# Restream/reindexer

Hardware: NVIDIA H100
Metric: KNN QPS @ recall@10 (10Mx768, k=10) + HBM GB/s vs roofline (higher is better)
Workload: dtype f32

## Files before the change

### include/rxgpu.h

```cpp
#ifndef RXGPU_H
#define RXGPU_H

#include <stddef.h>
#include <stdint.h>

#ifdef __cplusplus
extern "C" {
#endif

#define RXGPU_ABI_VERSION 4

enum { RXGPU_OK = 0, RXGPU_ERR_PARAMS = 3, RXGPU_ERR_LOGIC = 4, RXGPU_ERR_NOT_FOUND = 13, RXGPU_ERR_SYSTEM = 37 };

typedef enum { RXGPU_L2 = 0, RXGPU_IP = 1, RXGPU_COS = 2 } rxgpu_metric;

enum {
	RXGPU_FLAG_HOST_MIRROR = 1u
};

typedef struct rxgpu_index rxgpu_index;

const char* rxgpu_last_error(void);
int rxgpu_abi_version(void);
int rxgpu_device_count(void);
// ... 145 lines not shown
int rxgpu_sq8_prepare_query(const rxgpu_index*, const float* query, float query_norm, uint8_t* codes, float* offset);
int rxgpu_sq8_search_knn(const rxgpu_index*, uint32_t nq, const float* queries , const float* query_norms,
						 uint32_t k, float* out_dist, uint64_t* out_label, uint32_t* out_count);
int rxgpu_hnsw_search_knn_sq8(const rxgpu_index*, uint32_t nq, const float* queries , const float* query_norms, uint32_t k, uint32_t ef,
							  float* out_dist, uint64_t* out_label, uint32_t* out_count, uint32_t* stats );

int rxgpu_ivf_import(rxgpu_index*, uint32_t nlist, const float* centroids , const uint64_t* list_sizes );
int rxgpu_ivf_search_knn(const rxgpu_index*, uint32_t nq, const float* queries , uint32_t k, uint32_t nprobe, float* out_dist,
						 uint64_t* out_label, uint32_t* out_count);
int rxgpu_ivf_search_knn_large_k(const rxgpu_index*, uint32_t nq, const float* queries , uint32_t k, uint32_t nprobe,
								 float* out_dist, uint64_t* out_label, uint32_t* out_count);
int rxgpu_ivf_search_range(const rxgpu_index*, const float* query , float radius, uint32_t nprobe, uint64_t max_out,
						   float* out_dist, uint64_t* out_label, uint64_t* out_n);
int rxgpu_ivf_search_range_batch(const rxgpu_index*, uint32_t nq, const float* queries ,
								 const float* radius , uint32_t nprobe, uint64_t max_out,
								 float* out_dist, uint64_t* out_label, uint64_t* out_n );

int rxgpu_ivf_create(rxgpu_index*, uint32_t nlist, const float* centroids );
int rxgpu_ivf_add(rxgpu_index*, uint64_t n, const uint32_t* list_nos, const uint64_t* labels, const float* vecs );
int rxgpu_ivf_remove(rxgpu_index*, uint64_t label);
uint64_t rxgpu_ivf_size(const rxgpu_index*);
int rxgpu_ivf_list_stats(const rxgpu_index*, uint64_t* slab_rows, uint64_t* dead_rows, uint64_t* relocations, uint64_t* compactions);

typedef struct {
	int32_t niter;
	int32_t seed;
	int32_t max_points_per_centroid;
} rxgpu_ivf_train_params;
typedef struct {
	double obj;
	int32_t nsplit;
	float assign_ms;
	float update_ms;
	float host_ms;
} rxgpu_ivf_train_stats;
int rxgpu_ivf_train(rxgpu_index*, uint32_t nlist, uint64_t n, const float* vecs ,
					const float* norm_coefs , const rxgpu_ivf_train_params* params, float* out_centroids,
					rxgpu_ivf_train_stats* stats);
int rxgpu_ivf_assign(const rxgpu_index*, uint64_t n, const float* vecs , const float* norm_coefs, uint32_t* out_list_nos,
					 float* out_dist);
int rxgpu_ivf_add_assign(rxgpu_index*, uint64_t n, const uint64_t* labels, const float* vecs , const float* norm_coefs,
						 uint32_t* out_list_nos);
int rxgpu_kmeans_plan(uint64_t n, uint32_t nlist, int32_t seed, int32_t max_points_per_centroid, int32_t* out_sample, int32_t* out_init);

typedef struct {
	uint32_t ndocs;
	const uint32_t* doc_ids;
	const uint32_t* pos_begin;
	const uint32_t* positions;
} rxgpu_ft_postings;
typedef struct {
	double bm25_boost, bm25_weight, term_len_boost, term_len_weight, position_boost, position_weight;
} rxgpu_ft_field_config;
typedef struct {
	uint32_t merge_limit;
	int32_t min_rank;
	double bm25_k1, bm25_b;
	int32_t bm25_type;
	double distance_boost, distance_weight, full_match_boost;
	uint32_t nfields;
	const rxgpu_ft_field_config* fields;
	double summation_ranks_by_fields_ratio;
} rxgpu_ft_config;
typedef struct {
	int32_t op;
	float boost;
	float term_len_boost;
	const float* field_boosts;
	uint32_t nsubterms;
	const uint32_t* postings;
	const float* procs;
	const uint8_t* need_sum_rank;
	const uint8_t* suppressed;
	uint32_t nsynonyms;
	const uint32_t* synonym_ids;
	int32_t phrase_num;
	int32_t distance;
} rxgpu_ft_term;
typedef struct {
	uint32_t nterms;
	const rxgpu_ft_term* terms;
} rxgpu_ft_synonym;
typedef struct {
	uint32_t nterms;
	const rxgpu_ft_term* terms;
	uint32_t nsynonyms;
	const rxgpu_ft_synonym* synonyms;
} rxgpu_ft_query;
typedef struct {
	int32_t id;
	float proc;
	uint8_t field;
	uint8_t normalized_proc;
} rxgpu_ft_merge_info;
typedef struct rxgpu_ft_index rxgpu_ft_index;

int rxgpu_ft_create(rxgpu_ft_index** out, uint32_t total_docs, uint32_t nfields, const uint32_t* words_in_field, const float* avg_words,
					const uint8_t* removed, int device);
void rxgpu_ft_destroy(rxgpu_ft_index*);
int rxgpu_ft_add_postings(rxgpu_ft_index*, const rxgpu_ft_postings* list, uint32_t* out_id);
int rxgpu_ft_add_postings_packed(rxgpu_ft_index*, const uint8_t* data, uint64_t len, uint32_t count, uint32_t* out_id);
int rxgpu_ft_add_postings_packed_batch(rxgpu_ft_index*, uint32_t nlists, const uint8_t* const* data, const uint64_t* lens,
									   const uint32_t* counts, uint32_t* out_ids);
int rxgpu_ft_decode_packed(const uint8_t* data, uint64_t len, uint32_t count, uint32_t* doc_ids, uint32_t* pos_begin,
						   uint32_t* positions, uint64_t max_positions, uint64_t* npos);
int rxgpu_ft_merge(rxgpu_ft_index*, const rxgpu_ft_config* cfg, uint32_t nterms, const rxgpu_ft_term* terms, const uint8_t* excluded,
				   int rank_sort_type, uint64_t max_out, rxgpu_ft_merge_info* out, uint64_t* out_n);
int rxgpu_ft_merge_query(rxgpu_ft_index*, const rxgpu_ft_config* cfg, const rxgpu_ft_query* query, const uint8_t* excluded, int rank_sort_type,
						 uint64_t max_out, rxgpu_ft_merge_info* out, uint64_t* out_n);
typedef struct {
	uint32_t start, end;
} rxgpu_ft_area;
int rxgpu_ft_merge_query_areas(rxgpu_ft_index*, const rxgpu_ft_config* cfg, const rxgpu_ft_query* query, const uint8_t* excluded,
							   int rank_sort_type, int32_t max_areas_in_doc, uint64_t max_out, rxgpu_ft_merge_info* out,
							   uint32_t* out_area_begin, rxgpu_ft_area* out_areas, uint32_t* out_raw_count, uint64_t* out_n);
int rxgpu_ft_set_rows(rxgpu_ft_index*, const uint32_t* row_begin, const int32_t* row_ids);
int rxgpu_ft_select(rxgpu_ft_index*, const rxgpu_ft_config* cfg, uint32_t nterms, const rxgpu_ft_term* terms, const uint8_t* excluded,
					const uint8_t* row_status , int rank_sort_type, uint64_t limit, int32_t* out_row_ids,
					float* out_ranks , uint64_t* out_n);
int rxgpu_ft_select_query(rxgpu_ft_index*, const rxgpu_ft_config* cfg, const rxgpu_ft_query* query, const uint8_t* excluded,
						  const uint8_t* row_status, int rank_sort_type, uint64_t limit, int32_t* out_row_ids, float* out_ranks, uint64_t* out_n);
int rxgpu_sharded_ft_select(rxgpu_comm*, rxgpu_ft_index* shard, uint32_t doc_base, const rxgpu_ft_config* cfg, uint32_t nterms,
							const rxgpu_ft_term* terms, const uint8_t* excluded, const uint8_t* row_status, int rank_sort_type, uint64_t limit,
							int32_t* out_row_ids, float* out_ranks, uint64_t* out_n);
typedef struct {
	uint32_t launches;
	uint32_t preselected;
	uint64_t postings_scanned;
	uint64_t algorithmic_bytes;
	float device_ms;
} rxgpu_ft_stats;
void rxgpu_ft_last_stats(rxgpu_ft_stats* out);

int rxgpu_index_append_synth(rxgpu_index*, uint64_t seed, uint64_t first_row, uint64_t n);
int rxgpu_synth_fill_device(float* d_out, uint64_t seed, uint64_t first_index, uint64_t count, int device, void* stream);
int rxgpu_set_query_tile(rxgpu_index*, uint32_t qt);
typedef struct {
	uint32_t launches;
	uint32_t passes;
	uint32_t query_tile;
	uint32_t tie_replays;
	uint32_t tie_from_lists;
	uint64_t algorithmic_bytes;
	uint32_t scan_launches;
	float scan_kernel_ms;
	uint32_t tc_used;
	uint32_t tc_fallbacks;
	uint64_t tc_candidates;
	uint32_t tc_cluster;
	uint32_t tc_kernel;
} rxgpu_search_stats;
void rxgpu_last_search_stats(rxgpu_search_stats* out);
int rxgpu_set_tensor_core_filter(rxgpu_index*, int mode);
int rxgpu_set_profile(int on);
int rxgpu_tc_diag(int mode, void* d_counters);
int rxgpu_tc_audit(const rxgpu_index*, uint32_t nq, const float* queries, const float* tau, uint32_t query_block, uint32_t* out_shape,
                   uint32_t* slot_row, float* rowc, float* blockc, signed char* row_codes, signed char* query_codes, float* qc, float* kab,
                   int32_t* block_thr, float* row_bound);

#ifdef __cplusplus
}
#endif
#endif
```

### reindexer_b200/binding.py

```python
from __future__ import annotations

import ctypes as C
import os

import numpy as np

_HERE = os.path.dirname(os.path.abspath(__file__))
LIB_PATH = os.path.join(_HERE, "librxgpu.so")

L2, IP, COS = 0, 1, 2
FLAG_HOST_MIRROR = 1

_f32p = C.POINTER(C.c_float)
_u64p = C.POINTER(C.c_uint64)
_u32p = C.POINTER(C.c_uint32)
_i32p = C.POINTER(C.c_int32)
_u8p = C.POINTER(C.c_uint8)


class RxGpuError(RuntimeError):
    def __init__(self, code, msg):
        super().__init__(f"[{code}] {msg}")
        self.code = code
        self.what = msg
# ... 36 lines not shown
                ("postings", _u32p), ("procs", _f32p), ("need_sum_rank", _u8p), ("suppressed", _u8p), ("nsynonyms", C.c_uint32),
                ("synonym_ids", _u32p), ("phrase_num", C.c_int32), ("distance", C.c_int32)]


class FtSynonym(C.Structure):
    _fields_ = [("nterms", C.c_uint32), ("terms", C.POINTER(FtTerm))]


class FtQuery(C.Structure):
    _fields_ = [("nterms", C.c_uint32), ("terms", C.POINTER(FtTerm)), ("nsynonyms", C.c_uint32), ("synonyms", C.POINTER(FtSynonym))]


class Sq8Params(C.Structure):
    _fields_ = [("min_q", C.c_float), ("max_q", C.c_float), ("alpha", C.c_float), ("alpha_2", C.c_float), ("delta", C.c_float)]


class FtStats(C.Structure):
    _fields_ = [("launches", C.c_uint32), ("preselected", C.c_uint32), ("postings_scanned", C.c_uint64), ("algorithmic_bytes", C.c_uint64),
                ("device_ms", C.c_float)]


FT_MERGE_INFO_DTYPE = np.dtype([("id", np.int32), ("proc", np.float32), ("field", np.uint8), ("normalized_proc", np.uint8)], align=True)


class IvfTrainParams(C.Structure):
    _fields_ = [("niter", C.c_int32), ("seed", C.c_int32), ("max_points_per_centroid", C.c_int32)]


class IvfTrainStats(C.Structure):
    _fields_ = [("obj", C.c_double), ("nsplit", C.c_int32), ("assign_ms", C.c_float), ("update_ms", C.c_float), ("host_ms", C.c_float)]


class HnswBuildStats(C.Structure):
    _fields_ = [("batches", C.c_uint64), ("rows", C.c_uint64), ("distances", C.c_uint64), ("reverse_links", C.c_uint64),
                ("lists_pruned", C.c_uint64), ("search_select_ms", C.c_float), ("sort_ms", C.c_float), ("link_ms", C.c_float)]


class SearchStats(C.Structure):
    _fields_ = [("launches", C.c_uint32), ("passes", C.c_uint32), ("query_tile", C.c_uint32), ("tie_replays", C.c_uint32), ("tie_from_lists", C.c_uint32),
                ("algorithmic_bytes", C.c_uint64), ("scan_launches", C.c_uint32), ("scan_kernel_ms", C.c_float),
                ("tc_used", C.c_uint32), ("tc_fallbacks", C.c_uint32), ("tc_candidates", C.c_uint64), ("tc_cluster", C.c_uint32), ("tc_kernel", C.c_uint32)]


_SIGNATURES = {
    "rxgpu_last_error": (C.c_char_p, []),
    "rxgpu_abi_version": (C.c_int, []),
    "rxgpu_device_count": (C.c_int, []),
    "rxgpu_index_create": (C.c_int, [C.POINTER(C.c_void_p), C.c_int, C.c_uint32, C.c_uint64, C.c_int, C.c_uint32]),
    "rxgpu_index_clone": (C.c_int, [C.POINTER(C.c_void_p), C.c_void_p, C.c_uint64]),
    "rxgpu_index_destroy": (None, [C.c_void_p]),
    "rxgpu_index_resize": (C.c_int, [C.c_void_p, C.c_uint64]),
    "rxgpu_index_upsert": (C.c_int, [C.c_void_p, C.c_uint64, _f32p]),
    "rxgpu_index_upsert_batch": (C.c_int, [C.c_void_p, C.c_uint64, _u64p, _f32p]),
    "rxgpu_index_remove": (C.c_int, [C.c_void_p, C.c_uint64]),
    "rxgpu_index_get": (C.c_int, [C.c_void_p, C.c_uint64, C.POINTER(_f32p)]),
    "rxgpu_index_size": (C.c_uint64, [C.c_void_p]),
    "rxgpu_index_capacity": (C.c_uint64, [C.c_void_p]),
    "rxgpu_index_element_size": (C.c_uint64, [C.c_void_p]),
    "rxgpu_index_device_bytes": (C.c_uint64, [C.c_void_p]),
    "rxgpu_index_dim": (C.c_uint32, [C.c_void_p]),
    "rxgpu_index_metric": (C.c_int, [C.c_void_p]),
    "rxgpu_index_device": (C.c_int, [C.c_void_p]),
    "rxgpu_search_knn": (C.c_int, [C.c_void_p, C.c_uint32, _f32p, C.c_uint32, _f32p, _u64p, _u32p]),
    "rxgpu_search_range": (C.c_int, [C.c_void_p, _f32p, C.c_float, C.c_uint64, _f32p, _u64p, _u64p]),
    "rxgpu_search_range_batch": (C.c_int, [C.c_void_p, C.c_uint32, _f32p, _f32p, C.c_uint64, _f32p, _u64p, _u64p]),
    "rxgpu_last_range_results": (C.c_int, [C.c_uint64, C.c_uint64, _f32p, _u64p]),
    "rxgpu_comm_unique_id": (C.c_int, [C.c_void_p]),
    "rxgpu_comm_create": (C.c_int, [C.POINTER(C.c_void_p), C.c_int, C.c_int, C.c_void_p, C.c_int]),
    "rxgpu_comm_destroy": (None, [C.c_void_p]),
    "rxgpu_comm_rank": (C.c_int, [C.c_void_p]),
    "rxgpu_comm_size": (C.c_int, [C.c_void_p]),
    "rxgpu_sharded_search_knn": (C.c_int, [C.c_void_p, C.c_void_p, C.c_uint32, C.c_void_p, C.c_int, C.c_uint32, _f32p, _u64p, _u32p]),
    "rxgpu_sharded_search_range_batch": (C.c_int, [C.c_void_p, C.c_void_p, C.c_uint32, C.c_void_p, C.c_int, _f32p, C.c_uint64, _f32p, _u64p,
                                                   _u64p]),
    "rxgpu_shard_payload_bytes": (C.c_uint64, [C.c_uint32, C.c_uint32]),
    "rxgpu_merge_shards_device": (C.c_int, [C.c_uint32, C.c_uint32, C.c_uint32, C.c_uint32, C.c_void_p, C.c_void_p, C.c_void_p, C.c_void_p,
                                            C.c_void_p, C.c_void_p, C.c_void_p]),
    "rxgpu_search_knn_device": (C.c_int, [C.c_void_p, C.c_uint32, C.c_void_p, C.c_uint32, C.c_void_p, C.c_void_p, C.c_void_p,
                                          C.c_void_p, C.c_void_p]),
    "rxgpu_search_tie_rows_device": (C.c_int, [C.c_void_p, C.c_void_p, C.c_float, C.c_uint32, C.c_void_p, C.c_void_p, C.c_void_p,
                                               C.c_void_p, C.c_void_p]),
    "rxgpu_merge_shards": (C.c_int, [C.c_uint32, C.c_uint32, C.c_uint32, C.c_uint32, _f32p, _u32p, _u64p, _u32p, _u64p, _f32p, _u64p,
                                     _u64p, _u32p, _u8p]),
    "rxgpu_tie_replay": (C.c_int, [C.c_uint32, C.c_float, C.c_uint32, _f32p, _u64p, _u64p, C.c_uint32, _f32p, _u64p, _u64p, _f32p,
                                   _u64p, _u32p]),
    "rxgpu_select_knn": (C.c_int, [C.c_void_p, _f32p, C.POINTER(SelectParams), C.c_uint64, _i32p, _f32p, _u64p]),
    "rxgpu_select_postprocess": (C.c_int, [C.c_int, C.POINTER(SelectParams), C.c_uint64, _f32p, _u64p, _i32p, _f32p, _u64p]),
    "rxgpu_hnsw_import": (C.c_int, [C.c_void_p, C.POINTER(HnswGraph)]),
    "rxgpu_hnsw_search_knn": (C.c_int, [C.c_void_p, C.c_uint32, _f32p, C.c_uint32, C.c_uint32, _f32p, _u64p, _u32p, _u32p]),
    "rxgpu_hnsw_mark_deleted": (C.c_int, [C.c_void_p, C.c_uint64]),
    "rxgpu_hnsw_deleted_count": (C.c_uint64, [C.c_void_p]),
    "rxgpu_gather_labels_device": (C.c_int, [C.c_void_p, C.c_uint64, C.c_void_p, C.c_void_p, C.c_void_p]),
    "rxgpu_hnsw_search_range": (C.c_int, [C.c_void_p, _f32p, C.c_float, C.c_uint32, C.c_uint64, _f32p, _u64p, C.POINTER(C.c_uint64)]),
    "rxgpu_hnsw_search_range_batch": (C.c_int, [C.c_void_p, C.c_uint32, _f32p, _f32p, C.c_uint32, C.c_uint64, _f32p, _u64p, _u64p]),
    "rxgpu_hnsw_build": (C.c_int, [C.c_void_p, C.c_uint32, C.c_uint32, C.c_uint64, _i32p, C.c_uint64, C.POINTER(HnswBuildStats)]),
    "rxgpu_hnsw_build_plan": (C.c_int, [C.c_uint32, C.c_uint64, C.c_uint64, C.c_int32, _i32p, C.c_uint64, _i32p, _u64p, C.POINTER(C.c_uint64)]),
    "rxgpu_hnsw_export": (C.c_int, [C.c_void_p, C.c_uint64, _u32p, _u32p, _i32p, C.POINTER(C.c_int64), _u32p, C.POINTER(HnswGraph)]),
    "rxgpu_hnsw_search_knn_device": (C.c_int, [C.c_void_p, C.c_uint32, C.c_void_p, C.c_uint32, C.c_uint32, C.c_void_p, C.c_void_p,
                                               C.c_void_p, C.c_void_p, C.c_void_p]),
    "rxgpu_ivf_create": (C.c_int, [C.c_void_p, C.c_uint32, _f32p]),
    "rxgpu_ivf_add": (C.c_int, [C.c_void_p, C.c_uint64, _u32p, _u64p, _f32p]),
    "rxgpu_ivf_remove": (C.c_int, [C.c_void_p, C.c_uint64]),
    "rxgpu_ivf_size": (C.c_uint64, [C.c_void_p]),
    "rxgpu_ivf_list_stats": (C.c_int, [C.c_void_p, C.POINTER(C.c_uint64), C.POINTER(C.c_uint64), C.POINTER(C.c_uint64), C.POINTER(C.c_uint64)]),
    "rxgpu_hnsw_load_index_cache": (C.c_int, [C.c_void_p, C.c_void_p, C.c_void_p]),
    "rxgpu_hnsw_update": (C.c_int, [C.c_void_p, C.c_int32, C.c_uint32, C.c_uint32, C.c_void_p]),
    "rxgpu_hnsw_update_count": (C.c_uint64, [C.c_void_p]),
    "rxgpu_hnsw_stream_begin": (C.c_int, [C.c_void_p, _f32p, C.c_uint32, C.POINTER(C.c_void_p)]),
    "rxgpu_hnsw_stream_next": (C.c_int, [C.c_void_p, C.c_uint32, _f32p, _u64p, _u32p, C.POINTER(C.c_int)]),
    "rxgpu_hnsw_stream_end": (None, [C.c_void_p]),
    "rxgpu_sq8_attach": (C.c_int, [C.c_void_p, C.POINTER(Sq8Params), _u8p, _f32p]),
    "rxgpu_sq8_export": (C.c_int, [C.c_void_p, _u8p, _f32p]),
    "rxgpu_sq8_prepare_query": (C.c_int, [C.c_void_p, _f32p, C.c_float, _u8p, _f32p]),
    "rxgpu_sq8_search_knn": (C.c_int, [C.c_void_p, C.c_uint32, _f32p, _f32p, C.c_uint32, _f32p, _u64p, _u32p]),
    "rxgpu_hnsw_search_knn_sq8": (C.c_int, [C.c_void_p, C.c_uint32, _f32p, _f32p, C.c_uint32, C.c_uint32, _f32p, _u64p, _u32p, _u32p]),
    "rxgpu_ivf_import": (C.c_int, [C.c_void_p, C.c_uint32, _f32p, _u64p]),
    "rxgpu_ivf_train": (C.c_int, [C.c_void_p, C.c_uint32, C.c_uint64, _f32p, _f32p, C.POINTER(IvfTrainParams), _f32p, C.POINTER(IvfTrainStats)]),
    "rxgpu_ivf_assign": (C.c_int, [C.c_void_p, C.c_uint64, _f32p, _f32p, _u32p, _f32p]),
    "rxgpu_ivf_add_assign": (C.c_int, [C.c_void_p, C.c_uint64, _u64p, _f32p, _f32p, _u32p]),
    "rxgpu_kmeans_plan": (C.c_int, [C.c_uint64, C.c_uint32, C.c_int32, C.c_int32, _i32p, _i32p]),
    "rxgpu_ivf_search_knn": (C.c_int, [C.c_void_p, C.c_uint32, _f32p, C.c_uint32, C.c_uint32, _f32p, _u64p, _u32p]),
    "rxgpu_ivf_search_knn_large_k": (C.c_int, [C.c_void_p, C.c_uint32, _f32p, C.c_uint32, C.c_uint32, _f32p, _u64p, _u32p]),
    "rxgpu_ivf_search_range": (C.c_int, [C.c_void_p, _f32p, C.c_float, C.c_uint32, C.c_uint64, _f32p, _u64p, C.POINTER(C.c_uint64)]),
    "rxgpu_ivf_search_range_batch": (C.c_int, [C.c_void_p, C.c_uint32, _f32p, _f32p, C.c_uint32, C.c_uint64, _f32p, _u64p, _u64p]),
    "rxgpu_ft_create": (C.c_int, [C.POINTER(C.c_void_p), C.c_uint32, C.c_uint32, _u32p, _f32p, _u8p, C.c_int]),
    "rxgpu_ft_destroy": (None, [C.c_void_p]),
    "rxgpu_ft_add_postings": (C.c_int, [C.c_void_p, C.POINTER(FtPostings), _u32p]),
    "rxgpu_ft_add_postings_packed": (C.c_int, [C.c_void_p, _u8p, C.c_uint64, C.c_uint32, _u32p]),
    "rxgpu_ft_decode_packed": (C.c_int, [_u8p, C.c_uint64, C.c_uint32, _u32p, _u32p, _u32p, C.c_uint64, C.POINTER(C.c_uint64)]),
    "rxgpu_ft_merge": (C.c_int, [C.c_void_p, C.POINTER(FtConfig), C.c_uint32, C.POINTER(FtTerm), _u8p, C.c_int, C.c_uint64, C.c_void_p,
                                 C.POINTER(C.c_uint64)]),
    "rxgpu_ft_add_postings_packed_batch": (C.c_int, [C.c_void_p, C.c_uint32, C.POINTER(C.c_void_p), C.POINTER(C.c_uint64), _u32p, _u32p]),
    "rxgpu_ft_merge_query": (C.c_int, [C.c_void_p, C.c_void_p, C.c_void_p, _u8p, C.c_int, C.c_uint64, C.c_void_p, C.POINTER(C.c_uint64)]),
    "rxgpu_ft_merge_query_areas": (C.c_int, [C.c_void_p, C.c_void_p, C.c_void_p, _u8p, C.c_int, C.c_int32, C.c_uint64, C.c_void_p, _u32p,
                                              C.c_void_p, _u32p, C.POINTER(C.c_uint64)]),
    "rxgpu_ft_select_query": (C.c_int, [C.c_void_p, C.c_void_p, C.c_void_p, _u8p, _u8p, C.c_int, C.c_uint64, _i32p, _f32p,
                                         C.POINTER(C.c_uint64)]),
    "rxgpu_ft_set_rows": (C.c_int, [C.c_void_p, _u32p, _i32p]),
    "rxgpu_sharded_ft_select": (C.c_int, [C.c_void_p, C.c_void_p, C.c_uint32, C.POINTER(FtConfig), C.c_uint32, C.POINTER(FtTerm), _u8p, _u8p,
                                           C.c_int, C.c_uint64, _i32p, _f32p, C.POINTER(C.c_uint64)]),
    "rxgpu_comm_create_local": (C.c_int, [C.POINTER(C.c_void_p), C.c_int, C.POINTER(C.c_int)]),
    "rxgpu_ft_select": (C.c_int, [C.c_void_p, C.POINTER(FtConfig), C.c_uint32, C.POINTER(FtTerm), _u8p, _u8p, C.c_int, C.c_uint64, _i32p, _f32p,
                                  C.POINTER(C.c_uint64)]),
    "rxgpu_ft_last_stats": (None, [C.POINTER(FtStats)]),
    "rxgpu_index_append_synth": (C.c_int, [C.c_void_p, C.c_uint64, C.c_uint64, C.c_uint64]),
    "rxgpu_synth_fill_device": (C.c_int, [C.c_void_p, C.c_uint64, C.c_uint64, C.c_uint64, C.c_int, C.c_void_p]),
    "rxgpu_set_query_tile": (C.c_int, [C.c_void_p, C.c_uint32]),
    "rxgpu_last_search_stats": (None, [C.POINTER(SearchStats)]),
    "rxgpu_set_profile": (C.c_int, [C.c_int]),
    "rxgpu_tc_diag": (C.c_int, [C.c_int, C.c_void_p]),
    "rxgpu_tc_audit": (C.c_int, [C.c_void_p, C.c_uint32, _f32p, _f32p, C.c_uint32, _u32p, _u32p, _f32p, _f32p, C.c_void_p, C.c_void_p, _f32p,
                                 _f32p, _i32p, _f32p]),
    "rxgpu_set_tensor_core_filter": (C.c_int, [C.c_void_p, C.c_int]),
}

_lib = None


def lib():
    global _lib
    if _lib is None:
        if not os.path.exists(LIB_PATH):
            raise RxGpuError(37, f"{LIB_PATH} is missing: build the CUDA extension first (no CPU fallback exists)")
        l = C.CDLL(LIB_PATH)
        for name, (res, args) in _SIGNATURES.items():
            fn = getattr(l, name)
            fn.restype = res
            fn.argtypes = args
        _lib = l
    return _lib


def _check(rc):
    if rc != 0:
        raise RxGpuError(rc, lib().rxgpu_last_error().decode(errors="replace"))


def _p(a, t):
    return a.ctypes.data_as(t)


def device_count() -> int:
    return lib().rxgpu_device_count()


def last_search_stats() -> dict:
    s = SearchStats()
    lib().rxgpu_last_search_stats(C.byref(s))
    return {f: getattr(s, f) for f, _ in SearchStats._fields_}


class GpuBruteforceSearch:

    def __init__(self, metric: int, dim: int, capacity: int, device: int = 0, host_mirror: bool = False, _handle=None):
        self._lib = lib()
        self.metric, self.dim = metric, dim
        if _handle is not None:
            self._h = _handle
            return
        h = C.c_void_p()
        _check(self._lib.rxgpu_index_create(C.byref(h), metric, dim, capacity, device, FLAG_HOST_MIRROR if host_mirror else 0))
        self._h = h

    def close(self):
        if getattr(self, "_h", None):
            self._lib.rxgpu_index_destroy(self._h)
            self._h = None

    __del__ = close

    def clone(self, new_capacity: int) -> "GpuBruteforceSearch":
        h = C.c_void_p()
        _check(self._lib.rxgpu_index_clone(C.byref(h), self._h, new_capacity))
        return GpuBruteforceSearch(self.metric, self.dim, new_capacity, _handle=h)

    def max_elements(self) -> int:
        return self._lib.rxgpu_index_capacity(self._h)

    def current_element_count(self) -> int:
        return self._lib.rxgpu_index_size(self._h)

    size = current_element_count

    def element_size(self) -> int:
        return self._lib.rxgpu_index_element_size(self._h)

    def device_bytes(self) -> int:
        return self._lib.rxgpu_index_device_bytes(self._h)

    def add_point(self, vec, label: int):
        vec = np.ascontiguousarray(vec, dtype=np.float32)
        assert vec.size == self.dim
        _check(self._lib.rxgpu_index_upsert(self._h, label, _p(vec, _f32p)))

    def add_points(self, labels, vecs):
        vecs = np.ascontiguousarray(vecs, dtype=np.float32)
        labels = np.ascontiguousarray(labels, dtype=np.uint64)
        assert vecs.shape == (len(labels), self.dim)
        _check(self._lib.rxgpu_index_upsert_batch(self._h, len(labels), _p(labels, _u64p), _p(vecs, _f32p)))

    def remove_point(self, label: int):
        _check(self._lib.rxgpu_index_remove(self._h, label))

    def resize_index(self, new_capacity: int):
        _check(self._lib.rxgpu_index_resize(self._h, new_capacity))

    def float_ptr_by_external_label(self, label: int) -> np.ndarray:
        p = _f32p()
        _check(self._lib.rxgpu_index_get(self._h, label, C.byref(p)))
        return np.ctypeslib.as_array(p, (self.dim,)).copy()

    def search_knn(self, queries, k: int):
        q = np.ascontiguousarray(queries, dtype=np.float32)
        single = q.ndim == 1
        q = q.reshape(-1, self.dim)
        nq = q.shape[0]
        d = np.zeros((nq, max(k, 1)), np.float32)
        l = np.zeros((nq, max(k, 1)), np.uint64)
        c = np.zeros(nq, np.uint32)
        _check(self._lib.rxgpu_search_knn(self._h, nq, _p(q, _f32p), k, _p(d, _f32p), _p(l, _u64p), _p(c, _u32p)))
        if single:
            return d[0, :c[0]], l[0, :c[0]]
        return d[:, :k], l[:, :k], c

    def search_range(self, query, radius: float, max_out: int | None = None):
        q = np.ascontiguousarray(query, dtype=np.float32)
        max_out = self.size() if max_out is None else max_out
        d = np.zeros(max(max_out, 1), np.float32)
        l = np.zeros(max(max_out, 1), np.uint64)
        n = C.c_uint64(0)
        _check(self._lib.rxgpu_search_range(self._h, _p(q, _f32p), radius, max_out, _p(d, _f32p), _p(l, _u64p), C.byref(n)))
        m = min(n.value, max_out)
        return d[:m], l[:m], n.value

    def search_range_batch(self, queries, radius, max_out: int | None = None):
        q = np.ascontiguousarray(queries, dtype=np.float32).reshape(-1, self.dim)
        nq = q.shape[0]
        r = np.ascontiguousarray(np.broadcast_to(np.asarray(radius, dtype=np.float32), (nq,)))
        max_out = min(self.size(), 1 << 17) if max_out is None else max_out
        d = np.zeros((nq, max(max_out, 1)), np.float32)
        l = np.zeros((nq, max(max_out, 1)), np.uint64)
        c = np.zeros(nq, np.uint64)
        _check(self._lib.rxgpu_search_range_batch(self._h, nq, _p(q, _f32p), _p(r, _f32p), max_out, _p(d, _f32p), _p(l, _u64p),
                                                  _p(c, _u64p)))
        return d[:, :max_out], l[:, :max_out], c

    def select(self, query, k: int | None = None, radius: float | None = None, need_sort=True, is_array=False, raw=False,
               max_out: int | None = None):
        q = np.ascontiguousarray(query, dtype=np.float32)
        prm = SelectParams(k or 0, int(radius is not None), float(radius or 0.0), int(need_sort), int(is_array), int(raw))
        max_out = max_out if max_out is not None else max(self.size(), 1)
        ids = np.zeros(max_out, np.int32)
        ranks = np.zeros(max_out, np.float32)
        n = C.c_uint64(0)
        _check(self._lib.rxgpu_select_knn(self._h, _p(q, _f32p), C.byref(prm), max_out, _p(ids, _i32p), _p(ranks, _f32p), C.byref(n)))
        m = min(n.value, max_out)
        return ids[:m], ranks[:m]

    def search_knn_device(self, nq, d_queries_ptr, k1, d_dist_ptr, d_idx_ptr, d_label_ptr, d_count_ptr, stream=0):
        _check(self._lib.rxgpu_search_knn_device(self._h, nq, d_queries_ptr, k1, d_dist_ptr, d_idx_ptr, d_label_ptr, d_count_ptr,
                                                 stream or None))

    def search_tie_rows_device(self, d_query_ptr, dstar, k, d_dist_ptr, d_idx_ptr, d_label_ptr, d_count_ptr, stream=0):
        _check(self._lib.rxgpu_search_tie_rows_device(self._h, d_query_ptr, dstar, k, d_dist_ptr, d_idx_ptr, d_label_ptr, d_count_ptr,
                                                      stream or None))

# ... 114 lines not shown
    def hnsw_update_count(self) -> int:
        return int(self._lib.rxgpu_hnsw_update_count(self._h))

    def hnsw_mark_deleted(self, label: int):
        _check(self._lib.rxgpu_hnsw_mark_deleted(self._h, int(label)))

    def hnsw_deleted_count(self) -> int:
        return int(self._lib.rxgpu_hnsw_deleted_count(self._h))

    def hnsw_search_knn_device(self, nq, d_queries_ptr, k, ef, d_dist_ptr, d_idx_ptr, d_count_ptr, d_stats_ptr=0, stream=0):
        _check(self._lib.rxgpu_hnsw_search_knn_device(self._h, nq, d_queries_ptr, k, ef, d_dist_ptr, d_idx_ptr, d_count_ptr,
                                                      d_stats_ptr or None, stream or None))

    def gather_labels_device(self, n, d_idx_ptr, d_label_ptr, stream=0):
        _check(self._lib.rxgpu_gather_labels_device(self._h, n, d_idx_ptr, d_label_ptr, stream or None))

    def hnsw_search_range(self, query, radius: float, ef: int, max_out: int | None = None):
        q = np.ascontiguousarray(query, dtype=np.float32)
        max_out = self.size() if max_out is None else max_out
        d = np.zeros(max(max_out, 1), np.float32)
        l = np.zeros(max(max_out, 1), np.uint64)
        n = C.c_uint64(0)
        _check(self._lib.rxgpu_hnsw_search_range(self._h, _p(q, _f32p), radius, ef, max_out, _p(d, _f32p), _p(l, _u64p), C.byref(n)))
        m = min(n.value, max_out)
        return d[:m], l[:m], n.value

    def hnsw_search_range_batch(self, queries, radii, ef: int, max_out: int):
        q = np.ascontiguousarray(queries, dtype=np.float32).reshape(-1, self.dim)
        nq = q.shape[0]
        r = np.ascontiguousarray(np.broadcast_to(np.asarray(radii, dtype=np.float32), (nq,)))
        d = np.zeros((nq, max(max_out, 1)), np.float32)
        l = np.zeros((nq, max(max_out, 1)), np.uint64)
        c = np.zeros(nq, np.uint64)
        _check(self._lib.rxgpu_hnsw_search_range_batch(self._h, nq, _p(q, _f32p), _p(r, _f32p), ef, max_out, _p(d, _f32p), _p(l, _u64p),
                                                       _p(c, _u64p)))
        return d[:, :max_out], l[:, :max_out], c

    def hnsw_stream(self, query, batch_size: int, ef: int = 0, max_batches: int = 10**9):
        q = np.ascontiguousarray(query, np.float32)
        s = C.c_void_p()
        _check(self._lib.rxgpu_hnsw_stream_begin(self._h, _p(q, _f32p), ef, C.byref(s)))
        try:
            for _ in range(max_batches):
                d = np.zeros(max(batch_size, 1), np.float32)
                l = np.zeros(max(batch_size, 1), np.uint64)
                n, ex = C.c_uint32(0), C.c_int(0)
                _check(self._lib.rxgpu_hnsw_stream_next(s, batch_size, _p(d, _f32p), _p(l, _u64p), C.byref(n), C.byref(ex)))
                yield d[:n.value].copy(), l[:n.value].copy()
                if ex.value:
                    break
        finally:
            self._lib.rxgpu_hnsw_stream_end(s)

    def sq8_attach(self, params: dict, codes=None, offsets=None):
        p = Sq8Params(params["min_q"], params["max_q"], params["alpha"], params["alpha_2"], params["delta"])
        if codes is None:
            _check(self._lib.rxgpu_sq8_attach(self._h, C.byref(p), None, None))
        else:
            c = np.ascontiguousarray(codes, np.uint8)
            o = np.ascontiguousarray(offsets, np.float32)
            assert c.shape == (self.size(), self.dim) and o.shape == (self.size(),)
            _check(self._lib.rxgpu_sq8_attach(self._h, C.byref(p), _p(c, _u8p), _p(o, _f32p)))

    def sq8_export(self):
        codes = np.zeros((self.size(), self.dim), np.uint8)
        offs = np.zeros(self.size(), np.float32)
        _check(self._lib.rxgpu_sq8_export(self._h, _p(codes, _u8p), _p(offs, _f32p)))
        return codes, offs

    def sq8_prepare_query(self, query, query_norm=1.0):
        q = np.ascontiguousarray(query, np.float32)
        codes = np.zeros(self.dim, np.uint8)
        off = C.c_float(0)
        _check(self._lib.rxgpu_sq8_prepare_query(self._h, _p(q, _f32p), query_norm, _p(codes, _u8p), C.byref(off)))
        return codes, off.value

    def _sq8_search(self, fn, queries, k, query_norms, extra):
        q = np.ascontiguousarray(queries, dtype=np.float32).reshape(-1, self.dim)
        nq = q.shape[0]
        qn = None if query_norms is None else np.ascontiguousarray(query_norms, np.float32)
        d = np.zeros((nq, max(k, 1)), np.float32)
        l = np.zeros((nq, max(k, 1)), np.uint64)
        c = np.zeros(nq, np.uint32)
        _check(fn(self._h, nq, _p(q, _f32p), None if qn is None else _p(qn, _f32p), k, *extra, _p(d, _f32p), _p(l, _u64p), _p(c, _u32p)))
        return d, l, c

    def sq8_search_knn(self, queries, k: int, query_norms=None):
        return self._sq8_search(self._lib.rxgpu_sq8_search_knn, queries, k, query_norms, ())

    def hnsw_search_knn_sq8(self, queries, k: int, ef: int = 0, query_norms=None, with_stats=False):
        q = np.ascontiguousarray(queries, dtype=np.float32).reshape(-1, self.dim)
        nq = q.shape[0]
        qn = None if query_norms is None else np.ascontiguousarray(query_norms, np.float32)
        d = np.zeros((nq, max(k, 1)), np.float32)
        l = np.zeros((nq, max(k, 1)), np.uint64)
        c = np.zeros(nq, np.uint32)
        st = np.zeros((nq, 2), np.uint32)
        _check(self._lib.rxgpu_hnsw_search_knn_sq8(self._h, nq, _p(q, _f32p), None if qn is None else _p(qn, _f32p), k, ef, _p(d, _f32p),
                                                   _p(l, _u64p), _p(c, _u32p), _p(st, _u32p)))
        return (d, l, c, st) if with_stats else (d, l, c)

    def ivf_import(self, centroids, list_sizes):
        c = np.ascontiguousarray(centroids, np.float32)
        ls = np.ascontiguousarray(list_sizes, np.uint64)
        _check(self._lib.rxgpu_ivf_import(self._h, len(ls), _p(c, _f32p), _p(ls, _u64p)))

    def ivf_search_knn(self, queries, k: int, nprobe: int):
        q = np.ascontiguousarray(queries, dtype=np.float32).reshape(-1, self.dim)
        nq = q.shape[0]
        d = np.zeros((nq, max(k, 1)), np.float32)
        l = np.zeros((nq, max(k, 1)), np.uint64)
        c = np.zeros(nq, np.uint32)
        _check(self._lib.rxgpu_ivf_search_knn(self._h, nq, _p(q, _f32p), k, nprobe, _p(d, _f32p), _p(l, _u64p), _p(c, _u32p)))
        return d, l, c

    def ivf_search_knn_large_k(self, queries, k: int, nprobe: int):
        q = np.ascontiguousarray(queries, dtype=np.float32).reshape(-1, self.dim)
        nq = q.shape[0]
        d = np.zeros((nq, max(k, 1)), np.float32)
        l = np.zeros((nq, max(k, 1)), np.uint64)
        c = np.zeros(nq, np.uint32)
        _check(self._lib.rxgpu_ivf_search_knn_large_k(self._h, nq, _p(q, _f32p), k, nprobe, _p(d, _f32p), _p(l, _u64p), _p(c, _u32p)))
        return d, l, c

    def ivf_search_range(self, query, radius: float, nprobe: int, max_out: int | None = None):
        q = np.ascontiguousarray(query, dtype=np.float32)
        max_out = max(self.size(), self.ivf_size()) if max_out is None else max_out
        d = np.zeros(max(max_out, 1), np.float32)
        l = np.zeros(max(max_out, 1), np.uint64)
        n = C.c_uint64(0)
        _check(self._lib.rxgpu_ivf_search_range(self._h, _p(q, _f32p), radius, nprobe, max_out, _p(d, _f32p), _p(l, _u64p), C.byref(n)))
        m = min(n.value, max_out)
        return d[:m], l[:m], n.value

    def ivf_search_range_batch(self, queries, radii, nprobe: int, max_out: int):
        q = np.ascontiguousarray(queries, dtype=np.float32).reshape(-1, self.dim)
        nq = q.shape[0]
        r = np.ascontiguousarray(np.broadcast_to(np.asarray(radii, dtype=np.float32), (nq,)))
        d = np.zeros((nq, max(max_out, 1)), np.float32)
        l = np.zeros((nq, max(max_out, 1)), np.uint64)
        c = np.zeros(nq, np.uint64)
        _check(self._lib.rxgpu_ivf_search_range_batch(self._h, nq, _p(q, _f32p), _p(r, _f32p), nprobe, max_out, _p(d, _f32p), _p(l, _u64p),
                                                      _p(c, _u64p)))
        return d[:, :max_out], l[:, :max_out], c

    def append_synth(self, seed: int, first_row: int, n: int):
        _check(self._lib.rxgpu_index_append_synth(self._h, seed, first_row, n))

    def set_query_tile(self, qt: int):
        _check(self._lib.rxgpu_set_query_tile(self._h, qt))

    def set_tensor_core_filter(self, mode: int):
        _check(self._lib.rxgpu_set_tensor_core_filter(self._h, mode))

    def tc_audit(self, queries, tau, query_block: int = 128, row_bound: bool = True) -> dict:
        q = np.ascontiguousarray(queries, dtype=np.float32).reshape(-1, self.dim)
        nq = q.shape[0]
        t = np.ascontiguousarray(np.broadcast_to(np.asarray(tau, dtype=np.float32), (nq,)))
        shape = np.zeros(2, np.uint32)
        _check(self._lib.rxgpu_tc_audit(self._h, 0, None, None, query_block, _p(shape, _u32p), *([None] * 9)))
        S, B = int(shape[0]), int(shape[1])
        o = {"slot_row": np.zeros(max(S, 1), np.uint32), "rowc": np.zeros((max(S, 1), 4), np.float32),
             "blockc": np.zeros((max(B, 1), 8), np.float32), "row_codes": np.zeros((max(S, 1), self.dim), np.int8),
             "query_codes": np.zeros((max(nq, 1), self.dim), np.int8), "qc": np.zeros((max(nq, 1), 4), np.float32),
             "kab": np.zeros((max((nq + query_block - 1) // query_block, 1), 2), np.float32),
             "block_thr": np.zeros((max(nq, 1), max(B, 1)), np.int32),
             "row_bound": np.zeros((max(nq, 1), max(S, 1), 2), np.float32) if row_bound and S else None}
        _check(self._lib.rxgpu_tc_audit(self._h, nq, _p(q, _f32p), _p(t, _f32p), query_block, _p(shape, _u32p), _p(o["slot_row"], _u32p),
                                        _p(o["rowc"], _f32p), _p(o["blockc"], _f32p), o["row_codes"].ctypes.data,
                                        o["query_codes"].ctypes.data, _p(o["qc"], _f32p), _p(o["kab"], _f32p), _p(o["block_thr"], _i32p),
                                        None if o["row_bound"] is None else _p(o["row_bound"], _f32p)))
        nqb = (nq + query_block - 1) // query_block
        out = {"slot_row": o["slot_row"][:S], "rowc": o["rowc"][:S], "blockc": o["blockc"][:B], "row_codes": o["row_codes"][:S],
               "query_codes": o["query_codes"][:nq], "qc": o["qc"][:nq], "kab": o["kab"][:nqb], "block_thr": o["block_thr"][:nq, :B],
               "row_bound": None if o["row_bound"] is None else o["row_bound"][:nq, :S]}
        return out


COMM_ID_BYTES = 128


def comm_unique_id() -> bytes:
    buf = C.create_string_buffer(COMM_ID_BYTES)
    _check(lib().rxgpu_comm_unique_id(buf))
    return buf.raw


class ShardComm:

    def __init__(self, nranks: int, rank: int, comm_id: bytes | None, device: int, _handle=None):
        self._lib = lib()
        if _handle is not None:
            self._h = _handle
            return
        self._h = C.c_void_p()
        idbuf = C.create_string_buffer(comm_id, COMM_ID_BYTES) if comm_id is not None else None
        _check(self._lib.rxgpu_comm_create(C.byref(self._h), nranks, rank, idbuf, device))

    @staticmethod
    def local_group(nranks: int, devices=None):
        hs = (C.c_void_p * nranks)()
        dv = None if devices is None else (C.c_int * nranks)(*devices)
        _check(lib().rxgpu_comm_create_local(hs, nranks, dv))
        return [ShardComm(nranks, r, None, 0, _handle=C.c_void_p(hs[r])) for r in range(nranks)]

    def close(self):
        if self._h:
            self._lib.rxgpu_comm_destroy(self._h)
            self._h = C.c_void_p()

    def __del__(self):
        try:
            self.close()
        except Exception:
            pass

    def search_knn(self, shard: "GpuBruteforceSearch", queries, k: int, nq: int | None = None):
        if isinstance(queries, np.ndarray):
            q = np.ascontiguousarray(queries, np.float32)
            nq, qp, on_dev = q.shape[0], q.ctypes.data_as(C.c_void_p), 0
        else:
            qp, on_dev = C.c_void_p(int(queries)), 1
        kk = max(k, 1)
        od = np.zeros((nq, kk), np.float32)
        ol = np.zeros((nq, kk), np.uint64)
        oc = np.zeros(nq, np.uint32)
        _check(self._lib.rxgpu_sharded_search_knn(self._h, shard._h, nq, qp, on_dev, k, _p(od, _f32p), _p(ol, _u64p), _p(oc, _u32p)))
        return od, ol, oc

    def search_range_batch(self, shard: "GpuBruteforceSearch", queries, radius, max_out: int, nq: int | None = None):
        if isinstance(queries, np.ndarray):
            q = np.ascontiguousarray(queries, np.float32)
            nq, qp, on_dev = q.shape[0], q.ctypes.data_as(C.c_void_p), 0
        else:
            qp, on_dev = C.c_void_p(int(queries)), 1
        r = np.ascontiguousarray(np.broadcast_to(np.asarray(radius, dtype=np.float32), (nq,)))
        od = np.zeros((nq, max(max_out, 1)), np.float32)
        ol = np.zeros((nq, max(max_out, 1)), np.uint64)
        oc = np.zeros(nq, np.uint64)
        _check(self._lib.rxgpu_sharded_search_range_batch(self._h, shard._h, nq, qp, on_dev, _p(r, _f32p), max_out, _p(od, _f32p),
                                                          _p(ol, _u64p), _p(oc, _u64p)))
        return od[:, :max_out], ol[:, :max_out], oc


def select_postprocess(metric, dist, label, k=None, has_radius=False, need_sort=True, is_array=False, raw=False):
    d = np.ascontiguousarray(dist, np.float32)
    l = np.ascontiguousarray(label, np.uint64)
    prm = SelectParams(k or 0, int(has_radius), 0.0, int(need_sort), int(is_array), int(raw))
    ids = np.zeros(max(len(d), 1), np.int32)
    ranks = np.zeros(max(len(d), 1), np.float32)
    n = C.c_uint64(0)
    _check(lib().rxgpu_select_postprocess(metric, C.byref(prm), len(d), _p(d, _f32p), _p(l, _u64p), _p(ids, _i32p), _p(ranks, _f32p), C.byref(n)))
    return ids[:n.value], ranks[:n.value]


def merge_shards(k, dist, idx, label, count, shard_base):
    dist = np.ascontiguousarray(dist, np.float32)
    idx = np.ascontiguousarray(idx, np.uint32)
    label = np.ascontiguousarray(label, np.uint64)
    count = np.ascontiguousarray(count, np.uint32)
    base = np.ascontiguousarray(shard_base, np.uint64)
    ns, nq, k1 = dist.shape
    od = np.zeros((nq, max(k, 1)), np.float32)
    og = np.zeros((nq, max(k, 1)), np.uint64)
    ol = np.zeros((nq, max(k, 1)), np.uint64)
    oc = np.zeros(nq, np.uint32)
    nt = np.zeros(nq, np.uint8)
    _check(lib().rxgpu_merge_shards(ns, nq, k, k1, _p(dist, _f32p), _p(idx, _u32p), _p(label, _u64p), _p(count, _u32p), _p(base, _u64p),
                                    _p(od, _f32p), _p(og, _u64p), _p(ol, _u64p), _p(oc, _u32p), _p(nt, _u8p)))
    return od, og, ol, oc, nt


def tie_replay(k, dstar, lower, first):
    ld, lg, ll = (np.ascontiguousarray(a, t) for a, t in zip(lower, (np.float32, np.uint64, np.uint64)))
    fd, fg, fl = (np.ascontiguousarray(a, t) for a, t in zip(first, (np.float32, np.uint64, np.uint64)))
    od = np.zeros(max(k, 1), np.float32)
    ol = np.zeros(max(k, 1), np.uint64)
    oc = C.c_uint32(0)
    _check(lib().rxgpu_tie_replay(k, dstar, len(ld), _p(ld, _f32p), _p(lg, _u64p), _p(ll, _u64p), len(fd), _p(fd, _f32p), _p(fg, _u64p),
                                  _p(fl, _u64p), _p(od, _f32p), _p(ol, _u64p), C.byref(oc)))
    return od[:oc.value], ol[:oc.value]


class GpuFtIndex:

    def __init__(self, total_docs, words_in_field, avg_words, removed=None, device=0):
        self._lib = lib()
        w = np.ascontiguousarray(words_in_field, np.uint32).reshape(total_docs, -1)
        self.total_docs, self.nfields = total_docs, w.shape[1]
        a = np.ascontiguousarray(avg_words, np.float32)
        r = None if removed is None else np.ascontiguousarray(removed, np.uint8)
        h = C.c_void_p()
        _check(self._lib.rxgpu_ft_create(C.byref(h), total_docs, self.nfields, _p(w, _u32p), _p(a, _f32p), None if r is None else _p(r, _u8p),
                                         device))
        self._h = h

    def close(self):
        if getattr(self, "_h", None):
            self._lib.rxgpu_ft_destroy(self._h)
            self._h = None

    __del__ = close

    def add_postings(self, doc_ids, pos_begin, positions) -> int:
        d = np.ascontiguousarray(doc_ids, np.uint32)
        b = np.ascontiguousarray(pos_begin, np.uint32)
# ... 161 lines not shown
```

### reindexer_b200/csrc/index.cu

```cuda
#include <cuda_runtime.h>

#include <cub/device/device_radix_sort.cuh>
#include <cub/device/device_scan.cuh>
#include <cub/device/device_segmented_radix_sort.cuh>
#include <cub/device/device_segmented_sort.cuh>

#include <algorithm>
#include <atomic>
#include <cstdio>
#include <cstdlib>
#include <cstring>
#include <limits>
#include <memory>
#include <mutex>
#include <new>
#include <string>
#include <unordered_map>
#include <unordered_set>
#include <vector>

#include "../../include/rxgpu.h"
#include "internal.h"
#include "../host/knn_select.h"
#include "knn_scan.cuh"
// ... 520 lines not shown
		auto convert = [&](uint32_t b, uint32_t e) {
			const unsigned blocks = unsigned((uint64_t(e - b) * 32 + 255) / 256);
			tc_convert_rows<<<blocks, 256, 0, st>>>(ix->d_rows, ix->pitch, ix->dim, b, e, ix->d_row_slot, static_cast<unsigned char*>(ix->d_shadow),
													pitchQ / kTcChunkK, ix->metric == RXGPU_COS ? ix->d_norms : nullptr, ix->d_rowc);
			g_stats.launches += 1;
		};
		bool full = ix->shadow_dirty_all;
		if (!full) {
			const uint32_t kept = std::min(old, size), added = size - kept, gone = old - kept;
			uint64_t rewritten = 0;
			for (const auto& r : ix->shadow_dirty) {
				rewritten += r.first < kept ? std::min(r.second, kept) - r.first : 0u;
			}
			const uint64_t slots = uint64_t(ix->shadow_slots) + added;
			full = slots > ix->shadow_slot_cap ||
				   (uint64_t(ix->shadow_dead) + gone + ix->shadow_unsorted + added + rewritten) * kShadowResortDiv > slots;
			if (!full) {
				if (gone) {
					tc_kill_rows<<<(gone + 255) / 256, 256, 0, st>>>(kept, old, ix->d_row_slot, ix->d_slot_row, ix->d_rowc);
					g_stats.launches += 1;
				}
				for (const auto& r : ix->shadow_dirty) {
					if (r.first < kept) {
						convert(r.first, std::min(r.second, kept));
					}
				}
				if (added) {
					tc_assign_slots<<<(added + 255) / 256, 256, 0, st>>>(kept, size, ix->shadow_slots, ix->d_slot_row, ix->d_row_slot);
					g_stats.launches += 1;
					convert(kept, size);
				}
				ix->shadow_slots = uint32_t(slots);
				ix->shadow_dead += gone;
				ix->shadow_unsorted += uint32_t(added + rewritten);
			}
		}
		if (full) {
			if (size) {
				if (int rc = sortShadowSlots(ix, st, size)) {
					return rc;
				}
				convert(0, size);
			}
			ix->shadow_slots = size;
			ix->shadow_dead = 0;
			ix->shadow_unsorted = 0;
		}
		ix->shadow_rows = size;
		ix->shadow_dirty_all = false;
		ix->shadow_dirty.clear();
		const uint32_t slots = ix->shadow_slots;
		const uint64_t padded = (uint64_t(slots) + kTcTileRows - 1) / kTcTileRows * kTcTileRows;
		RX_CUDA(cudaMemsetAsync(ix->d_rowc + slots, 0, size_t(padded - slots) * sizeof(float4), st));
		const uint32_t nblocks = uint32_t(padded / 64);
		if (nblocks) {
			tc_block_consts<<<(nblocks * 32 + 255) / 256, 256, 0, st>>>(ix->d_rowc, ix->d_slot_row, slots, nblocks,
																		   1.f - tc_l2eps(ix->dim), ix->metric, ix->d_blockc);
			g_stats.launches += 1;
		}
		RX_CUDA(cudaGetLastError());
		RX_CUDA(cudaStreamSynchronize(st));
		ix->shadow_version = ix->version;
	}
	return 0;
}

constexpr uint32_t kTcClusterDefault = 2;
constexpr uint64_t kTcClusterMinRows = 1u << 23;
uint32_t tcClusterSize(uint32_t nblocks, uint32_t ntiles, uint32_t cmax) {
	for (uint32_t c = cmax; c > 1; c /= 2) {
		const uint32_t pad = (c - nblocks % c) % c;
		if (ntiles >= 2 && pad <= 1 && pad < nblocks) {
			return c;
		}
	}
	return 1;
}

struct TcBatch {
	uint32_t nq, nqb, cluster, ngroups, nqPad, kchunks, stages, queueSlots;
	int diag;
	size_t smem;
	int resident;
	TcKernel kfn;
	CUtensorMap mapQ;
};

int tcPrepare(const rxgpu_index* ix, Workspace& ws, cudaStream_t st, const float* d_queries, uint32_t nq, uint32_t candCap, TcBatch& b) {
	if (int rc = ensureShadow(ix, st)) {
		return rc;
	}
	const uint32_t pitchQ = ix->pitch_q, kchunks = pitchQ / kTcChunkK;
	const uint32_t nqb = tcQueryBlock(nq, kchunks);
	const uint32_t ntiles = uint32_t((ix->size + kTcTileRows - 1) / kTcTileRows);
	const uint32_t nblocks = (nq + nqb - 1) / nqb;
	const uint32_t cmax = ix->tc_cluster_max ? ix->tc_cluster_max : ix->size >= kTcClusterMinRows ? kTcClusterDefault : 1u;
	const uint32_t cluster = tcClusterSize(nblocks, ntiles, cmax);
	const uint32_t ngroups = (nblocks + cluster - 1) / cluster;
	const uint32_t nqPad = ngroups * cluster * nqb;
	RX_CUDA(ws.d_qcodes.ensure(size_t(nqPad) * pitchQ));
	RX_CUDA(ws.d_qc.ensure(nqPad));
	RX_CUDA(ws.d_qf.ensure(size_t(nqPad) * pitchQ));
	RX_CUDA(ws.d_tau.ensure(nqPad));
	RX_CUDA(ws.d_cand_count.ensure(nqPad));
	RX_CUDA(ws.d_cand_rows.ensure(size_t(nqPad) * candCap));
	RX_CUDA(ws.h_cand_count.ensure(nqPad));
	tc_prepare_queries<<<(nqPad * 32 + 255) / 256, 256, 0, st>>>(d_queries, nq, nqPad, ix->dim, pitchQ, ws.d_qcodes.p, ws.d_qc.p,
																 ws.d_qf.p);
	g_stats.launches += 1;
	RX_CUDA(cudaGetLastError());
	if (int rc = makeCodeMap(&b.mapQ, ws.d_qcodes.p, pitchQ, nqPad, nqb)) {
		return rc;
	}
	b.kfn = tcKernel(nqb, cluster);
	b.stages = tc_ring_stages(nqb, kchunks, kTcSmemLimit);
	b.queueSlots = tc_queue_slots(nqb, kchunks, b.stages, kTcSmemLimit);
	b.smem = tc_smem_bytes(nqb, kchunks, b.stages) + tc_queue_bytes(b.queueSlots);
	if (b.stages == 0 || b.queueSlots == 0) {
		return fail(RXGPU_ERR_SYSTEM, "rxgpu: no room for the tensor-core filter's candidate queues");
	}
	b.diag = g_tc_diag.load();
	if (const int diag = b.diag) {
		if (nqb != 128) {
			return fail(RXGPU_ERR_PARAMS, "rxgpu: the diagnostic filter instantiations take query blocks of 128");
		}
		b.kfn = tcDiagKernel(diag, cluster);
	}
	RX_CUDA(raiseSmemCeilingOnce(b.kfn, ix->device, int(kTcSmemLimit)));
	cudaLaunchConfig_t cfg{};
	cfg.gridDim = dim3(unsigned(ix->sm_count) / cluster * cluster);
	cfg.blockDim = dim3(kTcThreads);
	cfg.dynamicSmemBytes = b.smem;
	cudaLaunchAttribute attr[1];
	attr[0].id = cudaLaunchAttributeClusterDimension;
	attr[0].val.clusterDim.x = cluster;
	attr[0].val.clusterDim.y = 1;
	attr[0].val.clusterDim.z = 1;
	cfg.attrs = attr;
	cfg.numAttrs = 1;
	b.resident = 0;
	RX_CUDA(cudaOccupancyMaxActiveClusters(&b.resident, b.kfn, &cfg));
	if (b.resident < 1) {
		return fail(RXGPU_ERR_SYSTEM, "rxgpu: tensor-core filter kernel cannot be made resident");
	}
	b.nq = nq;
	b.nqb = nqb;
	b.cluster = cluster;
	b.ngroups = ngroups;
	b.nqPad = nqPad;
	b.kchunks = kchunks;
	return 0;
}

int tcLaunch(const rxgpu_index* ix, Workspace& ws, cudaStream_t st, const TcBatch& b, uint32_t k1, uint32_t candCap, uint32_t nrows, bool fixedTau) {
	const uint32_t nq = b.nq, nqb = b.nqb, cluster = b.cluster, ngroups = b.ngroups, kchunks = b.kchunks, pitchQ = ix->pitch_q;
	const uint32_t ntiles = (nrows + kTcTileRows - 1) / kTcTileRows;
	const int resident = b.resident;
	const TcKernel kfn = b.kfn;
	const CUtensorMap mapQ = b.mapQ;
	RX_CUDA(cudaMemsetAsync(ws.d_cand_count.p, 0, size_t(b.nqPad) * 4, st));
	RX_CUDA(cudaGetLastError());
	cudaLaunchConfig_t cfg{};
	cfg.blockDim = dim3(kTcThreads);
	cfg.dynamicSmemBytes = b.smem;
	cfg.stream = st;
	cudaLaunchAttribute attr[1];
	attr[0].id = cudaLaunchAttributeClusterDimension;
	attr[0].val.clusterDim.x = cluster;
	attr[0].val.clusterDim.y = 1;
	attr[0].val.clusterDim.z = 1;
	cfg.attrs = attr;
	cfg.numAttrs = 1;
	TcArgs a{};
	a.shadow = static_cast<const unsigned char*>(ix->d_shadow);
	a.rowc = ix->d_rowc;
	a.slot_row = ix->d_slot_row;
	a.blockc = ix->d_blockc;
	a.qc = ws.d_qc.p;
	a.tau = ws.d_tau.p;
	a.ub_list = fixedTau ? nullptr : ws.d_ub_list.p;
	a.ub_lock = fixedTau ? nullptr : ws.d_ub_lock.p;
	a.init_rows = fixedTau ? UINT32_MAX : uint32_t(std::min<uint64_t>(ix->size, kTcInitRows));
	a.rows = ix->d_rows;
	a.norm_coefs = ix->metric == RXGPU_COS ? ix->d_norms : nullptr;
	a.qf = ws.d_qf.p;
	a.pitch = ix->pitch;
	a.cand_rows = ws.d_cand_rows.p;
	a.cand_count = ws.d_cand_count.p;
	a.cand_cap = candCap;
	a.n = nrows;
	a.dim = ix->dim;
	a.kchunks = kchunks;
	a.nq_total = nq;
	a.k1 = k1;
	a.metric = ix->metric;
	a.queue_slots = b.queueSlots;
	a.stages = b.stages;
	a.diag = g_tc_diag_buf;
	for (uint32_t g0 = 0; g0 < ngroups;) {
		const uint32_t groups = std::min<uint32_t>(ngroups - g0, uint32_t(resident));
		const uint32_t walkers = uint32_t(std::min<uint64_t>(uint32_t(resident) / groups, ntiles));
		cfg.gridDim = dim3(groups * walkers * cluster);
		a.q0 = g0 * cluster * nqb;
		a.groups = groups;
		cudaEvent_t e0 = nullptr, e1 = nullptr;
		if (g_profile.load(std::memory_order_relaxed)) {
			RX_CUDA(cudaEventCreate(&e0));
			RX_CUDA(cudaEventCreate(&e1));
			RX_CUDA(cudaEventRecord(e0, st));
		}
		RX_CUDA(cudaLaunchKernelEx(&cfg, kfn, mapQ, a));
		RX_CUDA(cudaGetLastError());
		if (e0) {
			RX_CUDA(cudaEventRecord(e1, st));
			g_prof_events.emplace_back(e0, e1);
		}
		g_stats.launches += 1;
		g_stats.passes += 1;
		const uint32_t served = std::min(groups * cluster * nqb, nq - a.q0);
		g_stats.algorithmic_bytes += uint64_t(nrows) * pitchQ + uint64_t(nrows) * sizeof(float4) + uint64_t(served) * pitchQ;
		g0 += groups;
	}
	g_stats.tc_cluster = cluster;
	g_stats.tc_kernel = 1 + uint32_t(b.diag);
	g_stats.query_tile = nqb * cluster;
	return 0;
}

int tcFilter(const rxgpu_index* ix, Workspace& ws, cudaStream_t st, const float* d_queries, uint32_t nq, uint32_t k1, uint32_t candCap,
			 const unsigned int* h_tau) {
	TcBatch b;
	if (int rc = tcPrepare(ix, ws, st, d_queries, nq, candCap, b)) {
		return rc;
	}
	if (h_tau) {
		RX_CUDA(cudaMemcpyAsync(ws.d_tau.p, h_tau, size_t(nq) * 4, cudaMemcpyHostToDevice, st));
	} else {
		RX_CUDA(ws.d_ub_list.ensure(size_t(b.nqPad) * kTcMaxK1));
		RX_CUDA(ws.d_ub_lock.ensure(b.nqPad));
		RX_CUDA(raiseSmemCeilingOnce(tc_init_tau, ix->device, int(tc_init_smem_bytes())));
		tc_init_tau<<<(nq + kTcInitQ - 1) / kTcInitQ, 256, tc_init_smem_bytes(), st>>>(
			ix->d_rows, ix->pitch, b.kchunks, ix->metric == RXGPU_COS ? ix->d_norms : nullptr, uint32_t(std::min<uint64_t>(ix->size, kTcInitRows)),
			ws.d_qf.p, nq, k1, ix->metric, ws.d_tau.p, ws.d_ub_list.p, ws.d_ub_lock.p);
		g_stats.launches += 1;
	}
	return tcLaunch(ix, ws, st, b, k1, candCap, ix->shadow_slots, h_tau != nullptr);
}

int rerankRange(const rxgpu_index* ix, Workspace& ws, cudaStream_t st, const float* d_queries, uint32_t nq, uint32_t nctas, const uint32_t* d_qsel,
				uint32_t cap, const float* d_radius, uint64_t* d_keys, unsigned int* d_nkeys) {
	RX_CUDA(cudaMemsetAsync(d_nkeys, 0, size_t(nq) * 4, st));
	const size_t rsmem = size_t((ix->dim + 127) / 128) * 512 + size_t(kScanWarps) * (1 + kCandBuf) * 8;
	const float* norms = ix->metric == RXGPU_COS ? ix->d_norms : nullptr;
	if (ix->metric == RXGPU_L2) {
		RX_CUDA(raiseSmemCeilingOnce(knn_rerank<true>, ix->device, kScanSmemBudget));
		knn_rerank<true><<<nctas, kScanThreads, rsmem, st>>>(ix->d_rows, ix->pitch, ix->dim, norms, d_queries, ws.d_cand_rows.p, ws.d_cand_count.p,
															  cap, 1, nullptr, d_qsel, nullptr, d_radius, d_keys, d_nkeys);
	} else {
		RX_CUDA(raiseSmemCeilingOnce(knn_rerank<false>, ix->device, kScanSmemBudget));
		knn_rerank<false><<<nctas, kScanThreads, rsmem, st>>>(ix->d_rows, ix->pitch, ix->dim, norms, d_queries, ws.d_cand_rows.p, ws.d_cand_count.p,
															   cap, 1, nullptr, d_qsel, nullptr, d_radius, d_keys, d_nkeys);
	}
	RX_CUDA(cudaGetLastError());
	g_stats.launches += 1;
	return 0;
}

int scanTopKStaged(const rxgpu_index* ix, Workspace& ws, cudaStream_t st, const float* d_queries, uint32_t nq, uint32_t k1,
				   float* d_out_dist, uint32_t* d_out_idx, uint64_t* d_out_label, uint32_t* d_out_count) {
	const uint32_t cap = stageCandCap(k1);
	const uint32_t size = uint32_t(ix->size);
	TcBatch b;
	if (int rc = tcPrepare(ix, ws, st, d_queries, nq, cap, b)) {
		return rc;
	}
	RX_CUDA(ws.d_radius.ensure(nq));
	RX_CUDA(ws.d_range_n.ensure(nq));
	RX_CUDA(ws.d_range.ensure(size_t(nq) * cap));
	RX_CUDA(ws.d_stage_status.ensure(nq));
	RX_CUDA(ws.h_stage_status.ensure(nq));
	RX_CUDA(ws.d_reranked.ensure(1));
	RX_CUDA(ws.h_reranked.ensure(1));
	RX_CUDA(cudaMemsetAsync(ws.d_reranked.p, 0, sizeof(unsigned long long), st));
	uint32_t rows = std::min(size, stageSeedRows(k1));
	if (int rc = scanTopKExact(ix, ws, st, d_queries, nq, k1, kModeTopK, 0.f, d_out_dist, d_out_idx, d_out_label, d_out_count, rows)) {
		return rc;
	}
	knn_seed_tau<<<(nq + 255) / 256, 256, 0, st>>>(d_out_dist, d_out_count, k1, nq, ws.d_tau.p, ws.d_radius.p, ws.d_stage_status.p);
	RX_CUDA(cudaGetLastError());
	g_stats.launches += 1;
	SelectArgs s{};
	s.keys = ws.d_range.p;
	s.nkeys = ws.d_range_n.p;
	s.cand_count = ws.d_cand_count.p;
	s.labels = ix->d_labels;
	s.cap = cap;
	s.k1 = k1;
	s.mode = kModeTopK;
	s.tau = ws.d_tau.p;
	s.radius = ws.d_radius.p;
	s.status = ws.d_stage_status.p;
	s.reranked = ws.d_reranked.p;
	s.out_dist = d_out_dist;
	s.out_idx = d_out_idx;
	s.out_label = d_out_label;
	s.out_count = d_out_count;
	s.neg_zero = ix->metric != RXGPU_L2;
	const uint32_t slots = ix->shadow_slots;
	uint32_t prefix = rows;
	do {
		prefix = uint32_t(std::min<uint64_t>(slots, uint64_t(prefix) * kStageRatio));
		if (int rc = tcLaunch(ix, ws, st, b, k1, cap, prefix, true)) {
			return rc;
		}
		if (int rc = rerankRange(ix, ws, st, d_queries, nq, nq, nullptr, cap, ws.d_radius.p, ws.d_range.p, ws.d_range_n.p)) {
			return rc;
		}
		s.last = prefix == slots;
		knn_select_topk<<<nq, kSelThreads, 0, st>>>(s);
		RX_CUDA(cudaGetLastError());
		g_stats.launches += 1;
	} while (prefix < slots);
	RX_CUDA(cudaMemcpyAsync(ws.h_cand_count.p, ws.d_cand_count.p, size_t(nq) * 4, cudaMemcpyDeviceToHost, st));
	RX_CUDA(cudaMemcpyAsync(ws.h_stage_status.p, ws.d_stage_status.p, size_t(nq) * 4, cudaMemcpyDeviceToHost, st));
	RX_CUDA(cudaMemcpyAsync(ws.h_reranked.p, ws.d_reranked.p, sizeof(unsigned long long), cudaMemcpyDeviceToHost, st));
	RX_CUDA(cudaStreamSynchronize(st));
	for (uint32_t q = 0; q < nq; ++q) {
		if (ws.h_stage_status.p[q]) {
			g_stats.tc_fallbacks += 1;
			ws.h_cand_count.p[q] = UINT32_MAX;
			if (int rc = scanTopKExact(ix, ws, st, d_queries + size_t(q) * ix->dim, 1, k1, kModeTopK, 0.f, d_out_dist + size_t(q) * k1,
									   d_out_idx + size_t(q) * k1, d_out_label ? d_out_label + size_t(q) * k1 : nullptr, d_out_count + q)) {
				return rc;
			}
		}
	}
	ws.tc_lists_valid = true;
	ws.tc_lists_nq = nq;
	ws.tc_lists_cap = cap;
	ws.tc_lists_version = ix->version;
	g_stats.tc_used = 1;
	g_stats.tc_candidates = *ws.h_reranked.p;
	g_stats.algorithmic_bytes += *ws.h_reranked.p * (uint64_t(ix->dim) * 4 + 4);
	return 0;
}

int scanTopKTensorCore(const rxgpu_index* ix, Workspace& ws, cudaStream_t st, const float* d_queries, uint32_t nq, uint32_t k1,
					   float* d_out_dist, uint32_t* d_out_idx, uint64_t* d_out_label, uint32_t* d_out_count) {
	const uint32_t candCap = tcCandCap(k1);
	if (int rc = tcFilter(ix, ws, st, d_queries, nq, k1, candCap, nullptr)) {
		return rc;
	}
	RX_CUDA(ws.d_lists.ensure(size_t(nq) * k1));
	const size_t rsmem = size_t((ix->dim + 127) / 128) * 512 + size_t(kScanWarps) * (k1 + kCandBuf) * 8;
	const float* norms = ix->metric == RXGPU_COS ? ix->d_norms : nullptr;
	if (ix->metric == RXGPU_L2) {
		RX_CUDA(raiseSmemCeilingOnce(knn_rerank<true>, ix->device, kScanSmemBudget));
		knn_rerank<true><<<nq, kScanThreads, rsmem, st>>>(ix->d_rows, ix->pitch, ix->dim, norms, d_queries, ws.d_cand_rows.p,
														   ws.d_cand_count.p, candCap, k1, ws.d_lists.p);
	} else {
		RX_CUDA(raiseSmemCeilingOnce(knn_rerank<false>, ix->device, kScanSmemBudget));
		knn_rerank<false><<<nq, kScanThreads, rsmem, st>>>(ix->d_rows, ix->pitch, ix->dim, norms, d_queries, ws.d_cand_rows.p,
															ws.d_cand_count.p, candCap, k1, ws.d_lists.p);
	}
	MergeArgs m{};
	m.lists = ws.d_lists.p;
	m.labels = ix->d_labels;
	m.out_dist = d_out_dist;
	m.out_idx = d_out_idx;
	m.out_label = d_out_label;
	m.out_count = d_out_count;
	m.nlists = 1;
	m.qt = nq;
	m.k1 = k1;
	m.q_offset = 0;
	m.out_stride = k1;
	m.out_offset = 0;
	m.mode = kModeTopK;
	m.neg_zero = ix->metric != RXGPU_L2;
	knn_merge_lists<<<nq, 256, 0, st>>>(m);
	RX_CUDA(cudaGetLastError());
	g_stats.launches += 2;
	RX_CUDA(cudaMemcpyAsync(ws.h_cand_count.p, ws.d_cand_count.p, size_t(nq) * 4, cudaMemcpyDeviceToHost, st));
	RX_CUDA(cudaStreamSynchronize(st));
	uint64_t cands = 0;
	for (uint32_t q = 0; q < nq; ++q) {
		cands += std::min<unsigned>(ws.h_cand_count.p[q], candCap);
		if (ws.h_cand_count.p[q] > candCap) {
			g_stats.tc_fallbacks += 1;
			if (int rc = scanTopKExact(ix, ws, st, d_queries + size_t(q) * ix->dim, 1, k1, kModeTopK, 0.f, d_out_dist + size_t(q) * k1,
									   d_out_idx + size_t(q) * k1, d_out_label ? d_out_label + size_t(q) * k1 : nullptr, d_out_count + q)) {
				return rc;
			}
		}
	}
	ws.tc_lists_valid = true;
	ws.tc_lists_nq = nq;
	ws.tc_lists_cap = candCap;
	ws.tc_lists_version = ix->version;
	g_stats.tc_used = 1;
	g_stats.tc_candidates = cands;
	g_stats.algorithmic_bytes += cands * (uint64_t(ix->dim) * 4 + 4);
	return 0;
}

}

namespace rxgpu {
int scanTopK(const rxgpu_index* ix, Workspace& ws, cudaStream_t st, const float* d_queries, uint32_t nq, uint32_t k1, int mode, float bound,
			 float* d_out_dist, uint32_t* d_out_idx, uint64_t* d_out_label, uint32_t* d_out_count) {
	if (tcEligible(ix, nq, k1, mode) && k1 > kTcMaxK1) {
		return scanTopKStaged(ix, ws, st, d_queries, nq, k1, d_out_dist, d_out_idx, d_out_label, d_out_count);
	}
	if (tcEligible(ix, nq, k1, mode)) {
		return scanTopKTensorCore(ix, ws, st, d_queries, nq, k1, d_out_dist, d_out_idx, d_out_label, d_out_count);
	}
	if (mode == kModeTopK) {
		ws.tc_lists_valid = false;
	}
	return scanTopKExact(ix, ws, st, d_queries, nq, k1, mode, bound, d_out_dist, d_out_idx, d_out_label, d_out_count);
}

int setRowAt(rxgpu_index* ix, uint32_t idx, uint64_t label, const float* vec) {
	if (idx > ix->size || (idx == ix->size && ix->size >= ix->capacity)) {
		return fail(RXGPU_ERR_LOGIC, "The number of elements exceeds the specified limit\n");
	}
	const uint32_t other = ix->dict.find(label);
	if (other != LabelMap::kNotFound && other != idx) {
		return fail(RXGPU_ERR_LOGIC, "rxgpu: label already belongs to another row");
	}
	RX_CUDA(ix->st_rows.ensure(ix->pitch));
	RX_CUDA(cudaMemsetAsync(ix->st_rows.p, 0, size_t(ix->pitch) * 4, ix->stream));
	RX_CUDA(cudaMemcpyAsync(ix->st_rows.p, vec, size_t(ix->dim) * 4, cudaMemcpyHostToDevice, ix->stream));
	RX_CUDA(cudaMemcpyAsync(ix->d_rows + size_t(idx) * ix->pitch, ix->st_rows.p, size_t(ix->pitch) * 4, cudaMemcpyDeviceToDevice, ix->stream));
	RX_CUDA(cudaMemcpyAsync(ix->d_labels + idx, &label, 8, cudaMemcpyHostToDevice, ix->stream));
	if (ix->metric == RXGPU_COS) {
		norm_coef_kernel<<<1, 32, 0, ix->stream>>>(ix->d_rows, ix->pitch, ix->dim, idx, idx + 1, ix->d_norms);
		RX_CUDA(cudaGetLastError());
	}
	RX_CUDA(cudaStreamSynchronize(ix->stream));
	if (idx < ix->size) {
		if (ix->h_labels[idx] != label) {
			ix->dict.erase(ix->h_labels[idx]);
		}
		ix->h_labels[idx] = label;
	} else {
		ix->h_labels.push_back(label);
		ix->size += 1;
	}
	ix->dict.put(label, idx);
	if (ix->flags & RXGPU_FLAG_HOST_MIRROR) {
		std::memcpy(ix->h_rows.data() + size_t(idx) * ix->dim, vec, ix->dim * sizeof(float));
	}
	ix->touchRows(idx, uint64_t(idx) + 1);
	ix->version++;
	return 0;
}

int tieRowsAfterScan(const rxgpu_index* ix, Workspace& ws, cudaStream_t st, const float* d_queries, uint32_t nsel, const uint32_t* sel,
					 const float* dstar, uint32_t k, float* d_out_dist, uint32_t* d_out_idx, uint64_t* d_out_label, uint32_t* d_out_count) {
	if (nsel == 0) {
		return 0;
	}
	bool fromLists = ws.tc_lists_valid && ws.tc_lists_version == ix->version && k < kTcStagedMaxK1;
	for (uint32_t i = 0; fromLists && i < nsel; ++i) {
		fromLists = sel[i] < ws.tc_lists_nq && ws.h_cand_count.p[sel[i]] <= ws.tc_lists_cap;
	}
	if (!fromLists) {
		for (uint32_t i = 0; i < nsel; ++i) {
			if (int rc = scanTopKExact(ix, ws, st, d_queries + size_t(sel[i]) * ix->dim, 1, k, kModeTieRows, dstar[i], d_out_dist + size_t(i) * k,
									   d_out_idx + size_t(i) * k, d_out_label ? d_out_label + size_t(i) * k : nullptr, d_out_count + i)) {
				return rc;
			}
		}
		g_stats.tie_replays += nsel;
		return 0;
	}
	RX_CUDA(ws.d_sel.ensure(nsel));
	RX_CUDA(cudaMemcpyAsync(ws.d_sel.p, sel, size_t(nsel) * 4, cudaMemcpyHostToDevice, st));
	if (k > kTcMaxK1) {
		const uint32_t nq = ws.tc_lists_nq, cap = ws.tc_lists_cap;
		std::vector<float> rad(nq, -INFINITY);
		for (uint32_t i = 0; i < nsel; ++i) {
			rad[sel[i]] = nextafterf(dstar[i], INFINITY);
		}
		RX_CUDA(ws.d_radius.ensure(nq));
		RX_CUDA(ws.d_range_n.ensure(nq));
		RX_CUDA(ws.d_range.ensure(size_t(nq) * cap));
		RX_CUDA(cudaMemcpyAsync(ws.d_radius.p, rad.data(), size_t(nq) * 4, cudaMemcpyHostToDevice, st));
		if (int rc = rerankRange(ix, ws, st, d_queries, nq, nsel, ws.d_sel.p, cap, ws.d_radius.p, ws.d_range.p, ws.d_range_n.p)) {
			return rc;
		}
		SelectArgs s{};
		s.keys = ws.d_range.p;
		s.nkeys = ws.d_range_n.p;
		s.cand_count = ws.d_cand_count.p;
		s.qsel = ws.d_sel.p;
		s.labels = ix->d_labels;
		s.cap = cap;
		s.k1 = k;
		s.mode = kModeTieRows;
		s.out_dist = d_out_dist;
		s.out_idx = d_out_idx;
		s.out_label = d_out_label;
		s.out_count = d_out_count;
		s.neg_zero = ix->metric != RXGPU_L2;
		knn_select_topk<<<nsel, kSelThreads, 0, st>>>(s);
		RX_CUDA(cudaGetLastError());
		g_stats.launches += 1;
		g_stats.tie_replays += nsel;
		g_stats.tie_from_lists += nsel;
		return 0;
	}
	RX_CUDA(ws.d_selbound.ensure(nsel));
	RX_CUDA(ws.d_lists.ensure(size_t(nsel) * k));
	RX_CUDA(cudaMemcpyAsync(ws.d_selbound.p, dstar, size_t(nsel) * 4, cudaMemcpyHostToDevice, st));
	const size_t rsmem = size_t((ix->dim + 127) / 128) * 512 + size_t(kScanWarps) * (k + kCandBuf) * 8;
	const float* norms = ix->metric == RXGPU_COS ? ix->d_norms : nullptr;
	if (ix->metric == RXGPU_L2) {
		RX_CUDA(raiseSmemCeilingOnce(knn_rerank<true>, ix->device, kScanSmemBudget));
		knn_rerank<true><<<nsel, kScanThreads, rsmem, st>>>(ix->d_rows, ix->pitch, ix->dim, norms, d_queries, ws.d_cand_rows.p, ws.d_cand_count.p,
															 ws.tc_lists_cap, k, ws.d_lists.p, ws.d_sel.p, ws.d_selbound.p);
	} else {
		RX_CUDA(raiseSmemCeilingOnce(knn_rerank<false>, ix->device, kScanSmemBudget));
		knn_rerank<false><<<nsel, kScanThreads, rsmem, st>>>(ix->d_rows, ix->pitch, ix->dim, norms, d_queries, ws.d_cand_rows.p, ws.d_cand_count.p,
															  ws.tc_lists_cap, k, ws.d_lists.p, ws.d_sel.p, ws.d_selbound.p);
	}
	MergeArgs m{};
	m.lists = ws.d_lists.p;
	m.labels = ix->d_labels;
	m.out_dist = d_out_dist;
	m.out_idx = d_out_idx;
	m.out_label = d_out_label;
	m.out_count = d_out_count;
	m.nlists = 1;
	m.qt = nsel;
	m.k1 = k;
	m.q_offset = 0;
	m.out_stride = k;
	m.out_offset = 0;
	m.mode = kModeTieRows;
	m.neg_zero = ix->metric != RXGPU_L2;
	knn_merge_lists<<<nsel, 256, 0, st>>>(m);
	RX_CUDA(cudaGetLastError());
	g_stats.launches += 2;
	g_stats.tie_replays += nsel;
// ... 211 lines not shown
				RX_CUDA(ix->st_labels.ensure(size_t(std::min(slice, m))));
				for (uint64_t off = 0; off < m; off += slice) {
					const uint64_t cnt = std::min(slice, m - off);
					RX_CUDA(cudaMemcpyAsync(ix->st_rows.p, vecs + off * ix->dim, size_t(cnt) * ix->dim * sizeof(float), cudaMemcpyHostToDevice,
											ix->stream));
					RX_CUDA(cudaMemcpyAsync(ix->st_dst.p, dst.data() + off, size_t(cnt) * sizeof(uint32_t), cudaMemcpyHostToDevice, ix->stream));
					RX_CUDA(cudaMemcpyAsync(ix->st_labels.p, labels + off, size_t(cnt) * sizeof(uint64_t), cudaMemcpyHostToDevice, ix->stream));
					bool dup = false;
					if (cnt > 1) {
						std::vector<uint32_t> sorted(dst.begin() + off, dst.begin() + off + cnt);
						std::sort(sorted.begin(), sorted.end());
						dup = std::adjacent_find(sorted.begin(), sorted.end()) != sorted.end();
					}
					if (!dup) {
						scatter_rows_kernel<<<unsigned(cnt), 128, 0, ix->stream>>>(ix->st_rows.p, ix->st_dst.p, ix->st_labels.p, uint32_t(cnt), ix->dim,
																				   ix->pitch, ix->d_rows, ix->d_labels);
						RX_CUDA(cudaGetLastError());
					} else {
						for (uint64_t i = 0; i < cnt; ++i) {
							scatter_rows_kernel<<<1, 128, 0, ix->stream>>>(ix->st_rows.p + i * ix->dim, ix->st_dst.p + i, ix->st_labels.p + i, 1, ix->dim,
																		   ix->pitch, ix->d_rows, ix->d_labels);
						}
						RX_CUDA(cudaGetLastError());
					}
					if (ix->metric == RXGPU_COS) {
						for (uint64_t i = 0; i < cnt;) {
							uint64_t j = i + 1;
							while (j < cnt && dst[off + j] == dst[off + j - 1] + 1) {
								++j;
							}
							if (int rc = normsForRange(ix, dst[off + i], uint64_t(dst[off + j - 1]) + 1)) {
								return rc;
							}
							i = j;
						}
					}
					if (off + slice < m) {
						RX_CUDA(cudaStreamSynchronize(ix->stream));
					}
				}
			}
			RX_CUDA(cudaStreamSynchronize(ix->stream));
			for (size_t i = 0; i < fresh.size(); ++i) {
				ix->dict.put(fresh[i], uint32_t(ix->size + i));
				ix->h_labels.push_back(fresh[i]);
			}
			if (ix->flags & RXGPU_FLAG_HOST_MIRROR) {
				for (uint64_t i = 0; i < m; ++i) {
					std::memcpy(ix->h_rows.data() + size_t(dst[i]) * ix->dim, vecs + i * ix->dim, ix->dim * sizeof(float));
				}
			}
			for (uint64_t i = 0; i < m;) {
				uint64_t j = i + 1;
				while (j < m && dst[j] == dst[j - 1] + 1) {
					++j;
				}
				ix->touchRows(dst[i], uint64_t(dst[j - 1]) + 1);
				i = j;
			}
			ix->size = newSize;
			ix->version++;
		}
		if (accepted < n) {
			return fail(RXGPU_ERR_LOGIC, "The number of elements exceeds the specified limit\n");
		}
	} catch (const std::bad_alloc&) {
		return fail(RXGPU_ERR_SYSTEM, "rxgpu: out of host memory");
	}
	return 0;
}

int rxgpu_index_upsert(rxgpu_index* ix, uint64_t label, const float* vec) { return rxgpu_index_upsert_batch(ix, 1, &label, vec); }

int rxgpu_index_remove(rxgpu_index* ix, uint64_t label) {
	if (int rc = checkIndex(ix)) {
		return rc;
	}
	const uint32_t cur = ix->dict.find(label);
	if (cur == LabelMap::kNotFound) {
		return 0;
	}
	ix->dict.erase(label);
	ix->version++;
	const uint64_t last = ix->size - 1;
	if (cur != last) {
		ix->touchRows(cur, uint64_t(cur) + 1);
		const uint64_t lastLabel = ix->h_labels[last];
		ix->dict.put(lastLabel, cur);
		ix->h_labels[cur] = lastLabel;
		RX_CUDA(cudaMemcpyAsync(ix->d_rows + size_t(cur) * ix->pitch, ix->d_rows + size_t(last) * ix->pitch, ix->pitch * sizeof(float),
								cudaMemcpyDeviceToDevice, ix->stream));
		RX_CUDA(cudaMemcpyAsync(ix->d_labels + cur, ix->d_labels + last, sizeof(uint64_t), cudaMemcpyDeviceToDevice, ix->stream));
		if (ix->d_norms) {
			RX_CUDA(cudaMemcpyAsync(ix->d_norms + cur, ix->d_norms + last, sizeof(float), cudaMemcpyDeviceToDevice, ix->stream));
		}
		if (ix->flags & RXGPU_FLAG_HOST_MIRROR) {
			std::memcpy(ix->h_rows.data() + size_t(cur) * ix->dim, ix->h_rows.data() + size_t(last) * ix->dim, ix->dim * sizeof(float));
		}
		RX_CUDA(cudaStreamSynchronize(ix->stream));
	}
	ix->h_labels.pop_back();
	ix->size--;
	return 0;
}

int rxgpu_index_get(const rxgpu_index* ix, uint64_t label, const float** host_row) {
	if (!ix || !host_row) {
		return fail(RXGPU_ERR_PARAMS, "rxgpu: null handle");
	}
	const uint32_t idx = ix->dict.find(label);
	if (idx == LabelMap::kNotFound) {
		return fail(RXGPU_ERR_NOT_FOUND, "Label not found");
	}
	if (ix->flags & RXGPU_FLAG_HOST_MIRROR) {
		*host_row = ix->h_rows.data() + size_t(idx) * ix->dim;
		return 0;
	}
	RX_CUDA(cudaSetDevice(ix->device));
	g_row_scratch.resize(ix->dim);
	RX_CUDA(cudaMemcpy(g_row_scratch.data(), ix->d_rows + size_t(idx) * ix->pitch, ix->dim * sizeof(float), cudaMemcpyDeviceToHost));
	*host_row = g_row_scratch.data();
	return 0;
}

uint64_t rxgpu_index_size(const rxgpu_index* ix) { return ix ? ix->size : 0; }
uint64_t rxgpu_index_capacity(const rxgpu_index* ix) { return ix ? ix->capacity : 0; }
uint64_t rxgpu_index_element_size(const rxgpu_index* ix) { return ix ? uint64_t(ix->dim) * 4 + 8 : 0; }
uint64_t rxgpu_index_device_bytes(const rxgpu_index* ix) {
	if (!ix) {
		return 0;
	}
	const uint64_t cap = ix->capacity ? ix->capacity : 1;
	return cap * ix->pitch * 4 + cap * 8 + (ix->d_norms ? cap * 4 : 0);
}
uint32_t rxgpu_index_dim(const rxgpu_index* ix) { return ix ? ix->dim : 0; }
int rxgpu_index_metric(const rxgpu_index* ix) { return ix ? ix->metric : -1; }
int rxgpu_index_device(const rxgpu_index* ix) { return ix ? ix->device : -1; }

int rxgpu_set_query_tile(rxgpu_index* ix, uint32_t qt) {
	if (!ix) {
		return fail(RXGPU_ERR_PARAMS, "rxgpu: null handle");
	}
	ix->qt_override = qt;
	return 0;
}
int rxgpu_set_tensor_core_filter(rxgpu_index* ix, int mode) {
	if (!ix || mode < 0 || mode > 5) {
		return fail(RXGPU_ERR_PARAMS, "rxgpu: tensor-core filter mode must be 0..5");
	}
	ix->tc_mode = uint32_t(mode >= 3 ? 1 : mode);
	ix->tc_cluster_max = mode == 3 ? 1u : mode == 4 ? 2u : mode == 5 ? 4u : 0u;
	return 0;
}
int rxgpu_tc_diag(int mode, void* d_counters) {
	if (mode < 0 || mode > kTcDiagNoTest || (mode && !d_counters)) {
		return fail(RXGPU_ERR_PARAMS, "rxgpu: diagnostic filter mode must be 0..4, with a counter buffer");
	}
	const char* env = std::getenv("RXGPU_TC_DIAG");
	if (mode && !(env && std::strcmp(env, "1") == 0)) {
		return fail(RXGPU_ERR_LOGIC, "rxgpu: diagnostic filter instantiations are enabled only with RXGPU_TC_DIAG=1 in the environment");
	}
	g_tc_diag_buf = static_cast<unsigned long long*>(d_counters);
	g_tc_diag.store(mode);
	return 0;
}
int rxgpu_tc_audit(const rxgpu_index* ix, uint32_t nq, const float* queries, const float* tau, uint32_t query_block, uint32_t* out_shape,
				   uint32_t* slot_row, float* rowc, float* blockc, signed char* row_codes, signed char* query_codes, float* qc, float* kab,
				   int32_t* block_thr, float* row_bound) {
	if (int rc = checkIndex(ix)) {
		return rc;
	}
	if (!out_shape || (nq && (!queries || !tau)) || query_block == 0 || query_block > kTcMaxNq || query_block % 32) {
		return fail(RXGPU_ERR_PARAMS, "rxgpu: audit needs the shape output, queries with their thresholds and a query block of 32..128");
	}
	RX_CUDA(cudaSetDevice(ix->device));
	cudaStream_t st = ix->stream;
	if (int rc = ensureShadow(ix, st)) {
		return rc;
	}
	const uint32_t pitch = ix->pitch_q, kchunks = pitch / kTcChunkK, dim = ix->dim, slots = ix->shadow_slots;
	const uint32_t nblocks = uint32_t((uint64_t(slots) + kTcTileRows - 1) / kTcTileRows * kTcTileRows / 64);
	const uint32_t nqblocks = (nq + query_block - 1) / query_block;
	out_shape[0] = slots;
	out_shape[1] = nblocks;
	auto fetch = [&](void* dst, const void* src, size_t bytes) -> cudaError_t {
		return dst && bytes ? cudaMemcpy(dst, src, bytes, cudaMemcpyDeviceToHost) : cudaSuccess;
	};
	RX_CUDA(fetch(slot_row, ix->d_slot_row, size_t(slots) * 4));
	RX_CUDA(fetch(rowc, ix->d_rowc, size_t(slots) * sizeof(float4)));
	RX_CUDA(fetch(blockc, ix->d_blockc, size_t(nblocks) * 2 * sizeof(float4)));
	std::vector<signed char> sh(size_t(nblocks) * 64 * pitch), codes(size_t(nblocks) * 64 * pitch);
	RX_CUDA(fetch(sh.data(), ix->d_shadow, sh.size()));
	for (uint32_t s = 0; s < nblocks * 64; ++s) {
		const uint32_t blk = s / 64, r = s % 64;
		for (uint32_t c = 0; c < pitch; c += 16) {
			const uint32_t kc = c / kTcChunkK, unit = ((c % kTcChunkK) >> 4) ^ (r & 7u);
			std::memcpy(&codes[size_t(s) * pitch + c], &sh[(size_t(blk) * kchunks + kc) * kTcBlockBytes + r * 128u + unit * 16u], 16);
		}
	}
	if (row_codes) {
		for (uint32_t s = 0; s < slots; ++s) {
			std::memcpy(row_codes + size_t(s) * dim, &codes[size_t(s) * pitch], dim);
		}
	}
	if (nq == 0) {
		return 0;
	}
	DevBuf<float> d_q, d_qf, d_tau;
	DevBuf<unsigned char> d_qcodes;
	DevBuf<signed char> d_rcodes;
	DevBuf<float4> d_qc;
	DevBuf<float2> d_kab, d_bound;
	DevBuf<int> d_thr;
	RX_CUDA(d_q.ensure(size_t(nq) * dim));
	RX_CUDA(d_qf.ensure(size_t(nq) * pitch));
	RX_CUDA(d_tau.ensure(nq));
	RX_CUDA(d_qcodes.ensure(size_t(nq) * pitch));
	RX_CUDA(d_qc.ensure(nq));
	RX_CUDA(d_kab.ensure(nqblocks));
	RX_CUDA(d_thr.ensure(std::max<size_t>(size_t(nq) * nblocks, 1)));
	RX_CUDA(cudaMemcpyAsync(d_q.p, queries, size_t(nq) * dim * 4, cudaMemcpyHostToDevice, st));
	RX_CUDA(cudaMemcpyAsync(d_tau.p, tau, size_t(nq) * 4, cudaMemcpyHostToDevice, st));
	tc_prepare_queries<<<(nq * 32 + 255) / 256, 256, 0, st>>>(d_q.p, nq, nq, dim, pitch, d_qcodes.p, d_qc.p, d_qf.p);
	tc_audit_thresholds<<<nqblocks, 256, 0, st>>>(d_qc.p, d_tau.p, nq, query_block, dim, ix->metric, ix->d_blockc, nblocks, d_kab.p, d_thr.p);
	if (row_bound && slots) {
		RX_CUDA(d_rcodes.ensure(size_t(slots) * pitch));
		RX_CUDA(d_bound.ensure(size_t(nq) * slots));
		RX_CUDA(cudaMemcpyAsync(d_rcodes.p, codes.data(), size_t(slots) * pitch, cudaMemcpyHostToDevice, st));
		tc_audit_bounds<<<dim3((slots + 255) / 256, nq), 256, 0, st>>>(reinterpret_cast<const signed char*>(d_qcodes.p), d_qc.p, d_rcodes.p,
																		ix->d_rowc, pitch, slots, dim, ix->metric, d_bound.p);
	}
	RX_CUDA(cudaGetLastError());
	RX_CUDA(cudaStreamSynchronize(st));
	if (query_codes) {
		std::vector<signed char> qcodes(size_t(nq) * pitch);
		RX_CUDA(fetch(qcodes.data(), d_qcodes.p, qcodes.size()));
		for (uint32_t q = 0; q < nq; ++q) {
			std::memcpy(query_codes + size_t(q) * dim, &qcodes[size_t(q) * pitch], dim);
		}
	}
	RX_CUDA(fetch(qc, d_qc.p, size_t(nq) * sizeof(float4)));
	RX_CUDA(fetch(kab, d_kab.p, size_t(nqblocks) * sizeof(float2)));
	RX_CUDA(fetch(block_thr, d_thr.p, size_t(nq) * nblocks * 4));
	if (row_bound && slots) {
		RX_CUDA(fetch(row_bound, d_bound.p, size_t(nq) * slots * sizeof(float2)));
	}
	return 0;
}
int rxgpu_set_profile(int on) {
	g_profile.store(on ? 1 : 0);
	return 0;
}
void rxgpu_last_search_stats(rxgpu_search_stats* out) {
	if (out) {
		*out = g_stats;
	}
}

int rxgpu_search_knn_device(const rxgpu_index* ix, uint32_t nq, const float* d_queries, uint32_t k1, float* d_out_dist,
							uint32_t* d_out_idx, uint64_t* d_out_label, uint32_t* d_out_count, void* stream) {
	if (int rc = checkIndex(ix)) {
		return rc;
	}
	g_stats = rxgpu_search_stats{};
	if (nq == 0) {
		return 0;
	}
	if (k1 == 0 || k1 > kMaxSearchK1) {
		return fail(RXGPU_ERR_PARAMS, "rxgpu: k must be in [1, 65535]");
	}
	WsLease lease(ix);
	Workspace& ws = *lease.ws;
	cudaStream_t st = stream ? static_cast<cudaStream_t>(stream) : ix->stream;
	lease.st = st;
	if (ix->size == 0) {
		RX_CUDA(cudaMemsetAsync(d_out_count, 0, nq * sizeof(uint32_t), st));
		RX_CUDA(cudaStreamSynchronize(st));
		return 0;
	}
	if (int rc = scanTopK(ix, ws, st, d_queries, nq, k1, kModeTopK, 0.f, d_out_dist, d_out_idx, d_out_label, d_out_count)) {
		return rc;
	}
	RX_CUDA(cudaStreamSynchronize(st));
	collectProfile();
	return 0;
}

int rxgpu_search_tie_rows_device(const rxgpu_index* ix, const float* d_query, float dstar, uint32_t k, float* d_out_dist,
								 uint32_t* d_out_idx, uint64_t* d_out_label, uint32_t* d_out_count, void* stream) {
	if (int rc = checkIndex(ix)) {
		return rc;
	}
	if (k == 0 || k > kMaxSearchK1) {
		return fail(RXGPU_ERR_PARAMS, "rxgpu: k must be in [1, 65535]");
	}
	WsLease lease(ix);
	cudaStream_t st = stream ? static_cast<cudaStream_t>(stream) : ix->stream;
	lease.st = st;
	if (ix->size == 0) {
		RX_CUDA(cudaMemsetAsync(d_out_count, 0, sizeof(uint32_t), st));
		RX_CUDA(cudaStreamSynchronize(st));
		return 0;
	}
	if (int rc = scanTopK(ix, *lease.ws, st, d_query, 1, k, kModeTieRows, dstar, d_out_dist, d_out_idx, d_out_label, d_out_count)) {
		return rc;
	}
// ... 583 lines not shown
```

### reindexer_b200/csrc/internal.h

```cpp
#pragma once
#include <cuda_runtime.h>

#include <algorithm>
#include <atomic>
#include <functional>
#include <memory>
#include <mutex>
#include <string>
#include <utility>
#include <vector>

#include "../../include/rxgpu.h"
#include "../host/flat_map.h"

namespace rxgpu {

extern thread_local std::string g_err;
extern thread_local rxgpu_search_stats g_stats;
extern thread_local std::vector<std::pair<cudaEvent_t, cudaEvent_t>> g_prof_events;
extern std::atomic<int> g_profile;

inline void collectProfile() {
	for (auto& ev : g_prof_events) {
		float ms = 0.f;
		if (cudaEventElapsedTime(&ms, ev.first, ev.second) == cudaSuccess) {
			g_stats.scan_kernel_ms += ms;
			g_stats.scan_launches += 1;
		}
		cudaEventDestroy(ev.first);
		cudaEventDestroy(ev.second);
	}
	g_prof_events.clear();
}

inline int fail(int code, std::string msg) {
	g_err = std::move(msg);
	return code;
}

#define RX_CUDA(expr)                                                                                        \
	do {                                                                                                     \
		cudaError_t e_ = (expr);                                                                             \
		if (e_ != cudaSuccess) {                                                                             \
			return fail(RXGPU_ERR_SYSTEM, std::string("CUDA error: ") + cudaGetErrorString(e_) + " at " #expr); \
		}                                                                                                    \
	} while (0)

template <typename T>
struct DevBuf {
	T* p = nullptr;
	size_t n = 0;
	~DevBuf() { release(); }
	void release() {
		if (p) {
			cudaFree(p);
			p = nullptr;
			n = 0;
		}
	}
	cudaError_t ensure(size_t want) {
		if (want <= n) {
			return cudaSuccess;
		}
		release();
		cudaError_t e = cudaMalloc(reinterpret_cast<void**>(&p), want * sizeof(T));
		if (e == cudaSuccess) {
			n = want;
		}
		return e;
	}
};
template <typename T>
struct PinBuf {
	T* p = nullptr;
	size_t n = 0;
	~PinBuf() {
		if (p) {
			cudaFreeHost(p);
		}
	}
	cudaError_t ensure(size_t want) {
		if (want <= n) {
			return cudaSuccess;
		}
		if (p) {
			cudaFreeHost(p);
			p = nullptr;
			n = 0;
		}
		cudaError_t e = cudaMallocHost(reinterpret_cast<void**>(&p), want * sizeof(T));
		if (e == cudaSuccess) {
			n = want;
		}
		return e;
	}
};

constexpr int kScanSmemBudget = 100 * 1024;
inline cudaError_t raiseSmemCeilingOnceImpl(const void* fn, int device, int bytes) {
	static std::mutex mtx;
	static std::vector<std::pair<const void*, int>> done;
	std::lock_guard<std::mutex> lck(mtx);
	for (const auto& d : done) {
		if (d.first == fn && d.second == device) {
			return cudaSuccess;
		}
	}
	const cudaError_t e = cudaFuncSetAttribute(fn, cudaFuncAttributeMaxDynamicSharedMemorySize, bytes);
	if (e == cudaSuccess) {
		done.emplace_back(fn, device);
	}
	return e;
}
template <typename Kernel>
inline cudaError_t raiseSmemCeilingOnce(Kernel kfn, int device, int bytes) {
	return raiseSmemCeilingOnceImpl(reinterpret_cast<const void*>(kfn), device, bytes);
}

struct Workspace {
	cudaStream_t stream = nullptr;
	DevBuf<float> d_queries;
	DevBuf<uint64_t> d_lists;
	DevBuf<uint64_t> d_floor;
	DevBuf<float> d_out_dist;
	DevBuf<uint32_t> d_out_idx;
	DevBuf<uint64_t> d_out_label;
	DevBuf<uint32_t> d_out_count;
	DevBuf<uint64_t> d_range;
	DevBuf<unsigned long long> d_range_count;
	DevBuf<float> d_radius;
	DevBuf<unsigned int> d_range_n;
	PinBuf<unsigned int> h_range_n;
	DevBuf<unsigned char> d_qcodes;
	DevBuf<float4> d_qc;
	DevBuf<float> d_qf;
	DevBuf<unsigned int> d_tau, d_cand_count, d_ub_lock;
	DevBuf<float> d_ub_list;
	DevBuf<uint32_t> d_cand_rows;
	PinBuf<unsigned int> h_cand_count;
	DevBuf<unsigned int> d_stage_status;
	PinBuf<unsigned int> h_stage_status;
	DevBuf<unsigned long long> d_reranked;
	PinBuf<unsigned long long> h_reranked;
	PinBuf<float> h_queries;
	PinBuf<float> h_out_dist;
	PinBuf<uint32_t> h_out_idx;
	PinBuf<uint64_t> h_out_label;
	PinBuf<uint32_t> h_out_count;
	PinBuf<uint64_t> h_range;
	bool tc_lists_valid = false;
	uint32_t tc_lists_nq = 0;
	uint32_t tc_lists_cap = 0;
	uint64_t tc_lists_version = 0;
	DevBuf<uint32_t> d_sel;
	DevBuf<float> d_selbound;
	DevBuf<float> d_tie_dist;
	DevBuf<uint32_t> d_tie_idx, d_tie_count;
	DevBuf<uint64_t> d_tie_label;
	~Workspace() {
		if (stream) {
			cudaStreamDestroy(stream);
		}
	}
};

}

struct rxgpu_hnsw_device;
struct rxgpu_ivf_device;
struct rxgpu_sq8_device;
namespace rxgpu {
void hnswRelease(rxgpu_hnsw_device*);
void ivfRelease(rxgpu_ivf_device*);
void sq8Release(rxgpu_sq8_device*);
}

struct rxgpu_index {
	int metric = 0;
	uint32_t dim = 0;
	uint32_t pitch = 0;
	uint64_t capacity = 0;
	uint64_t size = 0;
	int device = 0;
	uint32_t flags = 0;
	int sm_count = 132;
	uint32_t qt_override = 0;
	uint64_t version = 0;

	float* d_rows = nullptr;
	uint64_t* d_labels = nullptr;
	float* d_norms = nullptr;

	std::vector<uint64_t> h_labels;
	rxgpu::LabelMap dict;
	std::vector<float> h_rows;

	cudaStream_t stream = nullptr;
	rxgpu::DevBuf<float> st_rows;
	rxgpu::DevBuf<uint32_t> st_dst;
	rxgpu::DevBuf<uint64_t> st_labels;
	mutable std::mutex ws_mtx;
	mutable std::vector<std::unique_ptr<rxgpu::Workspace>> ws_free;
	rxgpu_hnsw_device* hnsw = nullptr;
	rxgpu_ivf_device* ivf = nullptr;
	rxgpu_sq8_device* sq8 = nullptr;

	mutable std::mutex tc_mtx;
	mutable void* d_shadow = nullptr;
	mutable float4* d_rowc = nullptr;
	mutable uint32_t* d_slot_row = nullptr;
	mutable uint32_t* d_row_slot = nullptr;
	mutable float4* d_blockc = nullptr;
	mutable uint32_t pitch_q = 0;
	mutable uint64_t shadow_slot_cap = 0;
	mutable uint32_t shadow_slots = 0;
	mutable uint32_t shadow_rows = 0;
	mutable uint32_t shadow_unsorted = 0;
	mutable uint32_t shadow_dead = 0;
	mutable uint64_t shadow_version = ~0ull;
	static constexpr size_t kShadowLogMax = 4096;
	mutable std::vector<std::pair<uint32_t, uint32_t>> shadow_dirty;
	mutable bool shadow_dirty_all = true;
	uint64_t rows_touched_from = ~0ull;
	void touchRows(uint64_t begin, uint64_t end) {
		std::lock_guard<std::mutex> lck(tc_mtx);
		if (begin < end) {
			rows_touched_from = std::min(rows_touched_from, begin);
		}
		if (!d_shadow || shadow_dirty_all || begin >= end) {
			return;
		}
		if (!shadow_dirty.empty() && shadow_dirty.back().second == begin) {
			shadow_dirty.back().second = uint32_t(end);
		} else if (shadow_dirty.size() < kShadowLogMax) {
			shadow_dirty.emplace_back(uint32_t(begin), uint32_t(end));
		} else {
			shadow_dirty_all = true;
			shadow_dirty.clear();
		}
	}
	uint32_t tc_mode = 0;
	uint32_t tc_cluster_max = 0;

	~rxgpu_index() {
		cudaSetDevice(device);
		ws_free.clear();
		if (hnsw) {
			rxgpu::hnswRelease(hnsw);
		}
		if (ivf) {
			rxgpu::ivfRelease(ivf);
		}
		if (sq8) {
			rxgpu::sq8Release(sq8);
		}
		if (d_rows) {
			cudaFree(d_rows);
		}
		if (d_labels) {
			cudaFree(d_labels);
		}
		if (d_norms) {
			cudaFree(d_norms);
		}
		if (d_shadow) {
			cudaFree(d_shadow);
		}
		cudaFree(d_rowc);
		cudaFree(d_slot_row);
		cudaFree(d_row_slot);
		cudaFree(d_blockc);
		if (stream) {
			cudaStreamDestroy(stream);
		}
	}
};

namespace rxgpu {

struct WsLease {
	const rxgpu_index* idx;
	std::unique_ptr<Workspace> ws;
	cudaStream_t st = nullptr;
	explicit WsLease(const rxgpu_index* i) : idx(i) {
		{
			std::lock_guard<std::mutex> lck(idx->ws_mtx);
			if (!idx->ws_free.empty()) {
				ws = std::move(idx->ws_free.back());
				idx->ws_free.pop_back();
			}
		}
		if (!ws) {
			ws = std::make_unique<Workspace>();
		}
	}
	~WsLease() {
		if (st) {
			cudaStreamSynchronize(st);
		}
		std::lock_guard<std::mutex> lck(idx->ws_mtx);
		idx->ws_free.emplace_back(std::move(ws));
	}
};

int scanTopK(const rxgpu_index* ix, Workspace& ws, cudaStream_t st, const float* d_queries, uint32_t nq, uint32_t k1, int mode, float bound,
			 float* d_out_dist, uint32_t* d_out_idx, uint64_t* d_out_label, uint32_t* d_out_count);
int tieRowsAfterScan(const rxgpu_index* ix, Workspace& ws, cudaStream_t st, const float* d_queries, uint32_t nsel, const uint32_t* sel,
					 const float* dstar, uint32_t k, float* d_out_dist, uint32_t* d_out_idx, uint64_t* d_out_label, uint32_t* d_out_count);

struct Hit;
using RangeEmit = std::function<void(uint32_t q, const std::vector<Hit>& hits)>;
int rangeBatch(const rxgpu_index* ix, Workspace& ws, cudaStream_t st, const float* d_queries, uint32_t nq, const float* radius,
			   uint64_t max_out, const RangeEmit& emit);

struct ScanArgs;
struct MergeArgs;
cudaError_t launchScan(const rxgpu_index* ix, int qt, const ScanArgs& a, unsigned* gridOut, cudaStream_t st, bool dryRun = false,
					   bool keysOut = false);
cudaError_t launchMergeLists(const MergeArgs& m, uint32_t nq, cudaStream_t st);
cudaError_t launchNormCoefs(const float* rows, uint32_t pitch, uint32_t dim, uint32_t row_begin, uint32_t row_end, float* coefs, cudaStream_t st);
cudaError_t scatterRows(const float* staged, const uint32_t* dst, const uint64_t* staged_labels, uint32_t n, uint32_t dim, uint32_t pitch,
						float* rows, uint64_t* labels, float* norms, cudaStream_t st);
int scanRangeHits(const rxgpu_index* ix, cudaStream_t st, ScanArgs a, DevBuf<uint64_t>& d_keys, DevBuf<unsigned long long>& d_count,
				  PinBuf<uint64_t>& h_keys, const uint64_t* h_labels, std::vector<Hit>& res, uint32_t& scans);

struct IvfCentroids {
	const float* centroids;
	const float* cnorm;
	uint32_t nlist;
	bool own;
};
int ivfCentroids(const rxgpu_index* ix, IvfCentroids& out);
int ivfCheckCoarseDim(uint32_t dim);
cudaError_t ivfAssignRows(const rxgpu_index* ix, const float* centroids, const float* cnorm, uint32_t nlist, const float* x, uint32_t n,
						  uint64_t* keys, cudaStream_t st);
constexpr uint32_t kIvfMaxCentroids = 1u << 17;

int setRowAt(rxgpu_index* ix, uint32_t idx, uint64_t label, const float* vec);

inline int checkIndex(const rxgpu_index* ix) {
	if (!ix) {
		return fail(RXGPU_ERR_PARAMS, "rxgpu: null index handle");
	}
	RX_CUDA(cudaSetDevice(ix->device));
	return 0;
}

enum class CommOp { SumU64, SumU32, MaxU32 };
int commRank(const rxgpu_comm*);
int commSize(const rxgpu_comm*);
int commDevice(const rxgpu_comm*);
std::mutex& commMutex(rxgpu_comm*);
int commAllReduce(rxgpu_comm*, void* d_buf, size_t count, CommOp op, cudaStream_t st);
int commAllGather(rxgpu_comm*, const void* d_send, void* d_recv, size_t bytes, cudaStream_t st);

}
```

### reindexer_b200/csrc/knn_tc.cuh

```cuda
#pragma once
#include <cuda.h>

#include <type_traits>

#include "common.cuh"
#include "knn_scan.cuh"

namespace rxgpu {

constexpr int kTcThreads = 512;
constexpr int kTcConsumers = 3;
constexpr int kTcTileRows = 128;
constexpr int kTcChunkK = 128;
constexpr int kTcStages = 12;
constexpr int kTcStagesMin = 8;
constexpr int kTcBlockBytes = 64 * kTcChunkK;
constexpr uint32_t kTcMaxNq = 128;
constexpr uint32_t kTcMaxK1 = 128;
constexpr float kTcL2Eps = 1e-5f;

struct TcArgs {
	const unsigned char* shadow;
	const float4* rowc;
	const uint32_t* slot_row;
	const float4* blockc;
	const float4* qc;
	unsigned int* tau;
	float* ub_list;
	unsigned int* ub_lock;
	uint32_t init_rows;
	const float* rows;
	const float* norm_coefs;
	const float* qf;
	uint32_t pitch;
	uint32_t* cand_rows;
	unsigned int* cand_count;
	uint32_t cand_cap;
	uint32_t n;
	uint32_t dim;
	uint32_t kchunks;
	uint32_t nq_total;
	uint32_t q0;
	uint32_t groups;
	uint32_t k1;
	int metric;
	uint32_t queue_slots;
	uint32_t stages;
	unsigned long long* diag;
};

constexpr int kTcDiagStamps = 1;
constexpr int kTcDiagNoRare = 2;
constexpr int kTcDiagNoFetch = 3;
constexpr int kTcDiagNoTest = 4;
constexpr uint32_t kTcDiagSlots = 64;
constexpr uint32_t kTcDiagWalk = 8192;
constexpr uint32_t kTcDiagMarkEvery = 64;
enum : uint32_t {
	kTcDgFull,
	kTcDgMma,
	kTcDgDrain,
	kTcDgBar1,
	kTcDgTest,
	kTcDgAppend,
	kTcDgTurn,
	kTcDgBar2,
	kTcDgTile,
	kTcDgBlocks,
	kTcDgHits,
	kTcDgQueueWait,
	kTcDgPerWg,
	kTcDgEmpty = kTcConsumers * kTcDgPerWg,
	kTcDgProd = kTcDgEmpty + 1,
	kTcDgRescored = kTcDgProd + 1,
	kTcDgInserts,
	kTcDgRescoreCycles,
};
static_assert(kTcDgRescoreCycles < kTcDiagSlots, "diagnostic counters fit their slots");

__host__ __device__ inline size_t tc_smem_bytes(uint32_t nq_block, uint32_t kchunks, uint32_t stages = kTcStages) {
	return 1024  + size_t(nq_block) * kchunks * 128 + size_t(stages) * kTcBlockBytes + 256  +
		   size_t(nq_block) * (16  + kTcConsumers * (4 + 4) ) + 64;
}

__device__ __forceinline__ uint32_t smem_u32(const void* p) { return uint32_t(__cvta_generic_to_shared(p)); }
__device__ __forceinline__ void mbar_init(uint64_t* bar, uint32_t count) {
	asm volatile("mbarrier.init.shared::cta.b64 [%0], %1;" ::"r"(smem_u32(bar)), "r"(count));
}
__device__ __forceinline__ void mbar_expect_tx(uint64_t* bar, uint32_t bytes) {
	asm volatile("mbarrier.arrive.expect_tx.shared::cta.b64 _, [%0], %1;" ::"r"(smem_u32(bar)), "r"(bytes) : "memory");
}
__device__ __forceinline__ void mbar_arrive(uint64_t* bar) {
	asm volatile("mbarrier.arrive.shared::cta.b64 _, [%0];" ::"r"(smem_u32(bar)) : "memory");
}
__device__ __forceinline__ void mbar_wait(uint64_t* bar, uint32_t parity) {
	asm volatile(
		"{\n"
		".reg .pred p;\n"
		"WAIT_%=:\n"
		"mbarrier.try_wait.parity.shared::cta.b64 p, [%0], %1;\n"
		"@p bra DONE_%=;\n"
		"bra WAIT_%=;\n"
		"DONE_%=:\n"
		"}\n" ::"r"(smem_u32(bar)),
		"r"(parity)
		: "memory");
}
__device__ __forceinline__ void mbar_arrive_cluster(uint64_t* bar, uint32_t cta) {
	uint32_t remote;
	asm volatile("mapa.shared::cluster.u32 %0, %1, %2;" : "=r"(remote) : "r"(smem_u32(bar)), "r"(cta));
	asm volatile("mbarrier.arrive.shared::cluster.b64 _, [%0];" ::"r"(remote) : "memory");
}
__device__ __forceinline__ void tma_load_2d(void* dst, const CUtensorMap* map, uint64_t* bar, int32_t x, int32_t y) {
	asm volatile("cp.async.bulk.tensor.2d.shared::cluster.global.tile.mbarrier::complete_tx::bytes [%0], [%1, {%3, %4}], [%2];" ::"r"(
					 smem_u32(dst)),
				 "l"(map), "r"(smem_u32(bar)), "r"(x), "r"(y)
				 : "memory");
}
__device__ __forceinline__ void bulk_load(void* dst, const void* src, uint32_t bytes, uint64_t* bar) {
	asm volatile("cp.async.bulk.shared::cluster.global.mbarrier::complete_tx::bytes [%0], [%1], %2, [%3];" ::"r"(smem_u32(dst)), "l"(src),
				 "r"(bytes), "r"(smem_u32(bar))
				 : "memory");
}
__device__ __forceinline__ void bulk_load_mc(void* dst, const void* src, uint32_t bytes, uint64_t* bar, uint16_t mask) {
	asm volatile("cp.async.bulk.shared::cluster.global.mbarrier::complete_tx::bytes.multicast::cluster [%0], [%1], %2, [%3], %4;" ::"r"(
					 smem_u32(dst)),
				 "l"(src), "r"(bytes), "r"(smem_u32(bar)), "h"(mask)
				 : "memory");
}
__device__ __forceinline__ bool elect_one_sync() {
	uint32_t p;
	asm volatile(
		"{\n"
		".reg .pred P;\n"
		"elect.sync _|P, 0xffffffff;\n"
		"selp.u32 %0, 1, 0, P;\n"
		"}\n"
		: "=r"(p));
	return p != 0;
}
__device__ __forceinline__ uint32_t cluster_ctarank() {
	uint32_t r;
	asm volatile("mov.u32 %0, %%cluster_ctarank;" : "=r"(r));
	return r;
}
__device__ __forceinline__ void cluster_sync_all() {
	asm volatile("barrier.cluster.arrive.release.aligned;" ::: "memory");
	asm volatile("barrier.cluster.wait.acquire.aligned;" ::: "memory");
}
__device__ __forceinline__ uint64_t wgmma_desc_sw128(uint32_t smem_addr) {
	uint64_t d = 0;
	d |= uint64_t((smem_addr & 0x3FFFFu) >> 4);
	d |= uint64_t(1) << 16;
	d |= uint64_t(1024 >> 4) << 32;
	d |= uint64_t(1) << 62;
	return d;
}
__device__ __forceinline__ void wgmma_fence() { asm volatile("wgmma.fence.sync.aligned;" ::: "memory"); }
__device__ __forceinline__ void wgmma_commit() { asm volatile("wgmma.commit_group.sync.aligned;" ::: "memory"); }
template <int N>
__device__ __forceinline__ void wgmma_wait() {
	asm volatile("wgmma.wait_group.sync.aligned %0;" ::"n"(N) : "memory");
}
__device__ __forceinline__ void wgmma_m64n32k32(int (&d)[16], uint64_t adesc, uint64_t bdesc, uint32_t accumulate) {
	asm volatile(
		"{\n"
		".reg .pred p;\n"
		"setp.ne.b32 p, %18, 0;\n"
		"wgmma.mma_async.sync.aligned.m64n32k32.s32.s8.s8 "
		"{%0,%1,%2,%3,%4,%5,%6,%7,%8,%9,%10,%11,%12,%13,%14,%15}, "
		"%16, %17, p;\n"
		"}\n"
		: "+r"(d[0]), "+r"(d[1]), "+r"(d[2]), "+r"(d[3]), "+r"(d[4]), "+r"(d[5]), "+r"(d[6]), "+r"(d[7]), "+r"(d[8]), "+r"(d[9]), "+r"(d[10]), "+r"(d[11]),
		  "+r"(d[12]), "+r"(d[13]), "+r"(d[14]), "+r"(d[15])
		: "l"(adesc), "l"(bdesc), "r"(accumulate));
}
__device__ __forceinline__ void wgmma_m64n64k32(int (&d)[32], uint64_t adesc, uint64_t bdesc, uint32_t accumulate) {
	asm volatile(
		"{\n"
		".reg .pred p;\n"
		"setp.ne.b32 p, %34, 0;\n"
		"wgmma.mma_async.sync.aligned.m64n64k32.s32.s8.s8 "
		"{%0,%1,%2,%3,%4,%5,%6,%7,%8,%9,%10,%11,%12,%13,%14,%15,"
		"%16,%17,%18,%19,%20,%21,%22,%23,%24,%25,%26,%27,%28,%29,%30,%31}, "
		"%32, %33, p;\n"
		"}\n"
		: "+r"(d[0]), "+r"(d[1]), "+r"(d[2]), "+r"(d[3]), "+r"(d[4]), "+r"(d[5]), "+r"(d[6]), "+r"(d[7]), "+r"(d[8]), "+r"(d[9]), "+r"(d[10]), "+r"(d[11]),
		  "+r"(d[12]), "+r"(d[13]), "+r"(d[14]), "+r"(d[15]), "+r"(d[16]), "+r"(d[17]), "+r"(d[18]), "+r"(d[19]), "+r"(d[20]), "+r"(d[21]), "+r"(d[22]), "+r"(d[23]),
		  "+r"(d[24]), "+r"(d[25]), "+r"(d[26]), "+r"(d[27]), "+r"(d[28]), "+r"(d[29]), "+r"(d[30]), "+r"(d[31])
		: "l"(adesc), "l"(bdesc), "r"(accumulate));
}
__device__ __forceinline__ void wgmma_m64n96k32(int (&d)[48], uint64_t adesc, uint64_t bdesc, uint32_t accumulate) {
	asm volatile(
		"{\n"
		".reg .pred p;\n"
		"setp.ne.b32 p, %50, 0;\n"
		"wgmma.mma_async.sync.aligned.m64n96k32.s32.s8.s8 "
		"{%0,%1,%2,%3,%4,%5,%6,%7,%8,%9,%10,%11,%12,%13,%14,%15,"
		"%16,%17,%18,%19,%20,%21,%22,%23,%24,%25,%26,%27,%28,%29,%30,%31,"
		"%32,%33,%34,%35,%36,%37,%38,%39,%40,%41,%42,%43,%44,%45,%46,%47}, "
		"%48, %49, p;\n"
		"}\n"
		: "+r"(d[0]), "+r"(d[1]), "+r"(d[2]), "+r"(d[3]), "+r"(d[4]), "+r"(d[5]), "+r"(d[6]), "+r"(d[7]), "+r"(d[8]), "+r"(d[9]), "+r"(d[10]), "+r"(d[11]),
		  "+r"(d[12]), "+r"(d[13]), "+r"(d[14]), "+r"(d[15]), "+r"(d[16]), "+r"(d[17]), "+r"(d[18]), "+r"(d[19]), "+r"(d[20]), "+r"(d[21]), "+r"(d[22]), "+r"(d[23]),
		  "+r"(d[24]), "+r"(d[25]), "+r"(d[26]), "+r"(d[27]), "+r"(d[28]), "+r"(d[29]), "+r"(d[30]), "+r"(d[31]), "+r"(d[32]), "+r"(d[33]), "+r"(d[34]), "+r"(d[35]),
		  "+r"(d[36]), "+r"(d[37]), "+r"(d[38]), "+r"(d[39]), "+r"(d[40]), "+r"(d[41]), "+r"(d[42]), "+r"(d[43]), "+r"(d[44]), "+r"(d[45]), "+r"(d[46]), "+r"(d[47])
		: "l"(adesc), "l"(bdesc), "r"(accumulate));
}
__device__ __forceinline__ void wgmma_m64n128k32(int (&d)[64], uint64_t adesc, uint64_t bdesc, uint32_t accumulate) {
	asm volatile(
		"{\n"
		".reg .pred p;\n"
		"setp.ne.b32 p, %66, 0;\n"
		"wgmma.mma_async.sync.aligned.m64n128k32.s32.s8.s8 "
		"{%0,%1,%2,%3,%4,%5,%6,%7,%8,%9,%10,%11,%12,%13,%14,%15,"
		"%16,%17,%18,%19,%20,%21,%22,%23,%24,%25,%26,%27,%28,%29,%30,%31,"
		"%32,%33,%34,%35,%36,%37,%38,%39,%40,%41,%42,%43,%44,%45,%46,%47,"
		"%48,%49,%50,%51,%52,%53,%54,%55,%56,%57,%58,%59,%60,%61,%62,%63}, "
		"%64, %65, p;\n"
		"}\n"
		: "+r"(d[0]), "+r"(d[1]), "+r"(d[2]), "+r"(d[3]), "+r"(d[4]), "+r"(d[5]), "+r"(d[6]), "+r"(d[7]), "+r"(d[8]), "+r"(d[9]), "+r"(d[10]), "+r"(d[11]),
		  "+r"(d[12]), "+r"(d[13]), "+r"(d[14]), "+r"(d[15]), "+r"(d[16]), "+r"(d[17]), "+r"(d[18]), "+r"(d[19]), "+r"(d[20]), "+r"(d[21]), "+r"(d[22]), "+r"(d[23]),
		  "+r"(d[24]), "+r"(d[25]), "+r"(d[26]), "+r"(d[27]), "+r"(d[28]), "+r"(d[29]), "+r"(d[30]), "+r"(d[31]), "+r"(d[32]), "+r"(d[33]), "+r"(d[34]), "+r"(d[35]),
		  "+r"(d[36]), "+r"(d[37]), "+r"(d[38]), "+r"(d[39]), "+r"(d[40]), "+r"(d[41]), "+r"(d[42]), "+r"(d[43]), "+r"(d[44]), "+r"(d[45]), "+r"(d[46]), "+r"(d[47]),
		  "+r"(d[48]), "+r"(d[49]), "+r"(d[50]), "+r"(d[51]), "+r"(d[52]), "+r"(d[53]), "+r"(d[54]), "+r"(d[55]), "+r"(d[56]), "+r"(d[57]), "+r"(d[58]), "+r"(d[59]),
		  "+r"(d[60]), "+r"(d[61]), "+r"(d[62]), "+r"(d[63])
		: "l"(adesc), "l"(bdesc), "r"(accumulate));
}
template <int N>
__device__ __forceinline__ void wgmma_s8(int (&d)[N / 2], uint64_t adesc, uint64_t bdesc, uint32_t accumulate) {
	if constexpr (N == 32) {
		wgmma_m64n32k32(d, adesc, bdesc, accumulate);
	} else if constexpr (N == 64) {
		wgmma_m64n64k32(d, adesc, bdesc, accumulate);
	} else if constexpr (N == 96) {
		wgmma_m64n96k32(d, adesc, bdesc, accumulate);
	} else {
		static_assert(N == 128, "query block of 32, 64, 96 or 128");
		wgmma_m64n128k32(d, adesc, bdesc, accumulate);
	}
}

__host__ __device__ __forceinline__ float tc_l2eps(uint32_t dim) { return kTcL2Eps + float(dim + 1) * 0x1p-23f; }
constexpr uint32_t kTcDeadSlot = 0xFFFFFFFFu;
constexpr int kTcPassAll = -(1 << 30), kTcPassNone = 1 << 30;
__device__ __forceinline__ int tc_block_threshold(float R, float P, float Z, float ka, float kb, float4 b0, float4 b1) {
	if (b1.z != 0.f) {
		return b1.z > 0.f ? kTcPassAll : kTcPassNone;
	}
	const float m = P * fmaf(ka, b0.z, kb * b0.w);
	const float t = fminf(-R * b0.x, -R * b0.y) - m + Z * b1.x;
	if (t == INFINITY) {
		return kTcPassNone;
	}
	const float mag = fmaf(fabsf(R), b0.y, fmaf(Z, b1.y, m));
	const float f = t - fmaf(mag, 0x1p-18f, 1.f);
	if (!(f >= -0x1p30f)) {
		return kTcPassAll;
	}
	return f > 0x1p30f ? kTcPassNone : int(floorf(f));
}
__device__ __forceinline__ void tc_block_ab_add(float* s_ab, float4 qc, float delta) {
	if (qc.z > 0.f) {
		atomicMax(reinterpret_cast<unsigned int*>(&s_ab[0]), __float_as_uint((qc.z + qc.y) / qc.z));
		atomicMax(reinterpret_cast<unsigned int*>(&s_ab[1]), __float_as_uint(qc.y / qc.z + delta));
	}
}
__device__ __forceinline__ float2 tc_block_ab_k(const float* s_ab) {
	return make_float2((1.f + 0x1p-7f) * s_ab[0], (1.f + 0x1p-7f) * s_ab[1]);
}
__device__ __forceinline__ float2 tc_make_pr(int metric, float tau, float4 qc, float l2eps) {
	const float p = qc.z * qc.w;
	if (metric != kL2) {
		return make_float2(p, tau * qc.w);
	}
	return make_float2(p, 0.5f * (tau - (1.f - l2eps) * qc.z * qc.z) * qc.w);
}

struct TcQueue {
	uint32_t tail;
	uint32_t head;
	uint32_t done;
	uint32_t full_waits;
};
constexpr uint32_t kTcQueueMax = 512;
constexpr uint32_t kTcQueueMin = 128;
__host__ __device__ inline size_t tc_queue_bytes(uint32_t slots) {
	return kTcConsumers * sizeof(TcQueue) + size_t(kTcConsumers) * slots * 16;
}
inline uint32_t tc_ring_stages(uint32_t nq_block, uint32_t kchunks, size_t limit) {
	for (uint32_t s = kTcStages; s >= uint32_t(kTcStagesMin); --s) {
		if (tc_smem_bytes(nq_block, kchunks, s) + tc_queue_bytes(kTcQueueMin) <= limit) {
			return s;
		}
	}
	return 0;
}
inline uint32_t tc_queue_slots(uint32_t nq_block, uint32_t kchunks, uint32_t stages, size_t limit) {
	for (uint32_t s = kTcQueueMax; s >= kTcQueueMin; s /= 2) {
		if (tc_smem_bytes(nq_block, kchunks, stages) + tc_queue_bytes(s) <= limit) {
			return s;
		}
	}
	return 0;
}

__device__ __forceinline__ uint32_t ld_acquire_shared(const uint32_t* p) {
	uint32_t v;
	asm volatile("ld.acquire.cta.shared::cta.u32 %0, [%1];" : "=r"(v) : "r"(smem_u32(p)) : "memory");
	return v;
}
__device__ __forceinline__ void st_release_shared(uint32_t* p, uint32_t v) {
	asm volatile("st.release.cta.shared::cta.u32 [%0], %1;" ::"r"(smem_u32(p)), "r"(v) : "memory");
}

__device__ __forceinline__ bool tc_enqueue(TcQueue* qu, uint4* rec, uint32_t slots, uint32_t q, uint32_t slot, float x) {
	const uint32_t t = atomicAdd(&qu->tail, 1u);
	bool waited = false;
	while (t - ld_acquire_shared(&qu->head) >= slots) {
		waited = true;
		__nanosleep(64);
	}
	uint4* r = rec + (t & (slots - 1));
	r->x = q;
	r->y = slot;
	r->z = __float_as_uint(x);
	st_release_shared(&r->w, t + 1);
	return waited;
}

__device__ __noinline__ bool tc_enqueue_quad(TcQueue* qu, uint4* rec, uint32_t slots, uint32_t h, uint32_t q, uint32_t slot0, uint32_t slot1,
											 float x0, float x1, float x2, float x3) {
	bool waited = false;
	if (h & 1u) waited |= tc_enqueue(qu, rec, slots, q, slot0, x0);
	if (h & 2u) waited |= tc_enqueue(qu, rec, slots, q + 1, slot0, x1);
	if (h & 4u) waited |= tc_enqueue(qu, rec, slots, q, slot1, x2);
	if (h & 8u) waited |= tc_enqueue(qu, rec, slots, q + 1, slot1, x3);
	return waited;
}

constexpr float kTcTinyNorm = 0x1p-48f, kTcTinyNorm2 = 0x1p-96f;
__device__ __forceinline__ float2 tc_row_bound(const TcArgs& a, float x, float4 qc, float4 rc) {
	const float p = qc.x * rc.x * x;
	const float e = (1.f + 0x1p-8f) * fmaf(qc.z + qc.y, rc.y, (qc.y + float(a.dim + 16) * 0x1p-23f * qc.z) * rc.z);
	if (a.metric == kL2) {
		const float nn = qc.z * qc.z + rc.z * rc.z;
		return make_float2(fmaf(-2.f, p, fmaf(qc.z, qc.z, rc.z * rc.z)), nn < kTcTinyNorm2 ? INFINITY : 2.f * e + tc_l2eps(a.dim) * nn);
	}
	const float err = qc.z * rc.z < kTcTinyNorm2 ? INFINITY : e;
	if (a.metric == kCos) {
		return make_float2(-p * rc.w, err * rc.w);
	}
	return make_float2(-p, err);
}

__device__ __noinline__ float tc_bound_insert(const TcArgs& a, uint32_t q, float ub) {
	while (atomicCAS(&a.ub_lock[q], 0u, 1u) != 0u) {
	}
	__threadfence();
	volatile float* list = a.ub_list + size_t(q) * kTcMaxK1;
	uint32_t mi = 0;
	float mx = list[0];
	for (uint32_t x = 1; x < a.k1; ++x) {
		const float y = list[x];
		if (y > mx) {
			mx = y;
			mi = x;
		}
	}
	float tightened = mx;
	if (ub < mx) {
		list[mi] = ub;
		float nmx = list[0];
		for (uint32_t x = 1; x < a.k1; ++x) {
			nmx = fmaxf(nmx, list[x]);
		}
		atomicMin(&a.tau[q], float_ord(nmx));
		tightened = nmx;
	}
	__threadfence();
	atomicExch(&a.ub_lock[q], 0u);
	return tightened;
}

constexpr int kTcRescoreRows = 4;
template <bool kIsL2>
__device__ __noinline__ float tc_rescore(const TcArgs& a, unsigned todo, uint32_t row, uint32_t ql, uint32_t q0, int lane) {
	const uint32_t nch = a.kchunks, pitch4 = a.pitch >> 2;
	const float4* rows4 = reinterpret_cast<const float4*>(a.rows);
	float mine = 0.f;
	while (todo) {
		uint32_t rr[kTcRescoreRows];
		const float4* qp[kTcRescoreRows][1];
		int who[kTcRescoreRows];
#pragma unroll
		for (int i = 0; i < kTcRescoreRows; ++i) {
			who[i] = todo ? __ffs(todo) - 1 : who[0];
			todo &= todo - 1u;
			rr[i] = __shfl_sync(0xffffffffu, row, who[i]);
			qp[i][0] = reinterpret_cast<const float4*>(a.qf) + size_t(q0 + __shfl_sync(0xffffffffu, ql, who[i])) * nch * 32u;
		}
		float d[kTcRescoreRows][1];
		row_dists_warp<kIsL2, kTcRescoreRows, 1>(rows4, pitch4, nch, rr, qp, a.norm_coefs, lane, d);
#pragma unroll
		for (int i = 0; i < kTcRescoreRows; ++i) {
			mine = lane == who[i] ? d[i][0] : mine;
		}
	}
	return mine;
}

template <int kNq>
__device__ __forceinline__ float tc_min_thr(const float* s_thr, uint32_t ql) {
	float t = s_thr[ql];
#pragma unroll
	for (int w = 1; w < kTcConsumers; ++w) {
		t = fminf(t, s_thr[w * kNq + ql]);
	}
	return t;
}
template <int kNq, int kDiag>
__device__ __forceinline__ void tc_bookkeeper(const TcArgs& a, TcQueue* qu, const uint4* rec, uint32_t slots, uint32_t q0, const float4* s_qc,
											  float* s_thr, int lane, unsigned long long* dg) {
	[[maybe_unused]] unsigned long long n_rescored = 0, n_inserts = 0;
	[[maybe_unused]] long long rescore_cycles = 0;
	uint32_t head = 0;
	for (;;) {
		const bool fin = ld_acquire_shared(&qu->done) == 4;
		const uint32_t n = __shfl_sync(0xffffffffu, min(ld_acquire_shared(&qu->tail) - head, 32u), 0);
		if (n == 0) {
			if (__shfl_sync(0xffffffffu, fin, 0)) {
				break;
			}
			__nanosleep(256);
			continue;
		}
		bool active = uint32_t(lane) < n;
		uint32_t ql = 0, slot = 0;
		float x = 0.f;
		if (active) {
			const uint32_t t = head + lane;
			const uint4* r = rec + (t & (slots - 1));
			while (ld_acquire_shared(&r->w) != t + 1) {
			}
			ql = r->x;
			slot = r->y;
			x = __uint_as_float(r->z);
		}
		__syncwarp();
		head += n;
		if (lane == 0) {
			st_release_shared(&qu->head, head);
		}
		const uint32_t row = active ? a.slot_row[slot] : kTcDeadSlot;
		active = active && row != kTcDeadSlot;
		float d = 0.f, err = 0.f, tau = 0.f;
		if (active) {
			const float4 qc = s_qc[ql], rc = a.rowc[slot];
			const float2 de = tc_row_bound(a, x, qc, rc);
			d = de.x;
			err = de.y;
			tau = tc_min_thr<kNq>(s_thr, ql);
		}
		const bool append = active && !(d - err > tau);
		const unsigned peers = __match_any_sync(0xffffffffu, append ? ql : ~0u);
		const int leader = __ffs(peers) - 1;
		unsigned base = 0;
		if (append && lane == leader) {
			base = atomicAdd(&a.cand_count[q0 + ql], unsigned(__popc(peers)));
		}
		base = __shfl_sync(0xffffffffu, base, leader);
		if (append) {
			const unsigned pos = base + __popc(peers & ((1u << lane) - 1u));
			if (pos < a.cand_cap) {
				a.cand_rows[size_t(q0 + ql) * a.cand_cap + pos] = row;
			}
		}
		const bool rescore = append && row >= a.init_rows && d < tau;
		const unsigned todo = __ballot_sync(0xffffffffu, rescore);
		if (todo) {
			[[maybe_unused]] const long long c0 = kDiag == kTcDiagStamps ? clock64() : 0ll;
			const float dx = a.metric == kL2 ? tc_rescore<true>(a, todo, row, ql, q0, lane) : tc_rescore<false>(a, todo, row, ql, q0, lane);
			if constexpr (kDiag != 0) {
				n_rescored += __popc(todo);
				if constexpr (kDiag == kTcDiagStamps) {
					rescore_cycles += clock64() - c0;
				}
			}
			if (rescore && dx < tc_min_thr<kNq>(s_thr, ql)) {
				if constexpr (kDiag != 0) {
					++n_inserts;
				}
				const float nt = tc_bound_insert(a, q0 + ql, dx);
				for (uint32_t w = 0; w < kTcConsumers; ++w) {
					if (nt < s_thr[w * kNq + ql]) {
						s_thr[w * kNq + ql] = nt;
					}
				}
			}
		}
		__syncwarp();
	}
	if constexpr (kDiag != 0) {
		const unsigned long long ins = __reduce_add_sync(0xffffffffu, uint32_t(n_inserts));
		if (lane == 0) {
			atomicAdd(&dg[kTcDgRescored], n_rescored);
			atomicAdd(&dg[kTcDgInserts], ins);
			atomicAdd(&dg[kTcDgRescoreCycles], (unsigned long long)rescore_cycles);
		}
	}
}

template <int kNq, int kCluster, int kDiag = 0>
__global__ void __launch_bounds__(kTcThreads, 1)
	knn_tc_filter(const __grid_constant__ CUtensorMap map_queries, const __grid_constant__ TcArgs a) {
	static_assert(kNq % 32 == 0 && kNq <= int(kTcMaxNq), "query block");
	static_assert(kCluster == 1 || kCluster == 2 || kCluster == 4, "a stage is split in 1, 2 or 4 equal copies");
	constexpr bool kStamp = kDiag == kTcDiagStamps;
	auto clk = [] {
		if constexpr (kStamp) {
			return clock64();
		} else {
			return 0ll;
		}
	};
	unsigned long long* dg = kDiag ? a.diag + size_t(blockIdx.x) * kTcDiagSlots : nullptr;
	extern __shared__ unsigned char smem_raw[];
	unsigned char* base = smem_raw + ((1024u - (smem_u32(smem_raw) & 1023u)) & 1023u);
	constexpr uint32_t kQchunkBytes = kNq * 128;
	unsigned char* s_q = base;
	unsigned char* s_rows = s_q + size_t(a.kchunks) * kQchunkBytes;
	const uint32_t nstages = a.stages;
	uint64_t* bars = reinterpret_cast<uint64_t*>(s_rows + size_t(nstages) * kTcBlockBytes);
	uint64_t* full_bar = bars;
	uint64_t* empty_bar = bars + kTcStages;
	uint64_t* q_bar = bars + 2 * kTcStages;
	float* s_ab = reinterpret_cast<float*>(q_bar + 1);
	float4* s_qc = reinterpret_cast<float4*>(bars + 32);
	float* s_thr = reinterpret_cast<float*>(s_qc + kNq);
	int* s_tb = reinterpret_cast<int*>(s_thr + kTcConsumers * kNq);
	TcQueue* s_queue = reinterpret_cast<TcQueue*>(s_tb + kTcConsumers * kNq);
	uint4* s_rec = reinterpret_cast<uint4*>(s_queue + kTcConsumers);
	static_assert(2 * kTcStages + 2 <= 32, "barriers and (a*, b*) fit in front of the per-query constants");

	const int warp = __shfl_sync(0xffffffffu, int(threadIdx.x >> 5), 0), lane = threadIdx.x & 31;
	const uint32_t ntiles = (a.n + kTcTileRows - 1) / kTcTileRows;
	const uint32_t crank = kCluster > 1 ? cluster_ctarank() : 0u;
	const uint32_t cid = blockIdx.x / kCluster, ncl = gridDim.x / kCluster;
	const uint32_t walker = cid / a.groups, walkers = ncl / a.groups;
	const uint32_t q0 = a.q0 + ((cid % a.groups) * kCluster + crank) * kNq;
	const uint32_t nq_valid = q0 < a.nq_total ? min(uint32_t(kNq), a.nq_total - q0) : 0u;
	const float l2eps = tc_l2eps(a.dim);

	if (threadIdx.x == 0) {
		for (uint32_t s = 0; s < nstages; ++s) {
			mbar_init(&full_bar[s], 1);
			mbar_init(&empty_bar[s], 4 * kCluster);
		}
		mbar_init(q_bar, 1);
		asm volatile("fence.mbarrier_init.release.cluster;" ::: "memory");
		s_ab[0] = s_ab[1] = 0.f;
		for (int w = 0; w < kTcConsumers; ++w) {
			s_queue[w] = TcQueue{0u, 0u, 0u, 0u};
		}
	}
	for (uint32_t i = threadIdx.x; i < kTcConsumers * a.queue_slots; i += blockDim.x) {
		s_rec[i].w = 0u;
	}
	if constexpr (kDiag == kTcDiagNoFetch) {
		for (uint32_t i = threadIdx.x; i < nstages * kTcBlockBytes / 16; i += blockDim.x) {
			reinterpret_cast<uint4*>(s_rows)[i] = make_uint4(0u, 0u, 0u, 0u);
		}
		asm volatile("fence.proxy.async.shared::cta;" ::: "memory");
	}
	__syncthreads();
	const float delta = float(a.dim + 16) * 0x1p-23f;
	for (uint32_t i = threadIdx.x; i < kNq; i += blockDim.x) {
		const bool valid = i < nq_valid;
		const float thr = valid ? ord_float(a.tau[q0 + i]) : -INFINITY;
		const float4 qc = valid ? a.qc[q0 + i] : make_float4(0.f, 0.f, 0.f, 0.f);
		tc_block_ab_add(s_ab, qc, delta);
		s_qc[i] = qc;
		for (int w = 0; w < kTcConsumers; ++w) {
			s_thr[w * kNq + i] = thr;
			s_tb[w * kNq + i] = kTcPassNone;
		}
	}
	__syncthreads();
	if constexpr (kCluster > 1) {
		cluster_sync_all();
	}
	const uint32_t nblocks = walker < ntiles ? 2 * ((ntiles - walker + walkers - 1) / walkers) : 0u;

	if (warp == 0) {
		if (elect_one_sync()) {
			mbar_expect_tx(q_bar, a.kchunks * kQchunkBytes);
			for (uint32_t kc = 0; kc < a.kchunks; ++kc) {
				tma_load_2d(s_q + size_t(kc) * kQchunkBytes, &map_queries, q_bar, int32_t(kc * kTcChunkK), int32_t(q0));
			}
		}
		__syncwarp();
		uint64_t* full = full_bar;
		uint64_t* empty = empty_bar;
		unsigned char* ring_smem = s_rows;
		uint32_t stage = 0, phase = 0;
		[[maybe_unused]] long long t_empty = 0;
		[[maybe_unused]] const long long t_start = clk();
		for (uint32_t i = 0; i < nblocks; ++i) {
			const unsigned char* src = a.shadow + size_t(2 * (walker + (i >> 1) * walkers) + (i & 1u)) * a.kchunks * kTcBlockBytes;
			for (uint32_t kc = 0; kc < a.kchunks; ++kc) {
				[[maybe_unused]] const long long c0 = clk();
				mbar_wait(&empty[stage], phase ^ 1);
				if constexpr (kStamp) {
					t_empty += clk() - c0;
				}
				unsigned char* dst = ring_smem + size_t(stage) * kTcBlockBytes;
				if constexpr (kDiag == kTcDiagNoFetch) {
					if (elect_one_sync()) {
						mbar_arrive(&full[stage]);
					}
				} else if (elect_one_sync()) {
					mbar_expect_tx(&full[stage], kTcBlockBytes);
					if constexpr (kCluster == 1) {
						bulk_load(dst, src + size_t(kc) * kTcBlockBytes, kTcBlockBytes, &full[stage]);
					} else {
						constexpr uint32_t kPart = kTcBlockBytes / kCluster;
						bulk_load_mc(dst + crank * kPart, src + size_t(kc) * kTcBlockBytes + crank * kPart, kPart, &full[stage],
									 uint16_t((1u << kCluster) - 1u));
					}
				}
				__syncwarp();
				if (++stage == nstages) {
					stage = 0;
					phase ^= 1;
				}
			}
		}
		if constexpr (kStamp) {
			if (lane == 0) {
				atomicAdd(&dg[kTcDgEmpty], (unsigned long long)t_empty);
				atomicAdd(&dg[kTcDgProd], (unsigned long long)(clk() - t_start));
			}
		}
	} else if (warp < 4) {
		const uint32_t wg = uint32_t(warp) - 1;
		tc_bookkeeper<kNq, kDiag>(a, s_queue + wg, s_rec + wg * a.queue_slots, a.queue_slots, q0, s_qc, s_thr, lane, dg);
	} else {
		const uint32_t wg = uint32_t(warp) / 4 - 1, wtid = threadIdx.x - 128 * (wg + 1);
		float* thr = s_thr + wg * kNq;
		int* tb = s_tb + wg * kNq;
		TcQueue* qu = s_queue + wg;
		uint4* rec = s_rec + wg * a.queue_slots;
		const uint32_t slots = a.queue_slots;
		uint64_t* full = full_bar;
		uint64_t* empty = empty_bar;
		const unsigned char* ring_smem = s_rows;
		const uint32_t r0 = (wtid >> 5) * 16 + (lane >> 2), c2 = 2 * (lane & 3);
		const uint32_t my_q = wtid;
		unsigned int tau_ahead = my_q < nq_valid ? a.tau[q0 + my_q] : 0u;
		const bool l2 = a.metric == kL2;
		const float2 kab = tc_block_ab_k(s_ab);
		const float ka = kab.x, kb = kab.y;
		auto release = [&](uint32_t st) {
			if constexpr (kCluster == 1) {
				if (lane == 0) {
					mbar_arrive(&empty[st]);
				}
			} else if (lane < kCluster) {
				mbar_arrive_cluster(&empty[st], uint32_t(lane));
			}
		};
		mbar_wait(q_bar, 0);
		[[maybe_unused]] long long dt[kTcDgPerWg] = {};
		[[maybe_unused]] unsigned long long nhits = 0;
		[[maybe_unused]] uint32_t sink = 0;
		for (uint32_t blk = wg; blk < nblocks; blk += kTcConsumers) {
			const uint32_t t = walker + (blk >> 1) * walkers, half = blk & 1u;
			[[maybe_unused]] const uint32_t walk = blk >> 1;
			[[maybe_unused]] long long s0 = clk(), s1, s2, s3, s4, s5;
			if constexpr (kStamp) {
				if (half == 0 && wtid == 0 && walk % kTcDiagMarkEvery == 0 && walk < kTcDiagWalk) {
					unsigned long long now;
					asm volatile("mov.u64 %0, %%globaltimer;" : "=l"(now));
					a.diag[size_t(gridDim.x) * kTcDiagSlots + kTcDiagWalk + size_t(blockIdx.x) * (kTcDiagWalk / kTcDiagMarkEvery) +
						   walk / kTcDiagMarkEvery] = now;
				}
			}
			if (my_q < nq_valid) {
				const float tn = ord_float(tau_ahead);
				if (tn < thr[my_q]) {
					thr[my_q] = tn;
				}
				tau_ahead = a.tau[q0 + my_q];
			}
			const uint32_t sb = 2 * t + half, slot0 = sb * 64 + r0, slot1 = slot0 + 8;
			float4 bc0 = {}, bc1 = {};
			if (my_q < nq_valid) {
				bc0 = a.blockc[2 * sb];
				bc1 = a.blockc[2 * sb + 1];
			}
			int acc[kNq / 2];
#pragma unroll
			for (int i = 0; i < kNq / 2; ++i) {
				acc[i] = 0;
			}
			const uint32_t g0 = blk * a.kchunks;
			uint32_t stage = g0 % nstages, phase = (g0 / nstages) & 1u;
			[[maybe_unused]] const long long c_turn = clk();
			if (blk != 0) {
				asm volatile("bar.sync %0, 256;" ::"r"(4 + wg) : "memory");
			}
			if constexpr (kStamp) {
				dt[kTcDgTurn] += clk() - c_turn;
			}
			uint32_t prev = 0;
			for (uint32_t kc = 0; kc < a.kchunks; ++kc) {
				[[maybe_unused]] const long long c0 = clk();
				mbar_wait(&full[stage], phase);
				if constexpr (kStamp) {
					dt[kTcDgFull] += clk() - c0;
				}
				const uint32_t a_addr = smem_u32(ring_smem + size_t(stage) * kTcBlockBytes);
				const uint32_t b_addr = smem_u32(s_q + size_t(kc) * kQchunkBytes);
				wgmma_fence();
#pragma unroll
				for (uint32_t k = 0; k < kTcChunkK / 32; ++k) {
					wgmma_s8<kNq>(acc, wgmma_desc_sw128(a_addr + k * 32), wgmma_desc_sw128(b_addr + k * 32), (kc | k) != 0);
				}
				wgmma_commit();
				if (kc > 0) {
					wgmma_wait<1>();
					release(prev);
				}
				prev = stage;
				if (++stage == nstages) {
					stage = 0;
					phase ^= 1;
				}
			}
			if (blk + 1 < nblocks) {
				asm volatile("bar.arrive %0, 256;" ::"r"(4 + (wg + 1) % kTcConsumers) : "memory");
			}
			s1 = clk();
			wgmma_wait<0>();
			release(prev);
			if (my_q < nq_valid) {
				const float4 qc = s_qc[my_q];
				const float2 pr = tc_make_pr(a.metric, thr[my_q], qc, l2eps);
				tb[my_q] = tc_block_threshold(pr.y, pr.x, l2 ? qc.w : 0.f, ka, kb, bc0, bc1);
			}
			s2 = clk();
			asm volatile("bar.sync %0, 128;" ::"r"(1 + wg) : "memory");
			s3 = clk();
			const uint32_t ok = (slot0 < a.n ? 0x33333333u : 0u) | (slot1 < a.n ? 0xCCCCCCCCu : 0u);
			constexpr int kMaskWords = (kNq / 2 + 31) / 32;
			uint32_t hm[kMaskWords] = {};
			if constexpr (kDiag == kTcDiagNoTest) {
#pragma unroll
				for (int i = 0; i < kNq / 2; ++i) {
					sink ^= uint32_t(acc[i]);
				}
			} else {
#pragma unroll
				for (int j = 0; j < kNq / 8; ++j) {
					const int2 t2 = *reinterpret_cast<const int2*>(&tb[8 * j + c2]);
					const bool h0 = acc[4 * j] >= t2.x, h1 = acc[4 * j + 1] >= t2.y;
					const bool h2 = acc[4 * j + 2] >= t2.x, h3 = acc[4 * j + 3] >= t2.y;
					hm[4 * j / 32] |= (uint32_t(h0) | uint32_t(h1) << 1 | uint32_t(h2) << 2 | uint32_t(h3) << 3) << (4 * j % 32);
				}
			}
#pragma unroll
			for (int w = 0; w < kMaskWords; ++w) {
				hm[w] &= ok;
			}
			s4 = clk();
			[[maybe_unused]] uint32_t nh = 0;
#pragma unroll
			for (int w = 0; w < kMaskWords; ++w) {
				nh += __popc(hm[w]);
			}
			if constexpr (kDiag != 0) {
				nhits += nh;
			}
			if constexpr (kDiag != kTcDiagNoRare && kDiag != kTcDiagNoTest) {
				if (__any_sync(0xffffffffu, nh != 0)) {
#pragma unroll
					for (int j = 0; j < kNq / 8; ++j) {
						const uint32_t h = hm[4 * j / 32] >> (4 * j % 32) & 15u;
						if (h) {
							const bool waited = tc_enqueue_quad(qu, rec, slots, h, 8 * j + c2, slot0, slot1, float(acc[4 * j]), float(acc[4 * j + 1]),
																float(acc[4 * j + 2]), float(acc[4 * j + 3]));
							if constexpr (kStamp) {
								if (waited) {
									atomicAdd(&qu->full_waits, 1u);
								}
							}
						}
					}
				}
			}
			__syncwarp();
			s5 = clk();
			asm volatile("bar.sync %0, 128;" ::"r"(1 + wg) : "memory");
			if constexpr (kStamp) {
				const long long s6 = clk();
				dt[kTcDgMma] += s1 - s0;
				dt[kTcDgDrain] += s2 - s1;
				dt[kTcDgBar1] += s3 - s2;
				dt[kTcDgTest] += s4 - s3;
				dt[kTcDgAppend] += s5 - s4;
				dt[kTcDgBar2] += s6 - s5;
				dt[kTcDgTile] += s6 - s0;
				dt[kTcDgBlocks] += 1;
				const uint32_t h = __reduce_add_sync(0xffffffffu, nh);
				if (lane == 0 && h && walk < kTcDiagWalk) {
					atomicAdd(&a.diag[size_t(gridDim.x) * kTcDiagSlots + walk], (unsigned long long)h);
				}
			}
		}
		__syncwarp();
		if (lane == 0) {
			__threadfence_block();
			atomicAdd(&qu->done, 1u);
		}
		if constexpr (kDiag != 0) {
			const uint32_t h = __reduce_add_sync(0xffffffffu, uint32_t(nhits));
			const uint32_t x = __reduce_xor_sync(0xffffffffu, sink);
			if (lane == 0) {
				atomicAdd(&dg[wg * kTcDgPerWg + kTcDgHits], (unsigned long long)h);
				if constexpr (kDiag == kTcDiagNoTest) {
					atomicXor(&dg[wg * kTcDgPerWg + kTcDgTurn], (unsigned long long)x);
				}
				if constexpr (kStamp) {
					dt[kTcDgMma] -= dt[kTcDgFull] + dt[kTcDgTurn];
					for (uint32_t i = 0; i < kTcDgPerWg; ++i) {
						if (i != kTcDgHits) {
							atomicAdd(&dg[wg * kTcDgPerWg + i], (unsigned long long)dt[i]);
						}
					}
				}
			}
		}
	}
	__syncthreads();
	if constexpr (kStamp) {
		if (threadIdx.x < kTcConsumers) {
			dg[threadIdx.x * kTcDgPerWg + kTcDgQueueWait] = s_queue[threadIdx.x].full_waits;
		}
	}
	if constexpr (kCluster > 1) {
		cluster_sync_all();
	}
}

template <bool kIsL2>
__global__ void __launch_bounds__(kScanThreads) knn_rerank(const float* rows, uint32_t pitch, uint32_t dim, const float* norm_coefs,
															const float* queries, const uint32_t* cand_rows, const unsigned int* cand_count,
															uint32_t cand_cap, uint32_t k1, uint64_t* lists ,
															const uint32_t* qsel = nullptr, const float* tie_bound = nullptr,
															const float* radius = nullptr, uint64_t* range_keys = nullptr,
															unsigned int* range_count = nullptr) {
	extern __shared__ __align__(16) unsigned char smem_raw[];
	const int lane = threadIdx.x & 31, warp = threadIdx.x >> 5;
	const uint32_t q = qsel ? qsel[blockIdx.x] : blockIdx.x;
	const bool tie = tie_bound != nullptr;
	const bool range = radius != nullptr;
	const float rad = range ? radius[q] : 0.f;
	const float bound = tie ? tie_bound[blockIdx.x] : 0.f;
	const uint32_t nch = (dim + 127u) / 128u, dp4 = nch * 32u, pitch4 = pitch >> 2;
	const uint32_t m = k1 + kCandBuf;
	float4* sq4 = reinterpret_cast<float4*>(smem_raw);
	uint64_t* skeys = reinterpret_cast<uint64_t*>(smem_raw + size_t(dp4) * 16);
	{
		float* sq = reinterpret_cast<float*>(sq4);
		for (uint32_t i = threadIdx.x; i < dp4 * 4; i += blockDim.x) {
			sq[i] = i < dim ? queries[size_t(q) * dim + i] : 0.f;
		}
		for (uint32_t i = threadIdx.x; i < kScanWarps * m; i += blockDim.x) {
			skeys[i] = kKeyNone;
		}
	}
	__syncthreads();
	uint64_t* wkeys = skeys + size_t(warp) * m;
	uint64_t thr = kKeyNone;
	uint32_t cnt = 0;
	const uint32_t ncand = min(cand_count[q], cand_cap);
	const float4* rows4 = reinterpret_cast<const float4*>(rows);
	const uint32_t* my = cand_rows + size_t(q) * cand_cap;
	for (uint32_t i = warp; i < ncand; i += kScanWarps) {
		const uint32_t row = my[i];
		const float dist = row_dist_warp<kIsL2>(rows4, pitch4, nch, row, sq4, norm_coefs, lane);
		if (range) {
			if (lane == 0 && dist < rad) {
				range_keys[size_t(q) * cand_cap + atomicAdd(&range_count[q], 1u)] = make_key(dist, row);
			}
			continue;
		}
		const uint64_t key = !tie ? make_key(dist, row) : (dist <= bound ? ((uint64_t(row) << 32) | float_ord(dist)) : kKeyNone);
		if (key < thr) {
			if (lane == 0) {
				wkeys[k1 + cnt] = key;
			}
			++cnt;
			__syncwarp();
			if (cnt == kCandBuf) {
				warp_select(wkeys, k1 + cnt, k1, lane);
				thr = wkeys[k1 - 1];
				cnt = 0;
			}
		}
	}
	if (range) {
		return;
	}
	if (cnt) {
		warp_select(wkeys, k1 + cnt, k1, lane);
	}
	__syncthreads();
	if (warp == 0) {
		uint64_t last = 0;
		bool first = true;
		for (uint32_t r = 0; r < k1; ++r) {
			uint64_t best = kKeyNone;
			for (uint32_t i = lane; i < kScanWarps * k1; i += 32) {
				const uint32_t w = i / k1, j = i - w * k1;
				const uint64_t kx = skeys[size_t(w) * m + j];
				if ((first || kx > last) && kx < best) {
					best = kx;
				}
			}
#pragma unroll
			for (int off = 16; off > 0; off >>= 1) {
				const uint64_t ok = __shfl_xor_sync(0xffffffffu, best, off);
				best = ok < best ? ok : best;
			}
			if (lane == 0) {
				lists[size_t(blockIdx.x) * k1 + r] = best;
			}
			last = best;
			first = false;
		}
	}
}

constexpr uint32_t kTcStagedMaxK1 = 1024;
constexpr int kSelThreads = 512;
constexpr uint32_t kSelSort = 4096;

__global__ void knn_seed_tau(const float* seed_dist, const uint32_t* seed_count, uint32_t k1, uint32_t nq, unsigned int* tau, float* radius,
							 unsigned int* status) {
	const uint32_t q = blockIdx.x * blockDim.x + threadIdx.x;
	if (q >= nq) {
		return;
	}
	const float t = seed_count[q] >= k1 ? seed_dist[size_t(q) * k1 + k1 - 1] : NAN;
	const bool ok = isfinite(t);
	tau[q] = float_ord(ok ? t : -INFINITY);
	radius[q] = ok ? nextafterf(t, INFINITY) : -INFINITY;
	status[q] = ok ? 0u : 1u;
}

struct SelectArgs {
	const uint64_t* keys;
	const unsigned int* nkeys;
	const unsigned int* cand_count;
	const uint32_t* qsel;
	const uint64_t* labels;
	uint32_t cap;
	uint32_t k1;
	int mode;
	int last;
	unsigned int* tau;
	float* radius;
	unsigned int* status;
	unsigned long long* reranked;
	float* out_dist;
	uint32_t* out_idx;
	uint64_t* out_label;
	uint32_t* out_count;
	bool neg_zero;
};

__global__ void __launch_bounds__(kSelThreads) knn_select_topk(const SelectArgs a) {
	__shared__ uint64_t s_keys[kSelSort];
	__shared__ uint32_t s_hist[256];
	__shared__ uint64_t s_prefix, s_bound;
	__shared__ uint32_t s_below, s_n;
	const uint32_t b = blockIdx.x, q = a.qsel ? a.qsel[b] : b;
	const bool tie = a.mode == kModeTieRows;
	const int lane = threadIdx.x & 31;
	if (!tie) {
		if (threadIdx.x == 0) {
			atomicAdd(a.reranked, (unsigned long long)min(a.cand_count[q], a.cap));
		}
		if (a.status[q]) {
			if (threadIdx.x == 0) {
				a.tau[q] = float_ord(-INFINITY);
// ... 130 lines not shown
		const float v = p[c];
		mx = fmaxf(mx, fabsf(v));
		ss = fma(double(v), double(v), ss);
	}
	for (int off = 16; off > 0; off >>= 1) {
		mx = fmaxf(mx, __shfl_xor_sync(0xffffffffu, mx, off));
		ss += __shfl_xor_sync(0xffffffffu, ss, off);
	}
	const float s = mx / 127.f;
	double rr = 0.0;
	for (uint32_t c = 4 * lane; c < padded; c += 128) {
		uint32_t code4 = 0;
#pragma unroll
		for (uint32_t i = 0; i < 4; ++i) {
			const float v = c + i < dim ? p[c + i] : 0.f;
			const float code = s > 0.f ? fminf(fmaxf(rintf(v / s), -127.f), 127.f) : 0.f;
			const double rho = double(v) - double(s) * double(code);
			rr = fma(rho, rho, rr);
			code4 |= (uint32_t(int(code)) & 0xFFu) << (8 * i);
		}
		put(c, code4);
	}
	for (int off = 16; off > 0; off >>= 1) {
		rr += __shfl_xor_sync(0xffffffffu, rr, off);
	}
	return make_float3(s, __double2float_ru(sqrt(rr) * (1.0 + 0x1p-40)), __double2float_ru(sqrt(ss) * (1.0 + 0x1p-40)));
}

__global__ void tc_convert_rows(const float* rows, uint32_t pitch, uint32_t dim, uint32_t row_begin, uint32_t row_end, const uint32_t* row_slot,
								unsigned char* shadow, uint32_t kchunks, const float* norm_coefs, float4* rowc) {
	const uint32_t row = row_begin + (blockIdx.x * blockDim.x + threadIdx.x) / 32;
	const int lane = threadIdx.x & 31;
	if (row >= row_end) {
		return;
	}
	const uint32_t slot = row_slot[row], blk = slot / 64u, r = slot % 64u;
	const float3 srn = tc_quantize(rows + size_t(row) * pitch, dim, kchunks * kTcChunkK, lane, [&](uint32_t c, uint32_t code4) {
		const uint32_t kc = c / kTcChunkK, cc = c % kTcChunkK;
		const uint32_t unit = (cc >> 4) ^ (r & 7u);
		*reinterpret_cast<uint32_t*>(shadow + (size_t(blk) * kchunks + kc) * kTcBlockBytes + r * 128u + unit * 16u + (cc & 15u)) = code4;
	});
	if (lane == 0) {
		rowc[slot] = make_float4(srn.x, srn.y, srn.z, norm_coefs ? norm_coefs[row] : 1.f);
	}
}

__global__ void tc_sort_keys(const float* rows, uint32_t pitch, uint32_t dim, uint32_t n, const float* norm_coefs, int metric, uint64_t* keys,
							 uint32_t* vals) {
	const uint32_t row = (blockIdx.x * blockDim.x + threadIdx.x) / 32;
	const int lane = threadIdx.x & 31;
	if (row >= n) {
		return;
	}
	const float* p = rows + size_t(row) * pitch;
	float mx = 0.f, ss = 0.f;
	for (uint32_t c = lane; c < dim; c += 32) {
		const float v = p[c];
		mx = fmaxf(mx, fabsf(v));
		ss = fmaf(v, v, ss);
	}
	for (int off = 16; off > 0; off >>= 1) {
		mx = fmaxf(mx, __shfl_xor_sync(0xffffffffu, mx, off));
		ss += __shfl_xor_sync(0xffffffffu, ss, off);
	}
	if (lane == 0) {
		const float S = (mx / 127.f) * (norm_coefs ? norm_coefs[row] : 1.f);
		const uint64_t bucket = metric == kL2 ? float_ord(ss) >> 13 : 0u;
		keys[row] = bucket << 32 | ~float_ord(S);
		vals[row] = row;
	}
}

__global__ void tc_invert_slots(const uint32_t* slot_row, uint32_t n, uint32_t* row_slot) {
	const uint32_t s = blockIdx.x * blockDim.x + threadIdx.x;
	if (s < n) {
		row_slot[slot_row[s]] = s;
	}
}

__global__ void tc_assign_slots(uint32_t row_begin, uint32_t row_end, uint32_t slot_begin, uint32_t* slot_row, uint32_t* row_slot) {
	const uint32_t i = blockIdx.x * blockDim.x + threadIdx.x;
	if (row_begin + i < row_end) {
		slot_row[slot_begin + i] = row_begin + i;
		row_slot[row_begin + i] = slot_begin + i;
	}
}
__global__ void tc_kill_rows(uint32_t row_begin, uint32_t row_end, const uint32_t* row_slot, uint32_t* slot_row, float4* rowc) {
	const uint32_t row = row_begin + blockIdx.x * blockDim.x + threadIdx.x;
	if (row < row_end) {
		const uint32_t slot = row_slot[row];
		slot_row[slot] = kTcDeadSlot;
		rowc[slot] = make_float4(0.f, 0.f, 0.f, 0.f);
	}
}

__global__ void tc_block_consts(const float4* rowc, const uint32_t* slot_row, uint32_t nslots, uint32_t nblocks, float one_minus_eps,
								int metric, float4* blockc) {
	const uint32_t blk = (blockIdx.x * blockDim.x + threadIdx.x) / 32;
	const int lane = threadIdx.x & 31;
	if (blk >= nblocks) {
		return;
	}
	float u_lo = INFINITY, u_hi = 0.f, rho_hi = 0.f, nu_hi = 0.f, w_lo = INFINITY, w_hi = 0.f;
	bool live = false, pass_all = false;
	for (uint32_t i = 0; i < 2; ++i) {
		const uint32_t slot = blk * 64 + 2 * lane + i;
		if (slot >= nslots || slot_row[slot] == kTcDeadSlot) {
			continue;
		}
		live = true;
		const float4 rc = rowc[slot];
		const double S = double(rc.x) * double(rc.w);
		if (!(S > 0.0) || !isfinite(S) || !isfinite(rc.y) || !isfinite(rc.z) || rc.z < kTcTinyNorm) {
			pass_all = true;
			continue;
		}
		const float u0 = __double2float_rd(__ddiv_rd(1.0, S)), u1 = __double2float_ru(__ddiv_ru(1.0, S));
		const float rho = __double2float_ru(__ddiv_ru(double(rc.y), double(rc.x)));
		const float nu = __double2float_ru(__ddiv_ru(double(rc.z), double(rc.x)));
		float w0 = 0.f, w1 = 0.f;
		if (metric == kL2) {
			const double nn = double(rc.z) * double(rc.z);
			w0 = __double2float_rd(__ddiv_rd(__dmul_rd(nn, double(one_minus_eps)), 2.0 * S));
			w1 = __double2float_ru(__ddiv_ru(__dmul_ru(nn, double(one_minus_eps)), 2.0 * S));
		}
		if (!isfinite(u1) || !isfinite(rho) || !isfinite(nu) || !isfinite(w1) || u0 == 0.f) {
			pass_all = true;
			continue;
		}
		u_lo = fminf(u_lo, u0);
		u_hi = fmaxf(u_hi, u1);
		rho_hi = fmaxf(rho_hi, rho);
		nu_hi = fmaxf(nu_hi, nu);
		w_lo = fminf(w_lo, w0);
		w_hi = fmaxf(w_hi, w1);
	}
	for (int off = 16; off > 0; off >>= 1) {
		u_lo = fminf(u_lo, __shfl_xor_sync(0xffffffffu, u_lo, off));
		u_hi = fmaxf(u_hi, __shfl_xor_sync(0xffffffffu, u_hi, off));
		rho_hi = fmaxf(rho_hi, __shfl_xor_sync(0xffffffffu, rho_hi, off));
		nu_hi = fmaxf(nu_hi, __shfl_xor_sync(0xffffffffu, nu_hi, off));
		w_lo = fminf(w_lo, __shfl_xor_sync(0xffffffffu, w_lo, off));
		w_hi = fmaxf(w_hi, __shfl_xor_sync(0xffffffffu, w_hi, off));
	}
	live = __any_sync(0xffffffffu, live);
	pass_all = __any_sync(0xffffffffu, pass_all);
	if (lane == 0) {
		const float flag = pass_all ? 1.f : live ? 0.f : -1.f;
		blockc[2 * blk] = flag == 0.f ? make_float4(u_lo, u_hi, rho_hi, nu_hi) : make_float4(0.f, 0.f, 0.f, 0.f);
		blockc[2 * blk + 1] = flag == 0.f ? make_float4(w_lo, w_hi, flag, 0.f) : make_float4(0.f, 0.f, flag, 0.f);
	}
}

constexpr int kTcInitQ = 4;
constexpr uint32_t kTcInitRows = 4096;
__host__ __device__ inline size_t tc_init_smem_bytes() { return size_t(kTcInitQ) * kTcInitRows * sizeof(float); }
__global__ void __launch_bounds__(256) tc_init_tau(const float* rows, uint32_t pitch, uint32_t kchunks, const float* norm_coefs, uint32_t nrows,
												   const float* qf, uint32_t nq, uint32_t k1, int metric, unsigned int* tau, float* ub_list,
												   unsigned int* ub_lock) {
	extern __shared__ __align__(16) float s_d[];
	const uint32_t q0 = blockIdx.x * kTcInitQ;
	const uint32_t lane = threadIdx.x & 31, warp = threadIdx.x >> 5;
	const float4* rows4 = reinterpret_cast<const float4*>(rows);
	const float4* q4[kTcInitQ];
#pragma unroll
	for (int qi = 0; qi < kTcInitQ; ++qi) {
		q4[qi] = reinterpret_cast<const float4*>(qf) + size_t(q0 + qi < nq ? q0 + qi : q0) * kchunks * 32u;
	}
	constexpr uint32_t kRows = 4;
	for (uint32_t r0 = warp * kRows; r0 < kTcInitRows; r0 += 8 * kRows) {
		float dist[kRows][kTcInitQ];
		if (r0 < nrows) {
			uint32_t rr[kRows];
			const float4* qp[kRows][kTcInitQ];
#pragma unroll
			for (uint32_t x = 0; x < kRows; ++x) {
				rr[x] = min(r0 + x, nrows - 1);
#pragma unroll
				for (int qi = 0; qi < kTcInitQ; ++qi) {
					qp[x][qi] = q4[qi];
				}
			}
			if (metric == kL2) {
				row_dists_warp<true, kRows, kTcInitQ>(rows4, pitch / 4, kchunks, rr, qp, nullptr, lane, dist);
			} else {
				row_dists_warp<false, kRows, kTcInitQ>(rows4, pitch / 4, kchunks, rr, qp, norm_coefs, lane, dist);
			}
		}
#pragma unroll
		for (uint32_t x = 0; x < kRows; ++x) {
#pragma unroll
			for (int qi = 0; qi < kTcInitQ; ++qi) {
				if (lane == uint32_t(qi)) {
					const uint32_t r = r0 + x;
					s_d[qi * kTcInitRows + r] = r < nrows ? dist[x][qi] : INFINITY;
				}
			}
		}
	}
	__syncthreads();
	if (warp < kTcInitQ && q0 + warp < nq) {
		const uint32_t q = q0 + warp;
		float* d = s_d + warp * kTcInitRows;
		float last = INFINITY;
		for (uint32_t round = 0; round < kTcMaxK1; ++round) {
			float best = INFINITY;
			uint32_t at = lane;
			if (round < k1) {
				for (uint32_t j = lane; j < kTcInitRows; j += 32) {
					const float y = d[j];
					if (y < best) {
						best = y;
						at = j;
					}
				}
				for (int off = 16; off > 0; off >>= 1) {
					const float ob = __shfl_xor_sync(0xffffffffu, best, off);
					const uint32_t oa = __shfl_xor_sync(0xffffffffu, at, off);
					if (ob < best || (ob == best && oa < at)) {
						best = ob;
						at = oa;
					}
				}
				if (lane == 0) {
					d[at] = INFINITY;
				}
				__syncwarp();
				last = best;
			}
			if (lane == 0) {
				ub_list[size_t(q) * kTcMaxK1 + round] = round < k1 ? best : -INFINITY;
			}
		}
		if (lane == 0) {
			tau[q] = float_ord(last);
			ub_lock[q] = 0;
		}
	}
}

__global__ void tc_prepare_queries(const float* queries, uint32_t nq, uint32_t nq_pad, uint32_t dim, uint32_t pitch, unsigned char* codes,
								   float4* qc, float* qf) {
	const uint32_t q = (blockIdx.x * blockDim.x + threadIdx.x) / 32;
	const int lane = threadIdx.x & 31;
	if (q >= nq_pad) {
		return;
	}
	for (uint32_t c = lane; c < pitch; c += 32) {
		qf[size_t(q) * pitch + c] = q < nq && c < dim ? queries[size_t(q) * dim + c] : 0.f;
	}
	unsigned char* out = codes + size_t(q) * pitch;
	const float3 srn = tc_quantize(queries + size_t(q) * dim, q < nq ? dim : 0u, pitch, lane,
								   [&](uint32_t c, uint32_t code4) { *reinterpret_cast<uint32_t*>(out + c) = code4; });
	if (lane == 0 && q < nq) {
		qc[q] = make_float4(srn.x, srn.y, srn.z, srn.z > 0.f && srn.z < kTcTinyNorm ? INFINITY : srn.x > 0.f ? 1.f / srn.x : 1.f);
	}
}

__global__ void tc_audit_thresholds(const float4* qc, const float* tau, uint32_t nq, uint32_t nqb, uint32_t dim, int metric,
									const float4* blockc, uint32_t nblocks, float2* kab, int* thr) {
	__shared__ float s_ab[2];
	const uint32_t q0 = blockIdx.x * nqb, nv = min(nqb, nq - q0);
	if (threadIdx.x == 0) {
		s_ab[0] = s_ab[1] = 0.f;
	}
	__syncthreads();
	const float delta = float(dim + 16) * 0x1p-23f;
	for (uint32_t i = threadIdx.x; i < nv; i += blockDim.x) {
		tc_block_ab_add(s_ab, qc[q0 + i], delta);
	}
	__syncthreads();
	const float2 k = tc_block_ab_k(s_ab);
	if (threadIdx.x == 0) {
		kab[blockIdx.x] = k;
	}
	const float l2eps = tc_l2eps(dim);
	for (uint32_t i = threadIdx.x; i < nv * nblocks; i += blockDim.x) {
		const uint32_t q = q0 + i / nblocks, b = i % nblocks;
		const float4 c = qc[q];
		const float2 pr = tc_make_pr(metric, tau[q], c, l2eps);
		thr[size_t(q) * nblocks + b] = tc_block_threshold(pr.y, pr.x, metric == kL2 ? c.w : 0.f, k.x, k.y, blockc[2 * b], blockc[2 * b + 1]);
	}
}

__global__ void tc_audit_bounds(const signed char* qcodes, const float4* qc, const signed char* rcodes, const float4* rowc, uint32_t pitch,
								uint32_t nslots, uint32_t dim, int metric, float2* bound) {
	const uint32_t slot = blockIdx.x * blockDim.x + threadIdx.x, q = blockIdx.y;
	if (slot >= nslots) {
		return;
	}
	const char4* a = reinterpret_cast<const char4*>(qcodes + size_t(q) * pitch);
	const char4* b = reinterpret_cast<const char4*>(rcodes + size_t(slot) * pitch);
	int I = 0;
	for (uint32_t i = 0; i < pitch / 4; ++i) {
		const char4 x = a[i], y = b[i];
		I += int(x.x) * int(y.x) + int(x.y) * int(y.y) + int(x.z) * int(y.z) + int(x.w) * int(y.w);
	}
	TcArgs args{};
	args.dim = dim;
	args.metric = metric;
	bound[size_t(q) * nslots + slot] = tc_row_bound(args, float(I), qc[q], rowc[slot]);
}

}
```

Before: 76050.

## Defer non-promising TC candidates, drain later, and replace full rerank with bound lists

The bound list now holds exact (distance,row) keys, so the final top-k can be read from it with a small sort kernel instead of running a full per-query rerank over all candidates. Candidates that fail the current threshold are pushed to a per-block defer buffer and rescored only at the end, or when the queue is idle, if they can still beat the tightened tau. Queries whose defer buffer overflowed are flagged incomplete and reranked individually on the host loop. The tau-seeding kernel is split into row slices plus a merge kernel to parallelise seeding. This adds buffer memory, extra kernel launches, and correctness risk when defer capacity is exceeded.

```diff
diff --git a/include/rxgpu.h b/include/rxgpu.h
--- a/include/rxgpu.h
+++ b/include/rxgpu.h
@@ -321,6 +321,7 @@
 } rxgpu_search_stats;
 void rxgpu_last_search_stats(rxgpu_search_stats* out);
 int rxgpu_set_tensor_core_filter(rxgpu_index*, int mode);
+int rxgpu_set_tc_defer_cap(rxgpu_index*, uint32_t cap);
 int rxgpu_set_profile(int on);
 int rxgpu_tc_diag(int mode, void* d_counters);
 int rxgpu_tc_audit(const rxgpu_index*, uint32_t nq, const float* queries, const float* tau, uint32_t query_block, uint32_t* out_shape,
diff --git a/reindexer_b200/binding.py b/reindexer_b200/binding.py
--- a/reindexer_b200/binding.py
+++ b/reindexer_b200/binding.py
@@ -212,6 +212,7 @@
     "rxgpu_tc_audit": (C.c_int, [C.c_void_p, C.c_uint32, _f32p, _f32p, C.c_uint32, _u32p, _u32p, _f32p, _f32p, C.c_void_p, C.c_void_p, _f32p,
                                  _f32p, _i32p, _f32p]),
     "rxgpu_set_tensor_core_filter": (C.c_int, [C.c_void_p, C.c_int]),
+    "rxgpu_set_tc_defer_cap": (C.c_int, [C.c_void_p, C.c_uint32]),
 }
 
 _lib = None
@@ -632,6 +633,9 @@
 
     def set_tensor_core_filter(self, mode: int):
         _check(self._lib.rxgpu_set_tensor_core_filter(self._h, mode))
+
+    def set_tc_defer_cap(self, cap: int):
+        _check(self._lib.rxgpu_set_tc_defer_cap(self._h, cap))
 
     def tc_audit(self, queries, tau, query_block: int = 128, row_bound: bool = True) -> dict:
         q = np.ascontiguousarray(queries, dtype=np.float32).reshape(-1, self.dim)
diff --git a/reindexer_b200/csrc/index.cu b/reindexer_b200/csrc/index.cu
--- a/reindexer_b200/csrc/index.cu
+++ b/reindexer_b200/csrc/index.cu
@@ -696,6 +696,7 @@
 	return 0;
 }
 
+constexpr uint32_t kTcDeferCap = 4096;
 int tcLaunch(const rxgpu_index* ix, Workspace& ws, cudaStream_t st, const TcBatch& b, uint32_t k1, uint32_t candCap, uint32_t nrows, bool fixedTau) {
 	const uint32_t nq = b.nq, nqb = b.nqb, cluster = b.cluster, ngroups = b.ngroups, kchunks = b.kchunks, pitchQ = ix->pitch_q;
 	const uint32_t ntiles = (nrows + kTcTileRows - 1) / kTcTileRows;
@@ -703,6 +704,12 @@
 	const TcKernel kfn = b.kfn;
 	const CUtensorMap mapQ = b.mapQ;
 	RX_CUDA(cudaMemsetAsync(ws.d_cand_count.p, 0, size_t(b.nqPad) * 4, st));
+	const uint32_t deferCap = ix->tc_defer_cap ? ix->tc_defer_cap : kTcDeferCap;
+	if (!fixedTau) {
+		RX_CUDA(ws.d_defer.ensure(size_t(resident) * cluster * kTcConsumers * deferCap));
+		RX_CUDA(ws.d_incomplete.ensure(b.nqPad));
+		RX_CUDA(cudaMemsetAsync(ws.d_incomplete.p, 0, size_t(b.nqPad) * 4, st));
+	}
 	RX_CUDA(cudaGetLastError());
 	cudaLaunchConfig_t cfg{};
 	cfg.blockDim = dim3(kTcThreads);
@@ -725,6 +732,9 @@
 	a.ub_list = fixedTau ? nullptr : ws.d_ub_list.p;
 	a.ub_lock = fixedTau ? nullptr : ws.d_ub_lock.p;
 	a.init_rows = fixedTau ? UINT32_MAX : uint32_t(std::min<uint64_t>(ix->size, kTcInitRows));
+	a.defer = fixedTau ? nullptr : ws.d_defer.p;
+	a.defer_cap = deferCap;
+	a.incomplete = fixedTau ? nullptr : ws.d_incomplete.p;
 	a.rows = ix->d_rows;
 	a.norm_coefs = ix->metric == RXGPU_COS ? ix->d_norms : nullptr;
 	a.qf = ws.d_qf.p;
@@ -780,13 +790,17 @@
 	if (h_tau) {
 		RX_CUDA(cudaMemcpyAsync(ws.d_tau.p, h_tau, size_t(nq) * 4, cudaMemcpyHostToDevice, st));
 	} else {
+		const uint32_t seedRows = uint32_t(std::min<uint64_t>(ix->size, kTcInitRows));
+		const uint32_t slices = std::max<uint32_t>(1u, (seedRows + kTcInitSlice - 1) / kTcInitSlice);
 		RX_CUDA(ws.d_ub_list.ensure(size_t(b.nqPad) * kTcMaxK1));
 		RX_CUDA(ws.d_ub_lock.ensure(b.nqPad));
+		RX_CUDA(ws.d_seed.ensure(size_t(nq) * slices * k1));
 		RX_CUDA(raiseSmemCeilingOnce(tc_init_tau, ix->device, int(tc_init_smem_bytes())));
-		tc_init_tau<<<(nq + kTcInitQ - 1) / kTcInitQ, 256, tc_init_smem_bytes(), st>>>(
-			ix->d_rows, ix->pitch, b.kchunks, ix->metric == RXGPU_COS ? ix->d_norms : nullptr, uint32_t(std::min<uint64_t>(ix->size, kTcInitRows)),
-			ws.d_qf.p, nq, k1, ix->metric, ws.d_tau.p, ws.d_ub_list.p, ws.d_ub_lock.p);
-		g_stats.launches += 1;
+		tc_init_tau<<<dim3((nq + kTcInitQ - 1) / kTcInitQ, slices), 256, tc_init_smem_bytes(), st>>>(
+			ix->d_rows, ix->pitch, b.kchunks, ix->metric == RXGPU_COS ? ix->d_norms : nullptr, seedRows, ws.d_qf.p, nq, k1, ix->metric, ws.d_seed.p);
+		tc_init_tau_merge<<<(nq + 127) / 128, 128, 0, st>>>(ws.d_seed.p, nq, slices, k1, ws.d_tau.p, ws.d_ub_list.p, ws.d_ub_lock.p);
+		RX_CUDA(cudaGetLastError());
+		g_stats.launches += 2;
 	}
 	return tcLaunch(ix, ws, st, b, k1, candCap, ix->shadow_slots, h_tau != nullptr);
 }
@@ -896,17 +910,8 @@
 		return rc;
 	}
 	RX_CUDA(ws.d_lists.ensure(size_t(nq) * k1));
-	const size_t rsmem = size_t((ix->dim + 127) / 128) * 512 + size_t(kScanWarps) * (k1 + kCandBuf) * 8;
-	const float* norms = ix->metric == RXGPU_COS ? ix->d_norms : nullptr;
-	if (ix->metric == RXGPU_L2) {
-		RX_CUDA(raiseSmemCeilingOnce(knn_rerank<true>, ix->device, kScanSmemBudget));
-		knn_rerank<true><<<nq, kScanThreads, rsmem, st>>>(ix->d_rows, ix->pitch, ix->dim, norms, d_queries, ws.d_cand_rows.p,
-														   ws.d_cand_count.p, candCap, k1, ws.d_lists.p);
-	} else {
-		RX_CUDA(raiseSmemCeilingOnce(knn_rerank<false>, ix->device, kScanSmemBudget));
-		knn_rerank<false><<<nq, kScanThreads, rsmem, st>>>(ix->d_rows, ix->pitch, ix->dim, norms, d_queries, ws.d_cand_rows.p,
-															ws.d_cand_count.p, candCap, k1, ws.d_lists.p);
-	}
+	RX_CUDA(ws.h_incomplete.ensure(nq));
+	tc_sort_bound_lists<<<nq, kTcMaxK1, 0, st>>>(ws.d_ub_list.p, k1, ws.d_lists.p);
 	MergeArgs m{};
 	m.lists = ws.d_lists.p;
 	m.labels = ix->d_labels;
@@ -926,7 +931,10 @@
 	RX_CUDA(cudaGetLastError());
 	g_stats.launches += 2;
 	RX_CUDA(cudaMemcpyAsync(ws.h_cand_count.p, ws.d_cand_count.p, size_t(nq) * 4, cudaMemcpyDeviceToHost, st));
+	RX_CUDA(cudaMemcpyAsync(ws.h_incomplete.p, ws.d_incomplete.p, size_t(nq) * 4, cudaMemcpyDeviceToHost, st));
 	RX_CUDA(cudaStreamSynchronize(st));
+	const size_t rsmem = size_t((ix->dim + 127) / 128) * 512 + size_t(kScanWarps) * (k1 + kCandBuf) * 8;
+	const float* norms = ix->metric == RXGPU_COS ? ix->d_norms : nullptr;
 	uint64_t cands = 0;
 	for (uint32_t q = 0; q < nq; ++q) {
 		cands += std::min<unsigned>(ws.h_cand_count.p[q], candCap);
@@ -936,6 +944,24 @@
 									   d_out_idx + size_t(q) * k1, d_out_label ? d_out_label + size_t(q) * k1 : nullptr, d_out_count + q)) {
 				return rc;
 			}
+		} else if (ws.h_incomplete.p[q]) {
+			const float* qv = d_queries + size_t(q) * ix->dim;
+			const uint32_t* rows = ws.d_cand_rows.p + size_t(q) * candCap;
+			if (ix->metric == RXGPU_L2) {
+				RX_CUDA(raiseSmemCeilingOnce(knn_rerank<true>, ix->device, kScanSmemBudget));
+				knn_rerank<true><<<1, kScanThreads, rsmem, st>>>(ix->d_rows, ix->pitch, ix->dim, norms, qv, rows, ws.d_cand_count.p + q, candCap, k1,
+																  ws.d_lists.p);
+			} else {
+				RX_CUDA(raiseSmemCeilingOnce(knn_rerank<false>, ix->device, kScanSmemBudget));
+				knn_rerank<false><<<1, kScanThreads, rsmem, st>>>(ix->d_rows, ix->pitch, ix->dim, norms, qv, rows, ws.d_cand_count.p + q, candCap, k1,
+																   ws.d_lists.p);
+			}
+			MergeArgs one = m;
+			one.qt = 1;
+			one.q_offset = q;
+			knn_merge_lists<<<1, 256, 0, st>>>(one);
+			RX_CUDA(cudaGetLastError());
+			g_stats.launches += 2;
 		}
 	}
 	ws.tc_lists_valid = true;
@@ -1453,6 +1479,13 @@
 	ix->tc_cluster_max = mode == 3 ? 1u : mode == 4 ? 2u : mode == 5 ? 4u : 0u;
 	return 0;
 }
+int rxgpu_set_tc_defer_cap(rxgpu_index* ix, uint32_t cap) {
+	if (!ix) {
+		return fail(RXGPU_ERR_PARAMS, "rxgpu: null handle");
+	}
+	ix->tc_defer_cap = cap;
+	return 0;
+}
 int rxgpu_tc_diag(int mode, void* d_counters) {
 	if (mode < 0 || mode > kTcDiagNoTest || (mode && !d_counters)) {
 		return fail(RXGPU_ERR_PARAMS, "rxgpu: diagnostic filter mode must be 0..4, with a counter buffer");
diff --git a/reindexer_b200/csrc/internal.h b/reindexer_b200/csrc/internal.h
--- a/reindexer_b200/csrc/internal.h
+++ b/reindexer_b200/csrc/internal.h
@@ -135,7 +135,11 @@
 	DevBuf<float4> d_qc;
 	DevBuf<float> d_qf;
 	DevBuf<unsigned int> d_tau, d_cand_count, d_ub_lock;
-	DevBuf<float> d_ub_list;
+	DevBuf<uint64_t> d_ub_list;
+	DevBuf<uint64_t> d_seed;
+	DevBuf<uint4> d_defer;
+	DevBuf<unsigned int> d_incomplete;
+	PinBuf<unsigned int> h_incomplete;
 	DevBuf<uint32_t> d_cand_rows;
 	PinBuf<unsigned int> h_cand_count;
 	DevBuf<unsigned int> d_stage_status;
@@ -240,6 +244,7 @@
 		}
 	}
 	uint32_t tc_mode = 0;
+	uint32_t tc_defer_cap = 0;
 	uint32_t tc_cluster_max = 0;
 
 	~rxgpu_index() {
diff --git a/reindexer_b200/csrc/knn_tc.cuh b/reindexer_b200/csrc/knn_tc.cuh
--- a/reindexer_b200/csrc/knn_tc.cuh
+++ b/reindexer_b200/csrc/knn_tc.cuh
@@ -26,9 +26,12 @@
 	const float4* blockc;
 	const float4* qc;
 	unsigned int* tau;
-	float* ub_list;
+	uint64_t* ub_list;
 	unsigned int* ub_lock;
 	uint32_t init_rows;
+	uint4* defer;
+	uint32_t defer_cap;
+	unsigned int* incomplete;
 	const float* rows;
 	const float* norm_coefs;
 	const float* qf;
@@ -75,8 +78,13 @@
 	kTcDgRescored = kTcDgProd + 1,
 	kTcDgInserts,
 	kTcDgRescoreCycles,
+	kTcDgDeferred,
+	kTcDgDrainScored,
+	kTcDgDrainDropped,
+	kTcDgDrainPending,
+	kTcDgDrainTail,
 };
-static_assert(kTcDgRescoreCycles < kTcDiagSlots, "diagnostic counters fit their slots");
+static_assert(kTcDgDrainTail < kTcDiagSlots, "diagnostic counters fit their slots");
 
 __host__ __device__ inline size_t tc_smem_bytes(uint32_t nq_block, uint32_t kchunks, uint32_t stages = kTcStages) {
 	return 1024  + size_t(nq_block) * kchunks * 128 + size_t(stages) * kTcBlockBytes + 256  +
@@ -354,33 +362,34 @@
 	return make_float2(-p, err);
 }
 
-__device__ __noinline__ float tc_bound_insert(const TcArgs& a, uint32_t q, float ub) {
+__host__ __device__ __forceinline__ uint32_t tc_key_tau(uint64_t top) { return top == kKeyNone ? float_ord(INFINITY) : uint32_t(top >> 32); }
+
+__device__ __noinline__ float tc_bound_insert(const TcArgs& a, uint32_t q, uint64_t key) {
 	while (atomicCAS(&a.ub_lock[q], 0u, 1u) != 0u) {
 	}
 	__threadfence();
-	volatile float* list = a.ub_list + size_t(q) * kTcMaxK1;
+	volatile uint64_t* list = a.ub_list + size_t(q) * kTcMaxK1;
 	uint32_t mi = 0;
-	float mx = list[0];
+	uint64_t mx = list[0];
 	for (uint32_t x = 1; x < a.k1; ++x) {
-		const float y = list[x];
+		const uint64_t y = list[x];
 		if (y > mx) {
 			mx = y;
 			mi = x;
 		}
 	}
-	float tightened = mx;
-	if (ub < mx) {
-		list[mi] = ub;
-		float nmx = list[0];
+	if (key < mx) {
+		list[mi] = key;
+		mx = list[0];
 		for (uint32_t x = 1; x < a.k1; ++x) {
-			nmx = fmaxf(nmx, list[x]);
-		}
-		atomicMin(&a.tau[q], float_ord(nmx));
-		tightened = nmx;
+			const uint64_t y = list[x];
+			mx = y > mx ? y : mx;
+		}
+		atomicMin(&a.tau[q], tc_key_tau(mx));
 	}
 	__threadfence();
 	atomicExch(&a.ub_lock[q], 0u);
-	return tightened;
+	return ord_float(tc_key_tau(mx));
 }
 
 constexpr int kTcRescoreRows = 4;
@@ -420,16 +429,69 @@
 	return t;
 }
 template <int kNq, int kDiag>
-__device__ __forceinline__ void tc_bookkeeper(const TcArgs& a, TcQueue* qu, const uint4* rec, uint32_t slots, uint32_t q0, const float4* s_qc,
-											  float* s_thr, int lane, unsigned long long* dg) {
-	[[maybe_unused]] unsigned long long n_rescored = 0, n_inserts = 0;
+__device__ __forceinline__ void tc_score_rows(const TcArgs& a, unsigned todo, bool mine, uint32_t row, uint32_t ql, uint32_t q0, float* s_thr,
+											  int lane, unsigned long long& n_rescored, unsigned long long& n_inserts, long long& rescore_cycles) {
+	[[maybe_unused]] const long long c0 = kDiag == kTcDiagStamps ? clock64() : 0ll;
+	const float dx = a.metric == kL2 ? tc_rescore<true>(a, todo, row, ql, q0, lane) : tc_rescore<false>(a, todo, row, ql, q0, lane);
+	if constexpr (kDiag != 0) {
+		n_rescored += __popc(todo);
+		if constexpr (kDiag == kTcDiagStamps) {
+			rescore_cycles += clock64() - c0;
+		}
+	}
+	if (mine && !(dx > tc_min_thr<kNq>(s_thr, ql))) {
+		if constexpr (kDiag != 0) {
+			++n_inserts;
+		}
+		const float nt = tc_bound_insert(a, q0 + ql, make_key(dx, row));
+		for (uint32_t w = 0; w < kTcConsumers; ++w) {
+			if (nt < s_thr[w * kNq + ql]) {
+				s_thr[w * kNq + ql] = nt;
+			}
+		}
+	}
+}
+template <int kNq, int kDiag>
+__device__ __forceinline__ void tc_drain_chunk(const TcArgs& a, const uint4* e, uint32_t take, uint32_t q0, float* s_thr, int lane,
+											   unsigned long long& n_scored, unsigned long long& n_dropped, unsigned long long& n_rescored,
+											   unsigned long long& n_inserts, long long& rescore_cycles) {
+	uint32_t ql = 0, row = 0;
+	bool score = false;
+	if (uint32_t(lane) < take) {
+		const uint4 x = e[lane];
+		ql = x.x;
+		row = x.y;
+		const float thr = fminf(tc_min_thr<kNq>(s_thr, ql), ord_float(__ldcg(&a.tau[q0 + ql])));
+		score = !(__uint_as_float(x.z) > thr);
+	}
+	const unsigned todo = __ballot_sync(0xffffffffu, score);
+	if constexpr (kDiag != 0) {
+		n_scored += __popc(todo);
+		n_dropped += take - __popc(todo);
+	}
+	if (todo) {
+		tc_score_rows<kNq, kDiag>(a, todo, score, row, ql, q0, s_thr, lane, n_rescored, n_inserts, rescore_cycles);
+	}
+	__syncwarp();
+}
+template <int kNq, int kDiag>
+__device__ __forceinline__ uint32_t tc_bookkeeper(const TcArgs& a, TcQueue* qu, const uint4* rec, uint32_t slots, uint32_t q0, const float4* s_qc,
+											  float* s_thr, int lane, unsigned long long* dg, uint4* defer) {
+	[[maybe_unused]] unsigned long long n_rescored = 0, n_inserts = 0, n_deferred = 0, n_drain_scored = 0, n_drain_dropped = 0;
 	[[maybe_unused]] long long rescore_cycles = 0;
-	uint32_t head = 0;
+	uint32_t head = 0, ndef = 0;
 	for (;;) {
-		const bool fin = ld_acquire_shared(&qu->done) == 4;
+		const bool fin = __shfl_sync(0xffffffffu, ld_acquire_shared(&qu->done) == 4, 0);
 		const uint32_t n = __shfl_sync(0xffffffffu, min(ld_acquire_shared(&qu->tail) - head, 32u), 0);
+		if (n == 0 && ndef >= a.defer_cap / 2 && ndef != 0) {
+			const uint32_t take = min(ndef, 32u);
+			ndef -= take;
+			tc_drain_chunk<kNq, kDiag>(a, defer + ndef, take, q0, s_thr, lane, n_drain_scored, n_drain_dropped, n_rescored, n_inserts,
+									   rescore_cycles);
+			continue;
+		}
 		if (n == 0) {
-			if (__shfl_sync(0xffffffffu, fin, 0)) {
+			if (fin) {
 				break;
 			}
 			__nanosleep(256);
@@ -476,28 +538,27 @@
 				a.cand_rows[size_t(q0 + ql) * a.cand_cap + pos] = row;
 			}
 		}
-		const bool rescore = append && row >= a.init_rows && d < tau;
+		const bool fresh = append && row >= a.init_rows;
+		const bool rescore = fresh && d < tau;
+		const bool later = fresh && !rescore;
+		const unsigned dm = __ballot_sync(0xffffffffu, later);
+		if (dm) {
+			const uint32_t pos = ndef + __popc(dm & ((1u << lane) - 1u));
+			if (later) {
+				if (pos < a.defer_cap) {
+					defer[pos] = make_uint4(ql, row, __float_as_uint(d - err), 0u);
+				} else {
+					a.incomplete[q0 + ql] = 1u;
+				}
+			}
+			ndef = min(ndef + __popc(dm), a.defer_cap);
+			if constexpr (kDiag != 0) {
+				n_deferred += __popc(dm);
+			}
+		}
 		const unsigned todo = __ballot_sync(0xffffffffu, rescore);
 		if (todo) {
-			[[maybe_unused]] const long long c0 = kDiag == kTcDiagStamps ? clock64() : 0ll;
-			const float dx = a.metric == kL2 ? tc_rescore<true>(a, todo, row, ql, q0, lane) : tc_rescore<false>(a, todo, row, ql, q0, lane);
-			if constexpr (kDiag != 0) {
-				n_rescored += __popc(todo);
-				if constexpr (kDiag == kTcDiagStamps) {
-					rescore_cycles += clock64() - c0;
-				}
-			}
-			if (rescore && dx < tc_min_thr<kNq>(s_thr, ql)) {
-				if constexpr (kDiag != 0) {
-					++n_inserts;
-				}
-				const float nt = tc_bound_insert(a, q0 + ql, dx);
-				for (uint32_t w = 0; w < kTcConsumers; ++w) {
-					if (nt < s_thr[w * kNq + ql]) {
-						s_thr[w * kNq + ql] = nt;
-					}
-				}
-			}
+			tc_score_rows<kNq, kDiag>(a, todo, rescore, row, ql, q0, s_thr, lane, n_rescored, n_inserts, rescore_cycles);
 		}
 		__syncwarp();
 	}
@@ -507,6 +568,35 @@
 			atomicAdd(&dg[kTcDgRescored], n_rescored);
 			atomicAdd(&dg[kTcDgInserts], ins);
 			atomicAdd(&dg[kTcDgRescoreCycles], (unsigned long long)rescore_cycles);
+			atomicAdd(&dg[kTcDgDeferred], n_deferred);
+			atomicAdd(&dg[kTcDgDrainScored], n_drain_scored);
+			atomicAdd(&dg[kTcDgDrainDropped], n_drain_dropped);
+			atomicAdd(&dg[kTcDgDrainPending], (unsigned long long)ndef);
+		}
+	}
+	return ndef;
+}
+
+template <int kNq, int kDiag>
+__device__ __forceinline__ void tc_drain_deferred(const TcArgs& a, const uint32_t* ndef, uint32_t q0, float* s_thr, int warp, int lane,
+												  unsigned long long* dg) {
+	[[maybe_unused]] unsigned long long n_rescored = 0, n_inserts = 0, n_scored = 0, n_dropped = 0;
+	[[maybe_unused]] long long rescore_cycles = 0;
+	const uint32_t c0 = (ndef[0] + 31) / 32, c1 = c0 + (ndef[1] + 31) / 32, nchunks = c1 + (ndef[2] + 31) / 32;
+	for (uint32_t c = uint32_t(warp); c < nchunks; c += kTcThreads / 32) {
+		const uint32_t b = c < c0 ? 0u : c < c1 ? 1u : 2u, i = c - (b == 0 ? 0u : b == 1 ? c0 : c1);
+		const uint4* e = a.defer + (size_t(blockIdx.x) * kTcConsumers + b) * a.defer_cap + i * 32;
+		tc_drain_chunk<kNq, kDiag>(a, e, min(ndef[b] - i * 32, 32u), q0, s_thr, lane, n_scored, n_dropped, n_rescored, n_inserts,
+								   rescore_cycles);
+	}
+	if constexpr (kDiag != 0) {
+		const unsigned long long ins = __reduce_add_sync(0xffffffffu, uint32_t(n_inserts));
+		if (lane == 0) {
+			atomicAdd(&dg[kTcDgRescored], n_rescored);
+			atomicAdd(&dg[kTcDgInserts], ins);
+			atomicAdd(&dg[kTcDgRescoreCycles], (unsigned long long)rescore_cycles);
+			atomicAdd(&dg[kTcDgDrainScored], n_scored);
+			atomicAdd(&dg[kTcDgDrainDropped], n_dropped);
 		}
 	}
 }
@@ -541,7 +631,8 @@
 	int* s_tb = reinterpret_cast<int*>(s_thr + kTcConsumers * kNq);
 	TcQueue* s_queue = reinterpret_cast<TcQueue*>(s_tb + kTcConsumers * kNq);
 	uint4* s_rec = reinterpret_cast<uint4*>(s_queue + kTcConsumers);
-	static_assert(2 * kTcStages + 2 <= 32, "barriers and (a*, b*) fit in front of the per-query constants");
+	uint32_t* s_ndef = reinterpret_cast<uint32_t*>(s_ab + 2);
+	static_assert(2 * kTcStages + 1 + 3 <= 32, "barriers, (a*, b*) and s_ndef fit in front of the per-query constants");
 
 	const int warp = __shfl_sync(0xffffffffu, int(threadIdx.x >> 5), 0), lane = threadIdx.x & 31;
 	const uint32_t ntiles = (a.n + kTcTileRows - 1) / kTcTileRows;
@@ -644,7 +735,11 @@
 		}
 	} else if (warp < 4) {
 		const uint32_t wg = uint32_t(warp) - 1;
-		tc_bookkeeper<kNq, kDiag>(a, s_queue + wg, s_rec + wg * a.queue_slots, a.queue_slots, q0, s_qc, s_thr, lane, dg);
+		uint4* defer = a.defer ? a.defer + (size_t(blockIdx.x) * kTcConsumers + wg) * a.defer_cap : nullptr;
+		const uint32_t left = tc_bookkeeper<kNq, kDiag>(a, s_queue + wg, s_rec + wg * a.queue_slots, a.queue_slots, q0, s_qc, s_thr, lane, dg, defer);
+		if (lane == 0) {
+			s_ndef[wg] = left;
+		}
 	} else {
 		const uint32_t wg = uint32_t(warp) / 4 - 1, wtid = threadIdx.x - 128 * (wg + 1);
 		float* thr = s_thr + wg * kNq;
@@ -843,6 +938,15 @@
 		}
 	}
 	__syncthreads();
+	if (a.defer) {
+		[[maybe_unused]] const long long c0 = clk();
+		tc_drain_deferred<kNq, kDiag>(a, s_ndef, q0, s_thr, warp, lane, dg);
+		if constexpr (kStamp) {
+			if (lane == 0) {
+				atomicAdd(&dg[kTcDgDrainTail], (unsigned long long)(clk() - c0));
+			}
+		}
+	}
 	if constexpr (kStamp) {
 		if (threadIdx.x < kTcConsumers) {
 			dg[threadIdx.x * kTcDgPerWg + kTcDgQueueWait] = s_queue[threadIdx.x].full_waits;
@@ -1279,90 +1383,119 @@
 	}
 }
 
-constexpr int kTcInitQ = 4;
+constexpr int kTcInitQ = 16;
 constexpr uint32_t kTcInitRows = 4096;
-__host__ __device__ inline size_t tc_init_smem_bytes() { return size_t(kTcInitQ) * kTcInitRows * sizeof(float); }
-__global__ void __launch_bounds__(256) tc_init_tau(const float* rows, uint32_t pitch, uint32_t kchunks, const float* norm_coefs, uint32_t nrows,
-												   const float* qf, uint32_t nq, uint32_t k1, int metric, unsigned int* tau, float* ub_list,
-												   unsigned int* ub_lock) {
+constexpr uint32_t kTcInitSlice = 1024;
+constexpr uint32_t kTcInitSlices = kTcInitRows / kTcInitSlice;
+__host__ __device__ inline size_t tc_init_smem_bytes() { return size_t(kTcInitQ) * kTcInitSlice * sizeof(float); }
+__global__ void __launch_bounds__(256, 2) tc_init_tau(const float* rows, uint32_t pitch, uint32_t kchunks, const float* norm_coefs,
+													   uint32_t nrows, const float* qf, uint32_t nq, uint32_t k1, int metric, uint64_t* seed) {
 	extern __shared__ __align__(16) float s_d[];
-	const uint32_t q0 = blockIdx.x * kTcInitQ;
+	const uint32_t q0 = blockIdx.x * kTcInitQ, slice = blockIdx.y, slices = gridDim.y;
+	const uint32_t rb = slice * kTcInitSlice, nr = min(nrows - rb, kTcInitSlice);
 	const uint32_t lane = threadIdx.x & 31, warp = threadIdx.x >> 5;
 	const float4* rows4 = reinterpret_cast<const float4*>(rows);
-	const float4* q4[kTcInitQ];
-#pragma unroll
-	for (int qi = 0; qi < kTcInitQ; ++qi) {
-		q4[qi] = reinterpret_cast<const float4*>(qf) + size_t(q0 + qi < nq ? q0 + qi : q0) * kchunks * 32u;
-	}
-	constexpr uint32_t kRows = 4;
-	for (uint32_t r0 = warp * kRows; r0 < kTcInitRows; r0 += 8 * kRows) {
+	constexpr uint32_t kRows = 2;
+	for (uint32_t r0 = warp * kRows; r0 < nr; r0 += 8 * kRows) {
 		float dist[kRows][kTcInitQ];
-		if (r0 < nrows) {
-			uint32_t rr[kRows];
-			const float4* qp[kRows][kTcInitQ];
-#pragma unroll
-			for (uint32_t x = 0; x < kRows; ++x) {
-				rr[x] = min(r0 + x, nrows - 1);
-#pragma unroll
-				for (int qi = 0; qi < kTcInitQ; ++qi) {
-					qp[x][qi] = q4[qi];
-				}
-			}
-			if (metric == kL2) {
-				row_dists_warp<true, kRows, kTcInitQ>(rows4, pitch / 4, kchunks, rr, qp, nullptr, lane, dist);
-			} else {
-				row_dists_warp<false, kRows, kTcInitQ>(rows4, pitch / 4, kchunks, rr, qp, norm_coefs, lane, dist);
-			}
-		}
+		uint32_t rr[kRows];
+		const float4* qp[kRows][kTcInitQ];
 #pragma unroll
 		for (uint32_t x = 0; x < kRows; ++x) {
+			rr[x] = rb + min(r0 + x, nr - 1);
 #pragma unroll
 			for (int qi = 0; qi < kTcInitQ; ++qi) {
-				if (lane == uint32_t(qi)) {
-					const uint32_t r = r0 + x;
-					s_d[qi * kTcInitRows + r] = r < nrows ? dist[x][qi] : INFINITY;
+				qp[x][qi] = reinterpret_cast<const float4*>(qf) + size_t(q0 + qi < nq ? q0 + qi : q0) * kchunks * 32u;
+			}
+		}
+		if (metric == kL2) {
+			row_dists_warp<true, kRows, kTcInitQ>(rows4, pitch / 4, kchunks, rr, qp, nullptr, lane, dist);
+		} else {
+			row_dists_warp<false, kRows, kTcInitQ>(rows4, pitch / 4, kchunks, rr, qp, norm_coefs, lane, dist);
+		}
+#pragma unroll
+		for (uint32_t x = 0; x < kRows; ++x) {
+#pragma unroll
+			for (int qi = 0; qi < kTcInitQ; ++qi) {
+				if (lane == (x * kTcInitQ + qi) % 32u && r0 + x < nr) {
+					s_d[qi * kTcInitSlice + r0 + x] = dist[x][qi];
 				}
 			}
 		}
 	}
 	__syncthreads();
-	if (warp < kTcInitQ && q0 + warp < nq) {
-		const uint32_t q = q0 + warp;
-		float* d = s_d + warp * kTcInitRows;
-		float last = INFINITY;
-		for (uint32_t round = 0; round < kTcMaxK1; ++round) {
-			float best = INFINITY;
-			uint32_t at = lane;
-			if (round < k1) {
-				for (uint32_t j = lane; j < kTcInitRows; j += 32) {
-					const float y = d[j];
-					if (y < best) {
-						best = y;
-						at = j;
-					}
-				}
-				for (int off = 16; off > 0; off >>= 1) {
-					const float ob = __shfl_xor_sync(0xffffffffu, best, off);
-					const uint32_t oa = __shfl_xor_sync(0xffffffffu, at, off);
-					if (ob < best || (ob == best && oa < at)) {
-						best = ob;
-						at = oa;
-					}
-				}
-				if (lane == 0) {
-					d[at] = INFINITY;
-				}
-				__syncwarp();
-				last = best;
+	for (uint32_t qi = warp; qi < uint32_t(kTcInitQ) && q0 + qi < nq; qi += 8) {
+		const float* d = s_d + qi * kTcInitSlice;
+		uint64_t* out = seed + (size_t(q0 + qi) * slices + slice) * k1;
+		uint64_t last = 0;
+		for (uint32_t round = 0; round < k1; ++round) {
+			uint64_t best = kKeyNone;
+			for (uint32_t j = lane; j < nr; j += 32) {
+				const uint64_t key = make_key(d[j], rb + j);
+				if ((round == 0 || key > last) && key < best) {
+					best = key;
+				}
+			}
+#pragma unroll
+			for (int off = 16; off > 0; off >>= 1) {
+				const uint64_t o = __shfl_xor_sync(0xffffffffu, best, off);
+				best = o < best ? o : best;
 			}
 			if (lane == 0) {
-				ub_list[size_t(q) * kTcMaxK1 + round] = round < k1 ? best : -INFINITY;
-			}
-		}
-		if (lane == 0) {
-			tau[q] = float_ord(last);
-			ub_lock[q] = 0;
-		}
+				out[round] = best;
+			}
+			last = best;
+		}
+	}
+}
+__global__ void tc_init_tau_merge(const uint64_t* seed, uint32_t nq, uint32_t slices, uint32_t k1, unsigned int* tau, uint64_t* ub_list,
+								  unsigned int* ub_lock) {
+	const uint32_t q = blockIdx.x * blockDim.x + threadIdx.x;
+	if (q >= nq) {
+		return;
+	}
+	const uint64_t* in = seed + size_t(q) * slices * k1;
+	uint32_t head[kTcInitSlices];
+#pragma unroll
+	for (uint32_t s = 0; s < kTcInitSlices; ++s) {
+		head[s] = 0;
+	}
+	uint64_t last = kKeyNone;
+	for (uint32_t r = 0; r < k1; ++r) {
+		uint64_t best = kKeyNone;
+		uint32_t from = 0;
+#pragma unroll
+		for (uint32_t s = 0; s < kTcInitSlices; ++s) {
+			const uint64_t key = s < slices && head[s] < k1 ? in[size_t(s) * k1 + head[s]] : kKeyNone;
+			if (key < best) {
+				best = key;
+				from = s;
+			}
+		}
+#pragma unroll
+		for (uint32_t s = 0; s < kTcInitSlices; ++s) {
+			head[s] += best != kKeyNone && s == from;
+		}
+		ub_list[size_t(q) * kTcMaxK1 + r] = best;
+		last = best;
+	}
+	tau[q] = tc_key_tau(last);
+	ub_lock[q] = 0;
+}
+
+__global__ void __launch_bounds__(kTcMaxK1) tc_sort_bound_lists(const uint64_t* ub_list, uint32_t k1, uint64_t* lists) {
+	__shared__ uint64_t s_keys[kTcMaxK1];
+	const uint32_t q = blockIdx.x, t = threadIdx.x;
+	const uint64_t key = t < k1 ? ub_list[size_t(q) * kTcMaxK1 + t] : kKeyNone;
+	s_keys[t] = key;
+	__syncthreads();
+	if (t < k1) {
+		uint32_t at = 0;
+		for (uint32_t j = 0; j < k1; ++j) {
+			const uint64_t o = s_keys[j];
+			at += o < key || (o == key && j < t);
+		}
+		lists[size_t(q) * k1 + at] = key;
 	}
 }
 
```

After: 77960, median of 6. 1.03x the previous value.
